# lachlants/denet

Hardware: AMD Instinct MI355X
Metric: images/sec train step, DeNet-34 skip 512x512 (higher is better)
Workload: dtype f32

## Files before the change

denet_amd/build.py:

```python
import hashlib
import os
import subprocess
import sys

HERE = os.path.dirname(os.path.abspath(__file__))
CSRC = os.path.join(HERE, "csrc")
LIB = os.path.join(CSRC, "libdenet_hip.so")

SOURCES = ["runtime.hip", "igemm.hip", "bn.hip", "pool.hip", "elementwise.hip", "dss.hip", "samples.hip", "detect.hip", "winograd.hip", "wino2f.hip", "wino4f.hip", "wino4t.hip", "dgrad_s2.hip", "wino4g.hip", "stem.hip", "gemm3b.hip", "bn_moments.hip",
           "regression.hip", "augment.hip", "image.hip", "activation.hip", "conv_rect.hip", "pool_border.hip"]
NO_CONTRACT = {"dss.hip", "samples.hip", "detect.hip", "augment.hip", "image.hip"}
COMMON = ["--offload-arch=gfx950", "-O3", "-std=c++17", "-fPIC", "-Wall", "-Wno-unused-function"]


def _hipcc_version(hipcc):
    try:
        return subprocess.run([hipcc, "--version"], check=True, capture_output=True, text=True).stdout
    except (OSError, subprocess.CalledProcessError):
        return "unknown"


def _digest(parts, files):
    h = hashlib.sha256()
    for p in parts:
        h.update(p.encode())
        h.update(b"\0")
    for f in files:
        with open(f, "rb") as fh:
            h.update(hashlib.sha256(fh.read()).digest())
    return h.hexdigest()


def _stale(target, digest):
    stamp = target + ".sha256"
    if not (os.path.exists(target) and os.path.exists(stamp)):
        return True
    with open(stamp) as f:
        return f.read().strip() != digest


def _stamp(target, digest):
    with open(target + ".sha256", "w") as f:
        f.write(digest + "\n")


def build(force=False, verbose=False):
    hipcc = os.environ.get("HIPCC", "/opt/rocm/bin/hipcc")
    if not os.path.exists(hipcc):
        hipcc = "hipcc"
    version = _hipcc_version(hipcc)
    objs, todo = [], []
    headers = [os.path.join(CSRC, "common.h"), os.path.join(CSRC, "bn_final.h"), os.path.join(HERE, "..", "include", "denet_hip.h")]
    for src in SOURCES:
        s = os.path.join(CSRC, src)
        o = os.path.join(CSRC, src.replace(".hip", ".o"))
        objs.append(o)
        flags = COMMON + (["-ffp-contract=off"] if src in NO_CONTRACT else [])
        digest = _digest([version] + flags, [s] + headers)
        if force or _stale(o, digest):
            todo.append(([hipcc] + flags + ["-c", s, "-o", o], o, digest))
    todo.sort(key=lambda t: -os.path.getsize(t[0][-3]))
    running = []
    jobs = max(1, min(len(todo), int(os.environ.get("DENET_BUILD_JOBS", os.cpu_count() or 1))))

    def reap(block):
        for ent in list(running):
            proc, cmd, o, digest = ent
            rc = proc.wait() if block else proc.poll()
            if rc is None:
                continue
            running.remove(ent)
            if rc != 0:
                for other in running:
                    other[0].kill()
                raise subprocess.CalledProcessError(rc, cmd)
            _stamp(o, digest)
            if block:
                return

    for cmd, o, digest in todo:
        while len(running) >= jobs:
            reap(block=True)
        if verbose:
            print(" ".join(cmd), flush=True)
        running.append((subprocess.Popen(cmd), cmd, o, digest))
    while running:
        reap(block=True)
    link = ["--offload-arch=gfx950", "-shared", "-fPIC"]
    digest = _digest([version] + link, objs)
    if force or _stale(LIB, digest):
        cmd = [hipcc] + link + ["-o", LIB] + objs
        if verbose:
            print(" ".join(cmd), flush=True)
        subprocess.run(cmd, check=True)
        _stamp(LIB, digest)
    return LIB


if __name__ == "__main__":
    print(build(force="--force" in sys.argv, verbose=True))
```

denet_amd/csrc/dgrad_s2.hip:

```cpp
#include "common.h"
#include "../../include/denet_hip.h"
#include <stdlib.h>

namespace {

typedef __attribute__((address_space(3))) void* lds_ptr_t;
typedef int i32x4_t __attribute__((ext_vector_type(4)));

__device__ __forceinline__ void s2_store_b128(const f32x4& v, const i32x4_t& rsrc, int voff, int soff) {
    asm volatile("buffer_store_dwordx4 %0, %1, %2, %3 offen\n\ts_nop 1" ::"v"(v), "v"(voff), "s"(rsrc), "s"(soff) : "memory");
}

struct S2Params {
    const float* dy;
    const float* wp;
    const float* add;
    float* dx;
    double* stats;
    const float* bs_x;
    const float* bs_y;
    const float* bs_gamma;
    const float* bs_beta;
    const float* bs_mean;
    const float* bs_invstd;
    int bs_relu;
    int N, H, W, C, K, OH, OW;
    int bh, bw;
    int tiles_c;
    int chunks;
    unsigned dy_bytes, dx_bytes, w_bytes;
};

constexpr int S2_OOB = (int)0xF0000000u;
constexpr int S2_SLOTS = 81 * 16;
constexpr int S2_PIECES = 21;
constexpr int S2_BUF = S2_PIECES * 1024;
constexpr int S2_LDS = 2 * S2_BUF + 1024;
constexpr int S2_D = 9;
constexpr int S2_R = 18;

#define S2_WAIT_VM(vm) __builtin_amdgcn_s_waitcnt(((vm) & 15) | ((((vm) >> 4) & 3) << 14) | (7 << 4) | (15 << 8))
#define S2_BARRIER()                       \
    {                                      \
        asm volatile("" ::: "memory");     \
        __builtin_amdgcn_s_barrier();      \
        asm volatile("" ::: "memory");     \
    }

__device__ __forceinline__ int s2_key(int pi, int pj) { return ((pi & 1) << 3) | (pj & 7); }

template <int EP>
__global__ __launch_bounds__(256, 2) void dgrad_s2_kernel(const S2Params p) {
    extern __shared__ __attribute__((aligned(16))) char smem[];
    const int tid = threadIdx.x, lane = tid & 63;
    const int wave = __builtin_amdgcn_readfirstlane(tid >> 6);
    const uint32_t bid = xcd_remap(blockIdx.x, gridDim.x);
    const int cblk = (int)(bid % (uint32_t)p.tiles_c);
    const int brow = (int)(bid / (uint32_t)p.tiles_c);
    int blk = brow;
    const int bx = blk % p.bw;
    blk /= p.bw;
    const int by = blk % p.bh;
    const int n = blk / p.bh;
    const int c0 = cblk * 64;
    const int i0 = by * 8, j0 = bx * 8;
    const __amdgpu_buffer_rsrc_t rD = __builtin_amdgcn_make_buffer_rsrc((void*)p.dy, 0, p.dy_bytes, 0x00020000);
    const __amdgpu_buffer_rsrc_t rW = __builtin_amdgcn_make_buffer_rsrc((void*)p.wp, 0, p.w_bytes, 0x00020000);

    int pc_off[6];
#pragma unroll
    for (int j = 0; j < 6; ++j) {
        const int L = (wave + 4 * j) * 64 + lane;
        const int pos = L >> 4, sl = L & 15;
        const int pi = pos / 9, pj = pos - pi * 9;
        const int i = i0 + pi, jj = j0 + pj;
        const bool ok = L < S2_SLOTS && i < p.OH && jj < p.OW;
        pc_off[j] = ok ? (((n * p.OH + i) * p.OW + jj) * p.K + 4 * (sl ^ s2_key(pi, pj))) * 4 : S2_OOB;
    }
    int d_chunk = 0;
    auto issue = [&]() {
        const bool live = d_chunk < p.chunks;
        char* const dstb = smem + (d_chunk & 1) * S2_BUF;
#pragma unroll
        for (int j = 0; j < 6; ++j) {
            const int piece = wave + 4 * j;
            char* const dst = piece < S2_PIECES ? dstb + piece * 1024 : smem + 2 * S2_BUF;
            __builtin_amdgcn_raw_ptr_buffer_load_lds(rD, (lds_ptr_t)dst, 16, live ? pc_off[j] : S2_OOB, d_chunk * 256, 0, 0);
        }
        d_chunk += 1;
    };

    const int r15 = lane & 15, g = lane >> 4;
    const int w_voff = ((c0 + 16 * wave + r15) * 16 + 4 * g) * 4;
    const int w_tap = p.C * 64;
    const int w_step = 9 * w_tap;
    const int pr = r15 >> 3, pq = r15 & 7;
    int v_base[2][2];
    int v_key[2][2];
#pragma unroll
    for (int di = 0; di < 2; ++di)
#pragma unroll
        for (int dj = 0; dj < 2; ++dj) {
            v_base[di][dj] = ((pr + di) * 9 + pq + dj) * 256;
            v_key[di][dj] = s2_key(pr + di, pq + dj);
        }

    f32x4 acc[4][4];
#pragma unroll
    for (int a = 0; a < 4; ++a)
#pragma unroll
        for (int b = 0; b < 4; ++b) acc[a][b] = f32x4{0.f, 0.f, 0.f, 0.f};

    f32x4 fw[S2_R];
    const int steps_total = p.chunks * 4;
    auto load_w = [&](int s, int gt) {
        int st = 4 * s + gt / 9;
        st = st < steps_total ? st : steps_total - 1;
        fw[gt % S2_R] = __builtin_bit_cast(f32x4, __builtin_amdgcn_raw_buffer_load_b128(rW, w_voff, st * w_step + (gt % 9) * w_tap, 0));
    };

    issue();
    issue();
#pragma unroll
    for (int t = 0; t < S2_D; ++t) load_w(0, t);

    for (int s = 0; s < p.chunks; ++s) {
        S2_WAIT_VM(S2_D);
        S2_BARRIER();
        if (s >= 1) issue();
        const char* const buf = smem + (s & 1) * S2_BUF;
#pragma unroll
        for (int q = 0; q < 4; ++q) {
            f32x4 dv[2][2][4];
#pragma unroll
            for (int di = 0; di < 2; ++di)
#pragma unroll
                for (int dj = 0; dj < 2; ++dj)
#pragma unroll
                    for (int pb = 0; pb < 4; ++pb)
                        dv[di][dj][pb] = *(const f32x4*)(buf + v_base[di][dj] + pb * (2 * 9 * 256) + (((4 * q + g) ^ v_key[di][dj]) << 4));
            __builtin_amdgcn_sched_barrier(0);
#pragma unroll
            for (int tap = 0; tap < 9; ++tap) {
                const int gt = 9 * q + tap;
                load_w(s, gt + S2_D);
                const int r = tap / 3, sx = tap % 3;
                const int py = r == 1 ? 0 : 1, di = r == 0 ? 1 : 0;
                const int px = sx == 1 ? 0 : 1, dj = sx == 0 ? 1 : 0;
                const f32x4 wv = fw[gt % S2_R];
#pragma unroll
                for (int k = 0; k < 4; ++k)
#pragma unroll
                    for (int pb = 0; pb < 4; ++pb)
                        acc[2 * py + px][pb] = __builtin_amdgcn_mfma_f32_16x16x4f32(wv[k], dv[di][dj][pb][k], acc[2 * py + px][pb], 0, 0, 0);
                __builtin_amdgcn_sched_group_barrier(0x008, 1, 0);
                __builtin_amdgcn_sched_group_barrier(0x020, 1, 0);
                __builtin_amdgcn_sched_group_barrier(0x008, 15, 0);
                __builtin_amdgcn_sched_barrier(0);
            }
        }
    }
    __builtin_amdgcn_s_waitcnt(0);

    const f32x4 z = {0.f, 0.f, 0.f, 0.f};
    const i32x4_t rsX = {(int)(unsigned)(unsigned long long)p.dx, (int)(((unsigned long long)p.dx >> 32) & 0xffffu), (int)p.dx_bytes, 0x00020000};
    const __amdgpu_buffer_rsrc_t rA = __builtin_amdgcn_make_buffer_rsrc((void*)p.add, 0, p.add ? p.dx_bytes : 0u, 0x00020000);
    const __amdgpu_buffer_rsrc_t rBX = __builtin_amdgcn_make_buffer_rsrc((void*)p.bs_x, 0, p.bs_x ? p.dx_bytes : 0u, 0x00020000);
    const __amdgpu_buffer_rsrc_t rBY = __builtin_amdgcn_make_buffer_rsrc((void*)p.bs_y, 0, p.bs_y ? p.dx_bytes : 0u, 0x00020000);
    const bool has_add = p.add != nullptr;
    const bool mask_y = p.bs_relu && p.bs_y, mask_x = p.bs_relu && !p.bs_y;
    const int kc = c0 + 16 * wave + 4 * g;
    double ds[8];
#pragma unroll
    for (int c = 0; c < 8; ++c) ds[c] = 0.0;
    f32x4 bmu = z, bis = z, bsc = z, bsh = z;
    if (EP == 2) {
        bmu = *(const f32x4*)(p.bs_mean + kc);
        bis = *(const f32x4*)(p.bs_invstd + kc);
#pragma unroll
        for (int c = 0; c < 4; ++c) {
            bsc[c] = (p.bs_gamma ? p.bs_gamma[kc + c] : 1.f) * bis[c];
            bsh[c] = (p.bs_beta ? p.bs_beta[kc + c] : 0.f) - bmu[c] * bsc[c];
        }
    }
#pragma unroll
    for (int pb = 0; pb < 4; ++pb) {
        const int i = i0 + 2 * pb + pr, j = j0 + pq;
        const bool valid = i < p.OH && j < p.OW;
        const int voff = valid ? (((n * p.H + 2 * i) * p.W + 2 * j) * p.C + kc) * 4 : S2_OOB;
        f32x4 ssum = z, ssq = z;
        f32x4 av[4], xv[4], yv[4];
#pragma unroll
        for (int cl = 0; cl < 4; ++cl) {
            const int soff = ((cl >> 1) * p.W + (cl & 1)) * p.C * 4;
            av[cl] = z;
            if (has_add) av[cl] = __builtin_bit_cast(f32x4, __builtin_amdgcn_raw_buffer_load_b128(rA, voff, soff, 0));
            if (EP == 2) {
                xv[cl] = __builtin_bit_cast(f32x4, __builtin_amdgcn_raw_buffer_load_b128(rBX, voff, soff, 0));
                yv[cl] = __builtin_bit_cast(f32x4, __builtin_amdgcn_raw_buffer_load_b128(rBY, voff, soff, 0));
            }
        }
#pragma unroll
        for (int cl = 0; cl < 4; ++cl) {
            const int soff = ((cl >> 1) * p.W + (cl & 1)) * p.C * 4;
            const f32x4 o = acc[cl][pb] + av[cl];
            s2_store_b128(o, rsX, voff, soff);
            if (EP == 2) {
                f32x4 gq;
#pragma unroll
                for (int c = 0; c < 4; ++c) {
                    const float mk = mask_y ? yv[cl][c] : (mask_x ? fmaf(xv[cl][c], bsc[c], bsh[c]) : 1.f);
                    gq[c] = mk > 0.f ? o[c] : 0.f;
                    ssq[c] += gq[c] * ((xv[cl][c] - bmu[c]) * bis[c]);
                }
                ssum += gq;
            }
        }
        if (EP == 2 && valid) {
#pragma unroll
            for (int c = 0; c < 4; ++c) {
                ds[c] += (double)ssum[c];
                ds[4 + c] += (double)ssq[c];
            }
        }
    }
    if (EP != 2) return;
#pragma unroll
    for (int c = 0; c < 8; ++c) {
#pragma unroll
        for (int sh = 8; sh > 0; sh >>= 1) {
            const long long b = __double_as_longlong(ds[c]);
            int lo, hi;
            if (sh == 8) { lo = __builtin_amdgcn_update_dpp(0, (int)b, 0x128, 0xF, 0xF, false); hi = __builtin_amdgcn_update_dpp(0, (int)(b >> 32), 0x128, 0xF, 0xF, false); }
            else if (sh == 4) { lo = __builtin_amdgcn_update_dpp(0, (int)b, 0x124, 0xF, 0xF, false); hi = __builtin_amdgcn_update_dpp(0, (int)(b >> 32), 0x124, 0xF, 0xF, false); }
            else if (sh == 2) { lo = __builtin_amdgcn_update_dpp(0, (int)b, 0x122, 0xF, 0xF, false); hi = __builtin_amdgcn_update_dpp(0, (int)(b >> 32), 0x122, 0xF, 0xF, false); }
            else { lo = __builtin_amdgcn_update_dpp(0, (int)b, 0x121, 0xF, 0xF, false); hi = __builtin_amdgcn_update_dpp(0, (int)(b >> 32), 0x121, 0xF, 0xF, false); }
            ds[c] += __longlong_as_double(((long long)hi << 32) | (unsigned)lo);
        }
    }
    if (r15 == 0 && kc < p.C) {
        double* row = p.stats + (long)brow * 2 * p.C;
#pragma unroll
        for (int c = 0; c < 4; ++c) {
            row[kc + c] = ds[c];
            row[p.C + kc + c] = ds[4 + c];
        }
    }
}

__global__ __launch_bounds__(256) void dgrad_s2_pack_kernel(const float* __restrict__ w, float* __restrict__ P, int K, int C) {
    const long idx = (long)blockIdx.x * 256 + threadIdx.x;
    const long total = 9L * K * C;
    if (idx >= total) return;
    const int kk = (int)(idx & 15);
    long rest = idx >> 4;
    const int c = (int)(rest % C);
    rest /= C;
    const int tap = (int)(rest % 9);
    const int kc = (int)(rest / 9);
    P[idx] = w[((long)(kc * 16 + kk) * 9 + tap) * C + c];
}

}

extern "C" int denet_conv_dgrad_s2_ok(int N, int H, int W, int C, int K) {
    return (N > 0 && H > 0 && W > 0 && H % 2 == 0 && W % 2 == 0 && C > 0 && C % 64 == 0 && K > 0 && K % 64 == 0 &&
            (long)N * H * W * C * 4 < 0x7FFFFFFFL && (long)N * (H / 2) * (W / 2) * K * 4 < 0x7FFFFFFFL && 9L * K * C * 4 < 0x7FFFFFFFL) ? 1 : 0;
}

extern "C" int denet_conv_dgrad_s2_stats_rows(int N, int H, int W) {
    return N * ((H / 2 + 7) / 8) * ((W / 2 + 7) / 8);
}

extern "C" int denet_conv_dgrad_s2_pack(const float* w, float* packed, int C, int K, hipStream_t stream) {
    DENET_CHECK_ARG(w && packed && C > 0 && K > 0 && K % 16 == 0, "conv_dgrad_s2_pack: bad arguments");
    const long total = 9L * K * C;
    hipLaunchKernelGGL(dgrad_s2_pack_kernel, dim3((unsigned)((total + 255) / 256)), dim3(256), 0, stream, w, packed, K, C);
    DENET_CHECK_LAUNCH("conv_dgrad_s2_pack");
    return DENET_OK;
}

extern "C" int denet_conv_dgrad_s2(const float* dy, const float* w_packed, const float* add, float* dx, const denet_bn_link* sums_of,
                                   double* stats_partial, size_t stats_bytes, int* stats_rows, int N, int H, int W, int C, int K,
                                   hipStream_t stream) {
    DENET_CHECK_ARG(dy && w_packed && dx, "conv_dgrad_s2: null pointer");
    DENET_CHECK_ARG(denet_conv_dgrad_s2_ok(N, H, W, C, K), "conv_dgrad_s2: needs even H and W, C %% 64 = 0, K %% 64 = 0");
    S2Params p = {};
    p.dy = dy; p.wp = w_packed; p.add = add; p.dx = dx;
    p.N = N; p.H = H; p.W = W; p.C = C; p.K = K; p.OH = H / 2; p.OW = W / 2;
    p.bh = (p.OH + 7) / 8; p.bw = (p.OW + 7) / 8;
    p.tiles_c = C / 64; p.chunks = K / 64;
    p.dy_bytes = (unsigned)((size_t)N * p.OH * p.OW * K * 4);
    p.dx_bytes = (unsigned)((size_t)N * H * W * C * 4);
    p.w_bytes = (unsigned)((size_t)9 * K * C * 4);
    const long blocks = (long)N * p.bh * p.bw;
    int ep = 0;
    if (sums_of) {
        DENET_CHECK_ARG(stats_partial && stats_rows && stats_bytes >= (size_t)blocks * 2 * C * sizeof(double), "conv_dgrad_s2: statistics buffer too small");
        DENET_CHECK_ARG(sums_of->x && sums_of->mean && sums_of->invstd && (!sums_of->relu || sums_of->y || (sums_of->gamma && sums_of->beta)),
                        "conv_dgrad_s2: incomplete batch-norm description for the backward sums");
        *stats_rows = (int)blocks;
        p.stats = stats_partial;
        p.bs_x = sums_of->x; p.bs_y = sums_of->relu ? sums_of->y : nullptr; p.bs_gamma = sums_of->gamma; p.bs_beta = sums_of->beta;
        p.bs_mean = sums_of->mean; p.bs_invstd = sums_of->invstd; p.bs_relu = sums_of->relu;
        ep = 2;
    } else if (stats_rows) {
        *stats_rows = 0;
    }
    typedef void (*kern_t)(const S2Params);
    const kern_t fn = ep == 2 ? dgrad_s2_kernel<2> : dgrad_s2_kernel<0>;
    const int prof = denet_prof_begin(17, ep, 0, 0, stream);
    hipLaunchKernelGGL(fn, dim3((unsigned)(blocks * p.tiles_c)), dim3(256), S2_LDS, stream, p);
    denet_prof_end(prof, stream);
    DENET_CHECK_LAUNCH("conv_dgrad_s2");
    return DENET_OK;
}
```

denet_amd/csrc/gemm3b.hip:

```cpp
#include "common.h"

namespace {

typedef __bf16 bf16x8 __attribute__((ext_vector_type(8)));
typedef __bf16 bf16x2 __attribute__((ext_vector_type(2)));
typedef float f32x2 __attribute__((ext_vector_type(2)));
typedef unsigned u32x4 __attribute__((ext_vector_type(4)));

constexpr int BM = 128, BN = 128, BK = 32;
constexpr int ROWB = 80;
constexpr int IMG = BM * ROWB;
constexpr int OOBV = (int)0xF0000000u;

struct G3Params {
    const float* a;
    const float* b;
    const float* bias;
    float* c;
    int M, N, K;
    unsigned a_bytes, b_bytes;
};

__device__ __forceinline__ void split4(const f32x4 v, unsigned (&hi)[2], unsigned (&lo)[2]) {
#pragma unroll
    for (int p = 0; p < 2; ++p) {
        const f32x2 x = {v[2 * p], v[2 * p + 1]};
        const unsigned h = __builtin_bit_cast(unsigned, __builtin_convertvector(x, bf16x2));
        const f32x2 back = {__builtin_bit_cast(float, h << 16), __builtin_bit_cast(float, h & 0xFFFF0000u)};
        const f32x2 r = x - back;
        hi[p] = h;
        lo[p] = __builtin_bit_cast(unsigned, __builtin_convertvector(r, bf16x2));
    }
}

__global__ __launch_bounds__(256, 3) void gemm3b_nt_kernel(const G3Params p) {
    __shared__ __attribute__((aligned(16))) char smem[4 * IMG];
    char* Ah = smem;
    char* Al = smem + IMG;
    char* Bh = smem + 2 * IMG;
    char* Bl = smem + 3 * IMG;
    const int tid = threadIdx.x, lane = tid & 63, wave = tid >> 6;
    const int wm = wave & 1, wn = wave >> 1;
    const uint32_t tiles_n = p.N / BN;
    const uint32_t tile = xcd_remap(blockIdx.x, gridDim.x);
    const int m0 = (int)(tile / tiles_n) * BM, n0 = (int)(tile % tiles_n) * BN;
    const __amdgpu_buffer_rsrc_t ra = __builtin_amdgcn_make_buffer_rsrc((void*)p.a, 0, p.a_bytes, 0x00020000);
    const __amdgpu_buffer_rsrc_t rb = __builtin_amdgcn_make_buffer_rsrc((void*)p.b, 0, p.b_bytes, 0x00020000);
    const int lrow = tid >> 3, lk = (tid & 7) * 4;
    const int a_off = ((m0 + lrow) * p.K + lk) * 4, b_off = ((n0 + lrow) * p.K + lk) * 4;
    f32x4 ga[4], gb[4];
    auto gload = [&](int k0) {
#pragma unroll
        for (int i = 0; i < 4; ++i) {
            ga[i] = __builtin_bit_cast(f32x4, __builtin_amdgcn_raw_buffer_load_b128(
                ra, m0 + lrow + 32 * i < p.M ? a_off + (32 * i * p.K + k0) * 4 : OOBV, 0, 0));
            gb[i] = __builtin_bit_cast(f32x4, __builtin_amdgcn_raw_buffer_load_b128(rb, b_off + (32 * i * p.K + k0) * 4, 0, 0));
        }
    };
    typedef unsigned u32x2 __attribute__((ext_vector_type(2)));
    auto stage = [&]() {
#pragma unroll
        for (int i = 0; i < 4; ++i) {
            const int o = (lrow + 32 * i) * ROWB + lk * 2;
            unsigned h[2], l[2];
            split4(ga[i], h, l);
            *(u32x2*)(Ah + o) = u32x2{h[0], h[1]};
            *(u32x2*)(Al + o) = u32x2{l[0], l[1]};
            split4(gb[i], h, l);
            *(u32x2*)(Bh + o) = u32x2{h[0], h[1]};
            *(u32x2*)(Bl + o) = u32x2{l[0], l[1]};
        }
    };

    f32x16 acc[2][2];
#pragma unroll
    for (int i = 0; i < 2; ++i)
#pragma unroll
        for (int j = 0; j < 2; ++j)
#pragma unroll
            for (int e = 0; e < 16; ++e) acc[i][j][e] = 0.f;

    const int fa = (64 * wm + (lane & 31)) * ROWB + (lane >> 5) * 16;
    const int fb = (64 * wn + (lane & 31)) * ROWB + (lane >> 5) * 16;

    gload(0);
    stage();
    __syncthreads();
    const int nk = p.K / BK;
    for (int kb = 0; kb < nk; ++kb) {
        if (kb + 1 < nk) gload((kb + 1) * BK);
#pragma unroll
        for (int ks = 0; ks < 2; ++ks) {
            bf16x8 ah[2], al[2], bh[2], bl[2];
#pragma unroll
            for (int t = 0; t < 2; ++t) {
                ah[t] = *(const bf16x8*)(Ah + fa + t * 32 * ROWB + ks * 32);
                al[t] = *(const bf16x8*)(Al + fa + t * 32 * ROWB + ks * 32);
                bh[t] = *(const bf16x8*)(Bh + fb + t * 32 * ROWB + ks * 32);
                bl[t] = *(const bf16x8*)(Bl + fb + t * 32 * ROWB + ks * 32);
            }
#pragma unroll
            for (int i = 0; i < 2; ++i)
#pragma unroll
                for (int j = 0; j < 2; ++j) {
                    acc[i][j] = __builtin_amdgcn_mfma_f32_32x32x16_bf16(bh[j], al[i], acc[i][j], 0, 0, 0);
                    acc[i][j] = __builtin_amdgcn_mfma_f32_32x32x16_bf16(bl[j], ah[i], acc[i][j], 0, 0, 0);
                    acc[i][j] = __builtin_amdgcn_mfma_f32_32x32x16_bf16(bh[j], ah[i], acc[i][j], 0, 0, 0);
                }
        }
        __syncthreads();
        if (kb + 1 < nk) {
            stage();
            __syncthreads();
        }
    }
#pragma unroll
    for (int i = 0; i < 2; ++i) {
        const int m = m0 + 64 * wm + 32 * i + (lane & 31);
        if (m >= p.M) continue;
#pragma unroll
        for (int j = 0; j < 2; ++j)
#pragma unroll
            for (int q = 0; q < 4; ++q) {
                const int n = n0 + 64 * wn + 32 * j + 8 * q + 4 * (lane >> 5);
                f32x4 v = {acc[i][j][4 * q], acc[i][j][4 * q + 1], acc[i][j][4 * q + 2], acc[i][j][4 * q + 3]};
                if (p.bias) v += *(const f32x4*)(p.bias + n);
                *(f32x4*)(p.c + (long)m * p.N + n) = v;
            }
    }
}

__global__ __launch_bounds__(256) void transpose_f32_kernel(const float* __restrict__ src, float* __restrict__ dst, int R, int C) {
    __shared__ float tile[64][65];
    const int r0 = blockIdx.y * 64, c0 = blockIdx.x * 64;
    const int tx = threadIdx.x & 63, ty = threadIdx.x >> 6;
#pragma unroll
    for (int i = 0; i < 16; ++i) {
        const int r = r0 + ty + 4 * i, c = c0 + tx;
        tile[ty + 4 * i][tx] = (r < R && c < C) ? src[(long)r * C + c] : 0.f;
    }
    __syncthreads();
#pragma unroll
    for (int i = 0; i < 16; ++i) {
        const int c = c0 + ty + 4 * i, r = r0 + tx;
        if (r < R && c < C) dst[(long)c * R + r] = tile[tx][ty + 4 * i];
    }
}

}

extern "C" int denet_gemm_bf16x3_ok(int M, int N, int K) {
    return (M > 0 && N > 0 && K > 0 && N % 128 == 0 && K % 32 == 0 && (long)M * K * 4 < 0xF0000000L && (long)N * K * 4 < 0xF0000000L) ? 1 : 0;
}

extern "C" int denet_gemm_bf16x3_nt(const float* a, const float* b, const float* bias, float* c, int M, int N, int K,
                                    hipStream_t stream) {
    DENET_CHECK_ARG(a && b && c, "gemm_bf16x3_nt: null pointer");
    DENET_CHECK_ARG(denet_gemm_bf16x3_ok(M, N, K), "gemm_bf16x3_nt: needs N %% 128 = 0, K %% 32 = 0");
    G3Params p = {a, b, bias, c, M, N, K, (unsigned)((size_t)M * K * 4), (unsigned)((size_t)N * K * 4)};
    const unsigned tiles = (unsigned)(((M + BM - 1) / BM) * (N / BN));
    hipLaunchKernelGGL(gemm3b_nt_kernel, dim3(tiles), dim3(256), 0, stream, p);
    DENET_CHECK_LAUNCH("gemm_bf16x3_nt");
    return DENET_OK;
}

extern "C" int denet_transpose_f32(const float* src, float* dst, int R, int C, hipStream_t stream) {
    DENET_CHECK_ARG(src && dst && R > 0 && C > 0, "transpose_f32: bad arguments");
    hipLaunchKernelGGL(transpose_f32_kernel, dim3((C + 63) / 64, (R + 63) / 64), dim3(256), 0, stream, src, dst, R, C);
    DENET_CHECK_LAUNCH("transpose_f32");
    return DENET_OK;
}
```

denet_amd/csrc/wino4t.hip:

```cpp
#include "common.h"
#include "bn_final.h"
#include "../../include/denet_hip.h"
#include <stdlib.h>
#include <type_traits>

namespace {

typedef __attribute__((address_space(3))) void* lds_ptr_t;
typedef float f32x2 __attribute__((ext_vector_type(2)));
typedef int i32x4_t __attribute__((ext_vector_type(4)));

__device__ __forceinline__ void t_store_b128(const f32x4& v, const i32x4_t& rsrc, int voff, int soff) {
    asm volatile("buffer_store_dwordx4 %0, %1, %2, %3 offen\n\ts_nop 1" ::"v"(v), "v"(voff), "s"(rsrc), "s"(soff) : "memory");
}

struct W4TParams {
    const float* x;
    const float* U;
    const float* bias;
    const float* add;
    float* y;
    double* stats;
    const float* bs_x;
    const float* bs_y;
    const float* bs_gamma;
    const float* bs_beta;
    const float* bs_mean;
    const float* bs_invstd;
    int bs_relu;
    int N, H, W, C, K;
    int bh, bw;
    int tiles_k;
    int chunks;
    int relu;
    unsigned x_bytes, y_bytes, u_bytes;
    unsigned long long* dbg;
};

constexpr int T_OOB = (int)0xF0000000u;
constexpr int T_ROWS = 10;
constexpr int T_QS = 38;
constexpr int T_PLANE_SLOTS = T_ROWS * T_QS;
constexpr int T_PLANE_B = T_PLANE_SLOTS * 16;
constexpr int T_PATCH_SLOTS = 4 * T_PLANE_SLOTS;
constexpr int T_PATCH_B = 24 * 1024;
constexpr int T_V_B = 36 * 1024;
constexpr int T_LDS = T_PATCH_B + T_V_B;
#ifndef T_STAG
#define T_STAG 0
#endif
#ifndef T_STAG_N
#define T_STAG_N 1
#endif
#ifndef T_D_
#define T_D_ 3
#endif
#ifndef T_ISSUE_
#define T_ISSUE_ 9
#endif
constexpr int T_D = T_D_;
constexpr int T_R = 12;
constexpr int T_ISSUE = T_ISSUE_;
static_assert(36 % T_R == 0 && T_R >= 2 * T_D + 2, "the ring index must run on across chunks and cover the fragments in flight");

#define T_WAITCNT(vm) __builtin_amdgcn_s_waitcnt(((vm) & 15) | ((((vm) >> 4) & 3) << 14) | (7 << 4))
#define T_WAIT_VM(vm) __builtin_amdgcn_s_waitcnt(((vm) & 15) | ((((vm) >> 4) & 3) << 14) | (7 << 4) | (15 << 8))
#define T_BARRIER()                        \
    {                                      \
        asm volatile("" ::: "memory");     \
        __builtin_amdgcn_s_barrier();      \
        asm volatile("" ::: "memory");     \
    }

template <int LH>
__device__ __forceinline__ void t_bt3(const f32x2 (&d)[6], f32x2 (&o)[3]) {
    if (LH == 0) {
        o[0] = __builtin_elementwise_fma(f32x2{-5.f, -5.f}, d[2], __builtin_elementwise_fma(f32x2{4.f, 4.f}, d[0], d[4]));
        const f32x2 p = __builtin_elementwise_fma(f32x2{-4.f, -4.f}, d[2], d[4]);
        const f32x2 q = __builtin_elementwise_fma(f32x2{-4.f, -4.f}, d[1], d[3]);
        o[1] = p + q;
        o[2] = p - q;
    } else {
        const f32x2 p = d[4] - d[2];
        const f32x2 q = d[3] - d[1];
        o[0] = __builtin_elementwise_fma(f32x2{2.f, 2.f}, q, p);
        o[1] = __builtin_elementwise_fma(f32x2{-2.f, -2.f}, q, p);
        o[2] = __builtin_elementwise_fma(f32x2{-5.f, -5.f}, d[3], __builtin_elementwise_fma(f32x2{4.f, 4.f}, d[1], d[5]));
    }
}
__device__ __forceinline__ void t_bt6(const f32x2 (&t)[6], f32x2 (&o)[6]) {
    o[0] = __builtin_elementwise_fma(f32x2{-5.f, -5.f}, t[2], __builtin_elementwise_fma(f32x2{4.f, 4.f}, t[0], t[4]));
    const f32x2 p = __builtin_elementwise_fma(f32x2{-4.f, -4.f}, t[2], t[4]);
    const f32x2 q = __builtin_elementwise_fma(f32x2{-4.f, -4.f}, t[1], t[3]);
    o[1] = p + q;
    o[2] = p - q;
    const f32x2 p2 = t[4] - t[2];
    const f32x2 q2 = t[3] - t[1];
    o[3] = __builtin_elementwise_fma(f32x2{2.f, 2.f}, q2, p2);
    o[4] = __builtin_elementwise_fma(f32x2{-2.f, -2.f}, q2, p2);
    o[5] = __builtin_elementwise_fma(f32x2{-5.f, -5.f}, t[3], __builtin_elementwise_fma(f32x2{4.f, 4.f}, t[1], t[5]));
}

template <int LH>
__device__ __forceinline__ void t_transform(const char* prd, char* vwr) {
    f32x2 t[3][6];
#pragma unroll
    for (int b = 0; b < 6; ++b) {
        f32x2 d[6];
#pragma unroll
        for (int a = LH; a < LH + 5; ++a) d[a] = *(const f32x2*)(prd + (a * T_QS + (b & 3) * 9 + (b >> 2)) * 16);
        if (LH == 0) d[5] = f32x2{0.f, 0.f};
        else d[0] = f32x2{0.f, 0.f};
        f32x2 o[3];
        t_bt3<LH>(d, o);
        t[0][b] = o[0];
        t[1][b] = o[1];
        t[2][b] = o[2];
    }
#pragma unroll
    for (int i = 0; i < 3; ++i) {
        f32x2 o[6];
        t_bt6(t[i], o);
#pragma unroll
        for (int m = 0; m < 6; ++m) *(f32x2*)(vwr + (6 * (3 * LH + i) + m) * 1024) = o[m];
    }
}

template <int N>
__device__ __forceinline__ double t_row_ror(double v) {
    const long long b = __double_as_longlong(v);
    const int lo = __builtin_amdgcn_update_dpp(0, (int)b, 0x120 + N, 0xF, 0xF, false);
    const int hi = __builtin_amdgcn_update_dpp(0, (int)(b >> 32), 0x120 + N, 0xF, 0xF, false);
    return __longlong_as_double(((long long)hi << 32) | (unsigned)lo);
}

constexpr float T_AT[4][6] = {{1, 1, 1, 1, 1, 0}, {0, 1, -1, 2, -2, 0}, {0, 1, 1, 4, 4, 0}, {0, 1, -1, 8, -8, 1}};

#ifdef T_TRACE
#define T_STAMP() if (p.dbg && (blockIdx.x & 63) == 0 && tid == 0 && dbg_n < 32) p.dbg[(blockIdx.x >> 6) * 32 + dbg_n++] = __builtin_amdgcn_s_memtime()
#else
#define T_STAMP()
#endif
#ifndef T_EXP
#define T_EXP 0
#endif

template <int EP>
__global__ __launch_bounds__(256, 2) void wino4t_kernel(const W4TParams p) {
    extern __shared__ __attribute__((aligned(16))) char smem[];
    char* const vbuf = smem + T_PATCH_B;
    const int tid = threadIdx.x, lane = tid & 63;
    const int wave = __builtin_amdgcn_readfirstlane(tid >> 6);
    const uint32_t bid = xcd_remap(blockIdx.x, gridDim.x);
    const int kblk = (int)(bid % (uint32_t)p.tiles_k);
    const int brow = (int)(bid / (uint32_t)p.tiles_k);
    int blk = brow;
    const int bx = blk % p.bw;
    blk /= p.bw;
    const int by = blk % p.bh;
    const int n = blk / p.bh;
    const int k0 = kblk * 64;
    const int y0 = by * 8, x0 = bx * 32;
    const __amdgpu_buffer_rsrc_t rX = __builtin_amdgcn_make_buffer_rsrc((void*)p.x, 0, p.x_bytes, 0x00020000);

    int pc_off[6];
#pragma unroll
    for (int j = 0; j < 6; ++j) {
        const int L = (wave + 4 * j) * 64 + lane;
        const int pl = L / T_PLANE_SLOTS, rem = L - pl * T_PLANE_SLOTS;
        const int row = rem / T_QS, q = rem - row * T_QS;
        const int v = q / 9, u = q - v * 9;
        const int pcx = 4 * u + v;
        const int iy = y0 - 1 + row, ix = x0 - 1 + pcx;
        const bool ok = L < T_PATCH_SLOTS && q < 36 && pcx < 34 && (unsigned)iy < (unsigned)p.H && (unsigned)ix < (unsigned)p.W;
        pc_off[j] = ok ? (((n * p.H + iy) * p.W + ix) * p.C + pl * 4) * 4 : T_OOB;
    }
    int d_chunk = 0;
    auto issue = [&]() {
        if (T_EXP & 8) return;
        const bool live = d_chunk < p.chunks;
#pragma unroll
        for (int j = 0; j < 6; ++j)
            __builtin_amdgcn_raw_ptr_buffer_load_lds(rX, (lds_ptr_t)(smem + (wave + 4 * j) * 1024), 16, live ? pc_off[j] : T_OOB,
                                                     d_chunk * 64, 0, 0);
        d_chunk += 1;
    };

    const int t_half = lane & 1, t_tx = (lane >> 1) & 7, t_ty = (lane >> 4) & 1;
    const int t_cq = ((lane >> 5) & 1) | ((wave & 1) << 1), t_lh = wave >> 1;
    const int t_rd = t_cq * T_PLANE_B + (4 * t_ty * T_QS + t_tx) * 16 + t_half * 8;
    char* const t_wr = vbuf + t_cq * 256 + (t_ty * 8 + t_tx) * 16 + t_half * 8;

    const int r15 = lane & 15, g = lane >> 4;
    const int kw = wave;
    const char* const v_rd = vbuf + g * 256 + r15 * 16;
    const __amdgpu_buffer_rsrc_t rU = __builtin_amdgcn_make_buffer_rsrc((void*)p.U, 0, p.u_bytes, 0x00020000);
    const int u_voff = ((k0 + 16 * ((T_EXP & 256) ? (kw & 1) : kw) + r15) * 16 + 4 * g) * 4;
    const int u_xi = p.K * 64;
    const int u_chunk = 36 * u_xi;

    f32x4 acc[36];
#pragma unroll
    for (int i = 0; i < 36; ++i) acc[i] = f32x4{0.f, 0.f, 0.f, 0.f};

    f32x4 fu[T_R];
    if (T_EXP & 32) {
#pragma unroll
        for (int i = 0; i < T_R; ++i) asm volatile("" : "=v"(fu[i]));
    }
    auto load_u = [&](int chunk, int pair) {
        if (T_EXP & 32) return;
        if ((T_EXP & 128) && (pair & 1)) {
            fu[(2 * pair) % T_R] = fu[(2 * pair - 2) % T_R];
            fu[(2 * pair + 1) % T_R] = fu[(2 * pair - 1) % T_R];
            return;
        }
        const int so = chunk * u_chunk + (2 * pair) * u_xi;
        fu[(2 * pair) % T_R] = __builtin_bit_cast(f32x4, __builtin_amdgcn_raw_buffer_load_b128(rU, u_voff, so, 0));
        fu[(2 * pair + 1) % T_R] = __builtin_bit_cast(f32x4, __builtin_amdgcn_raw_buffer_load_b128(rU, u_voff, so + u_xi, 0));
    };
    f32x4 fv[2][2];
    if (T_EXP & 64) asm volatile("" : "=v"(fv[0][0]), "=v"(fv[0][1]), "=v"(fv[1][0]), "=v"(fv[1][1]));
    auto read_v = [&](int pair) {
        if (T_EXP & 64) return;
        fv[pair & 1][0] = *(const f32x4*)(v_rd + (2 * pair) * 1024);
        fv[pair & 1][1] = *(const f32x4*)(v_rd + (2 * pair + 1) * 1024);
    };

#if T_STAG
    {
        const bool late = T_STAG == 1 ? ((blockIdx.x >> 8) & 1) && blockIdx.x < 512 : (blockIdx.x & 1) && blockIdx.x < 512;
        if (late) {
#pragma unroll
            for (int i = 0; i < T_STAG_N; ++i) __builtin_amdgcn_s_sleep(115);
        }
    }
#endif
    int dbg_n = 0;
    (void)dbg_n;
    T_STAMP();
    issue();
    if (!(T_EXP & 2)) {
#pragma unroll
        for (int pr = 0; pr < T_D; ++pr) load_u(0, pr);
    }

    for (int s = 0; s < p.chunks; ++s) {
        T_WAIT_VM(2 * T_D);
        T_STAMP();
        T_BARRIER();
        T_STAMP();
        if (!(T_EXP & 1)) {
            const char* prd = smem + t_rd;
            if (t_lh == 0) t_transform<0>(prd, t_wr);
            else t_transform<1>(prd, t_wr);
        }
        T_WAITCNT(63);
        T_STAMP();
        T_BARRIER();
        T_STAMP();
        if (!(T_EXP & 2)) {
            const int sn = s + 1 < p.chunks ? s + 1 : s;
            read_v(0);
            __builtin_amdgcn_sched_barrier(0);
#pragma unroll
            for (int pr = 0; pr < 18; ++pr) {
                if (pr + T_D < 18) load_u(s, pr + T_D);
                else load_u(sn, pr + T_D - 18);
                if (pr + 1 < 18) read_v(pr + 1);
                const f32x4 ua = fu[(2 * pr) % T_R], ub = fu[(2 * pr + 1) % T_R];
                const f32x4 va = fv[pr & 1][0], vb = fv[pr & 1][1];
#pragma unroll
                for (int j = 0; j < 4; ++j) {
                    acc[2 * pr] = __builtin_amdgcn_mfma_f32_16x16x4f32(ua[j], va[j], acc[2 * pr], 0, 0, 0);
                    acc[2 * pr + 1] = __builtin_amdgcn_mfma_f32_16x16x4f32(ub[j], vb[j], acc[2 * pr + 1], 0, 0, 0);
                }
                __builtin_amdgcn_sched_group_barrier(0x008, 1, 0);
                __builtin_amdgcn_sched_group_barrier(0x020, 1, 0);
                __builtin_amdgcn_sched_group_barrier(0x008, 1, 0);
                __builtin_amdgcn_sched_group_barrier(0x020, 1, 0);
                if (pr + 1 < 18) {
                    __builtin_amdgcn_sched_group_barrier(0x008, 1, 0);
                    __builtin_amdgcn_sched_group_barrier(0x100, 1, 0);
                    __builtin_amdgcn_sched_group_barrier(0x008, 1, 0);
                    __builtin_amdgcn_sched_group_barrier(0x100, 1, 0);
                    __builtin_amdgcn_sched_group_barrier(0x008, 4, 0);
                } else {
                    __builtin_amdgcn_sched_group_barrier(0x008, 6, 0);
                }
                __builtin_amdgcn_sched_barrier(0);
                if (pr == T_ISSUE && s + 1 < p.chunks) {
                    issue();
                    __builtin_amdgcn_sched_barrier(0);
                }
            }
        } else if (s + 1 < p.chunks) {
            issue();
        }
    }
    T_STAMP();
    if (T_EXP & 4) {
#pragma unroll
        for (int i = 0; i < 36; ++i) asm volatile("" ::"v"(acc[i]));
        return;
    }

    f32x4 Y[16];
    {
        f32x4 Z[6][4];
#pragma unroll
        for (int l = 0; l < 6; ++l)
#pragma unroll
            for (int j = 0; j < 4; ++j) {
                f32x4 a = {0.f, 0.f, 0.f, 0.f};
                bool fst = true;
#pragma unroll
                for (int m = 0; m < 6; ++m) {
                    const float c = T_AT[j][m];
                    if (c == 0.f) continue;
                    if (fst) a = c == 1.f ? acc[6 * l + m] : acc[6 * l + m] * c;
                    else if (c == 1.f) a += acc[6 * l + m];
                    else if (c == -1.f) a -= acc[6 * l + m];
                    else a = __builtin_elementwise_fma(f32x4{c, c, c, c}, acc[6 * l + m], a);
                    fst = false;
                }
                Z[l][j] = a;
            }
#pragma unroll
        for (int i = 0; i < 4; ++i)
#pragma unroll
            for (int j = 0; j < 4; ++j) {
                f32x4 a = {0.f, 0.f, 0.f, 0.f};
                bool fst = true;
#pragma unroll
                for (int l = 0; l < 6; ++l) {
                    const float c = T_AT[i][l];
                    if (c == 0.f) continue;
                    if (fst) a = c == 1.f ? Z[l][j] : Z[l][j] * c;
                    else if (c == 1.f) a += Z[l][j];
                    else if (c == -1.f) a -= Z[l][j];
                    else a = __builtin_elementwise_fma(f32x4{c, c, c, c}, Z[l][j], a);
                    fst = false;
                }
                Y[4 * i + j] = a;
            }
    }

    T_STAMP();
    const int oy = y0 + 4 * (r15 >> 3), ox = x0 + 4 * (r15 & 7);
    const f32x4 z = {0.f, 0.f, 0.f, 0.f};
    const i32x4_t rsY = {(int)(unsigned)(unsigned long long)p.y, (int)(((unsigned long long)p.y >> 32) & 0xffffu), (int)p.y_bytes, 0x00020000};
    const __amdgpu_buffer_rsrc_t rA = __builtin_amdgcn_make_buffer_rsrc((void*)p.add, 0, p.add ? p.y_bytes : 0u, 0x00020000);
    const __amdgpu_buffer_rsrc_t rBX = __builtin_amdgcn_make_buffer_rsrc((void*)p.bs_x, 0, p.bs_x ? p.y_bytes : 0u, 0x00020000);
    const __amdgpu_buffer_rsrc_t rBY = __builtin_amdgcn_make_buffer_rsrc((void*)p.bs_y, 0, p.bs_y ? p.y_bytes : 0u, 0x00020000);
    const float floor_ = p.relu ? 0.f : -__builtin_inff();
    const bool has_add = p.add != nullptr;
    const bool mask_y = p.bs_relu && p.bs_y, mask_x = p.bs_relu && !p.bs_y;
    double ds[8];
    const int kc = k0 + 16 * kw + 4 * g;
    const bool valid = oy < p.H && ox < p.W && kc < p.K;
    {
#pragma unroll
        for (int c = 0; c < 8; ++c) ds[c] = 0.0;
        const int voff = valid ? (((n * p.H + oy) * p.W + ox) * p.K + kc) * 4 : T_OOB;
        const int voff_st = (T_EXP & 16) ? (valid ? (voff & 0xFFFFF) : T_OOB) : voff;
        const int kcs = valid ? kc : 0;
        f32x4 b = z;
        if (p.bias) b = *(const f32x4*)(p.bias + kcs);
        f32x4 bmu = z, bis = z, bsc = z, bsh = z;
        if (EP == 2) {
            bmu = *(const f32x4*)(p.bs_mean + kcs);
            bis = *(const f32x4*)(p.bs_invstd + kcs);
#pragma unroll
            for (int c = 0; c < 4; ++c) {
                bsc[c] = (p.bs_gamma ? p.bs_gamma[kcs + c] : 1.f) * bis[c];
                bsh[c] = (p.bs_beta ? p.bs_beta[kcs + c] : 0.f) - bmu[c] * bsc[c];
            }
        }
#pragma unroll
        for (int i = 0; i < 4; ++i) {
            f32x4 ssum = z, ssq = z;
            f32x4 av[4], xv[4], yv[4];
#pragma unroll
            for (int j = 0; j < 4; ++j) {
                const int soff = (i * p.W + j) * p.K * 4;
                av[j] = z;
                if (has_add) av[j] = __builtin_bit_cast(f32x4, __builtin_amdgcn_raw_buffer_load_b128(rA, voff, soff, 0));
                if (EP == 2) {
                    xv[j] = __builtin_bit_cast(f32x4, __builtin_amdgcn_raw_buffer_load_b128(rBX, voff, soff, 0));
                    yv[j] = __builtin_bit_cast(f32x4, __builtin_amdgcn_raw_buffer_load_b128(rBY, voff, soff, 0));
                }
            }
#pragma unroll
            for (int j = 0; j < 4; ++j) {
                const int soff = (i * p.W + j) * p.K * 4;
                f32x4 o = (Y[4 * i + j] + b) + av[j];
#pragma unroll
                for (int c = 0; c < 4; ++c) o[c] = fmaxf(o[c], floor_);
                t_store_b128(o, rsY, voff_st, soff);
                if (EP == 2) {
                    f32x4 gq;
#pragma unroll
                    for (int c = 0; c < 4; ++c) {
                        const float mk = mask_y ? yv[j][c] : (mask_x ? fmaf(xv[j][c], bsc[c], bsh[c]) : 1.f);
                        gq[c] = mk > 0.f ? o[c] : 0.f;
                        ssq[c] += gq[c] * ((xv[j][c] - bmu[c]) * bis[c]);
                    }
                    ssum += gq;
                } else if (EP == 1) {
                    ssum += o;
                    ssq += o * o;
                }
            }
            if (EP != 0 && valid) {
#pragma unroll
                for (int c = 0; c < 4; ++c) {
                    ds[c] += (double)ssum[c];
                    ds[4 + c] += (double)ssq[c];
                }
            }
        }
    }
    T_STAMP();
    if (EP == 0) return;
#pragma unroll
    for (int c = 0; c < 8; ++c) {
        ds[c] += t_row_ror<8>(ds[c]);
        ds[c] += t_row_ror<4>(ds[c]);
        ds[c] += t_row_ror<2>(ds[c]);
        ds[c] += t_row_ror<1>(ds[c]);
    }
    if (r15 == 0 && kc < p.K) {
        double* row = p.stats + (long)brow * 2 * p.K;
#pragma unroll
        for (int c = 0; c < 4; ++c) {
            row[kc + c] = ds[c];
            row[p.K + kc + c] = ds[4 + c];
        }
    }
    T_STAMP();
}

__global__ __launch_bounds__(256) void wino4t_pack_kernel(const float* __restrict__ U, float* __restrict__ P, int K, int C) {
    const long idx = (long)blockIdx.x * 256 + threadIdx.x;
    const long total = 36L * K * C / 4;
    if (idx >= total) return;
    const int q = (int)(idx & 3);
    long rest = idx >> 2;
    const int k = (int)(rest % K);
    rest /= K;
    const int xi = (int)(rest % 36);
    const int chunk = (int)(rest / 36);
    *(f32x4*)(P + idx * 4) = *(const f32x4*)(U + ((long)xi * K + k) * C + chunk * 16 + q * 4);
}

unsigned long long* g_w4t_dbg = nullptr;

}

#ifdef T_TRACE
extern "C" int denet_conv_wino4t_debug(unsigned long long* buf) { g_w4t_dbg = buf; return 0; }
#endif

extern "C" int denet_conv_wino4t_ok(int N, int H, int W, int C, int K) {
    return (N > 0 && H > 0 && W > 0 && H % 4 == 0 && W % 4 == 0 && C > 0 && C % 16 == 0 && K > 0 && K % 64 == 0 &&
            (long)N * H * W * C * 4 < 0x7FFFFFFFL && (long)N * H * W * K * 4 < 0x7FFFFFFFL && 36L * K * C * 4 < 0x7FFFFFFFL) ? 1 : 0;
}

extern "C" int denet_conv_wino4t_stats_rows(int N, int H, int W) {
    return N * ((H + 7) / 8) * ((W + 31) / 32);
}

extern "C" int denet_conv_wino4t_pack(const float* u, float* packed, int C, int K, hipStream_t stream) {
    DENET_CHECK_ARG(u && packed && C > 0 && C % 16 == 0 && K > 0, "conv_wino4t_pack: bad arguments");
    const long total = 36L * K * C / 4;
    hipLaunchKernelGGL(wino4t_pack_kernel, dim3((unsigned)((total + 255) / 256)), dim3(256), 0, stream, u, packed, K, C);
    DENET_CHECK_LAUNCH("conv_wino4t_pack");
    return DENET_OK;
}

extern "C" int denet_conv_wino4t_sums(const float* x, const float* u_packed, const float* bias, const float* add, float* y, int relu,
                                      double* stats_partial, size_t stats_bytes, int* stats_rows, const denet_bn_link* sums_of, int N,
                                      int H, int W, int C, int K, hipStream_t stream) {
    DENET_CHECK_ARG(x && u_packed && y, "conv_wino4t: null pointer");
    DENET_CHECK_ARG(denet_conv_wino4t_ok(N, H, W, C, K), "conv_wino4t: needs H, W %% 4 = 0, C %% 16 = 0, K %% 64 = 0");
    W4TParams p = {};
    p.x = x; p.U = u_packed; p.bias = bias; p.add = add; p.y = y;
    p.N = N; p.H = H; p.W = W; p.C = C; p.K = K;
    p.bh = (H + 7) / 8; p.bw = (W + 31) / 32;
    p.tiles_k = K / 64; p.chunks = C / 16; p.relu = relu;
    p.x_bytes = (unsigned)((size_t)N * H * W * C * 4);
    p.y_bytes = (unsigned)((size_t)N * H * W * K * 4);
    p.u_bytes = (unsigned)((size_t)36 * K * C * 4);
    p.dbg = g_w4t_dbg;
    const long blocks = (long)N * p.bh * p.bw;
    int ep = 0;
    if (stats_partial) {
        DENET_CHECK_ARG(stats_rows && stats_bytes >= (size_t)blocks * 2 * K * sizeof(double), "conv_wino4t: statistics buffer too small");
        *stats_rows = (int)blocks;
        p.stats = stats_partial;
        ep = 1;
        if (sums_of) {
            DENET_CHECK_ARG(sums_of->x && sums_of->mean && sums_of->invstd && (!sums_of->relu || sums_of->y || (sums_of->gamma && sums_of->beta)),
                            "conv_wino4t: incomplete batch-norm description for the backward sums");
            p.bs_x = sums_of->x; p.bs_y = sums_of->relu ? sums_of->y : nullptr; p.bs_gamma = sums_of->gamma; p.bs_beta = sums_of->beta;
            p.bs_mean = sums_of->mean; p.bs_invstd = sums_of->invstd; p.bs_relu = sums_of->relu;
            ep = 2;
        }
    }
    typedef void (*kern_t)(const W4TParams);
    static const kern_t kerns[3] = {wino4t_kernel<0>, wino4t_kernel<1>, wino4t_kernel<2>};
    static bool attr_done[3] = {};
    const kern_t fn = kerns[ep];
    if (!attr_done[ep]) {
        const hipError_t e = hipFuncSetAttribute((const void*)fn, hipFuncAttributeMaxDynamicSharedMemorySize, 163840);
        if (e != hipSuccess) {
            denet_set_error("conv_wino4t: hipFuncSetAttribute(%d B LDS): %s", T_LDS, hipGetErrorString(e));
            return -(int)e;
        }
        attr_done[ep] = true;
    }
    static const int lds_req = [] { const char* e = getenv("DENET_W4T_LDS"); const int v = e ? atoi(e) : 0; return v > T_LDS && v <= 163840 ? v : T_LDS; }();
    const int prof = denet_prof_begin(16, ep, 0, 0, stream);
    hipLaunchKernelGGL(fn, dim3((unsigned)(blocks * p.tiles_k)), dim3(256), lds_req, stream, p);
    denet_prof_end(prof, stream);
    DENET_CHECK_LAUNCH("conv_wino4t");
    return DENET_OK;
}
```

denet_amd/csrc/winograd.hip:

```cpp
#include "common.h"
#include <stdlib.h>
#include "../../include/denet_hip.h"

int denet_gemm_batched_nt(const float* a, const float* w, float* out, int batch, int M, int Nc, int Kc, long stride_a,
                          long stride_w, long stride_out, hipStream_t stream);
int denet_gemm_batched_tune(const float* a, const float* w, float* out, int batch, int M, int Nc, int Kc, long stride_a,
                            long stride_w, long stride_out, hipStream_t stream);

int denet_wgrad_batched(const float* x, const float* dy, float* dw, float* workspace, size_t workspace_bytes, int batch,
                        int T, int Cc, int Kr, hipStream_t stream);
int denet_wgrad_batched_tune(const float* x, const float* dy, float* dw, float* workspace, size_t workspace_bytes, int batch,
                             int T, int Cc, int Kr, hipStream_t stream);

int denet_wino4f_block(int tile, long T, int C, int K);
int denet_wino4f_stats_rows(int tb, long T);
int denet_wino4f_run(int tb, const float* V, const float* U, const float* bias, const float* add, float* y, double* stats,
                     const float* bs_x, const float* bs_y, const float* bs_gamma, const float* bs_beta, const float* bs_mean,
                     const float* bs_invstd, int bs_relu, int N, int H, int W, int C, int K, int relu, hipStream_t stream);

int denet_wino4g_splits(int tile, long T, int C, int K);
size_t denet_wino4g_workspace_bytes(int splits, int C, int K);
int denet_wino4g_run(int splits, const float* dM, const float* V, float* dU, float* part, size_t part_bytes, long T, int C, int K,
                     hipStream_t stream);

namespace {

__device__ __forceinline__ f32x4 ld4(const float* p) { return *(const f32x4*)p; }

template <int MO>
struct Wino;
template <>
struct Wino<2> {
    static constexpr int TS = 4;
    static constexpr float BT[4][4] = {{1, 0, -1, 0}, {0, 1, 1, 0}, {0, -1, 1, 0}, {0, 1, 0, -1}};
    static constexpr float G[4][3] = {{1, 0, 0}, {0.5f, 0.5f, 0.5f}, {0.5f, -0.5f, 0.5f}, {0, 0, 1}};
    static constexpr float AT[2][4] = {{1, 1, 1, 0}, {0, 1, -1, -1}};
};
template <>
struct Wino<4> {
    static constexpr int TS = 6;
    static constexpr float BT[6][6] = {{4, 0, -5, 0, 1, 0},  {0, -4, -4, 1, 1, 0}, {0, 4, -4, -1, 1, 0},
                                       {0, -2, -1, 2, 1, 0}, {0, 2, -1, -2, 1, 0}, {0, 4, 0, -5, 0, 1}};
    static constexpr float G[6][3] = {{0.25f, 0, 0},
                                      {-1.f / 6, -1.f / 6, -1.f / 6},
                                      {-1.f / 6, 1.f / 6, -1.f / 6},
                                      {1.f / 24, 1.f / 12, 1.f / 6},
                                      {1.f / 24, -1.f / 12, 1.f / 6},
                                      {0, 0, 1}};
    static constexpr float AT[4][6] = {{1, 1, 1, 1, 1, 0}, {0, 1, -1, 2, -2, 0}, {0, 1, 1, 4, 4, 0}, {0, 1, -1, 8, -8, 1}};
};

__device__ __forceinline__ float wino_fma(float c, float v, float acc) { return __builtin_fmaf(c, v, acc); }
__device__ __forceinline__ f32x4 wino_fma(float c, f32x4 v, f32x4 acc) {
    f32x4 r;
    r[0] = __builtin_fmaf(c, v[0], acc[0]);
    r[1] = __builtin_fmaf(c, v[1], acc[1]);
    r[2] = __builtin_fmaf(c, v[2], acc[2]);
    r[3] = __builtin_fmaf(c, v[3], acc[3]);
    return r;
}

#define WINO_DOT(acc, NL, COEF, VAL)                       \
    {                                                      \
        bool first_ = true;                                \
        _Pragma("unroll") for (int l_ = 0; l_ < (NL); ++l_) { \
            const float c_ = (COEF);                       \
            if (c_ != 0.f) {                               \
                if (first_) acc = c_ * (VAL);              \
                else acc = wino_fma(c_, (VAL), acc);       \
                first_ = false;                            \
            }                                              \
        }                                                  \
    }

template <int MO>
__global__ __launch_bounds__(256) void wino_input_kernel(const float* __restrict__ x, float* __restrict__ V, int N, int H,
                                                         int W, int C, int TH, int TW, long T, int up) {
    using WT = Wino<MO>;
    constexpr int TS = WT::TS;
    const int c4n = C / 4;
    const long idx = (long)blockIdx.x * 256 + threadIdx.x;
    if (idx >= T * c4n) return;
    const int c4 = (int)(idx % c4n);
    const long t = idx / c4n;
    const int tx = (int)(t % TW);
    const int ty = (int)((t / TW) % TH);
    const int n = (int)(t / ((long)TW * TH));
    const f32x4 z = {0.f, 0.f, 0.f, 0.f};
    f32x4 tt[TS][TS];
#pragma unroll
    for (int j = 0; j < TS; ++j) {
        const int ix = MO * tx - 1 + j;
        f32x4 d[TS];
#pragma unroll
        for (int i = 0; i < TS; ++i) {
            const int iy = MO * ty - 1 + i;
            const bool ok = ((unsigned)iy < (unsigned)H) && ((unsigned)ix < (unsigned)W);
            d[i] = ok ? ld4(x + (((long)n * (H >> up) + (iy >> up)) * (W >> up) + (ix >> up)) * C + c4 * 4) : z;
        }
#pragma unroll
        for (int i = 0; i < TS; ++i) {
            f32x4 acc = z;
            WINO_DOT(acc, TS, WT::BT[i][l_], d[l_]);
            tt[i][j] = acc;
        }
    }
#pragma unroll
    for (int i = 0; i < TS; ++i)
#pragma unroll
        for (int j = 0; j < TS; ++j) {
            f32x4 acc = z;
            WINO_DOT(acc, TS, WT::BT[j][l_], tt[i][l_]);
            *(f32x4*)(V + ((long)(TS * i + j) * T + t) * C + c4 * 4) = acc;
        }
}

struct BnFoldDev {
    const float* x;
    const float* aux;
    const float* y;
    const float* gamma;
    const float* beta;
    const float* mean;
    const float* invstd;
    const float* coef;
    float* out;
    int relu;
};

template <int MO, bool BWD>
__global__ __launch_bounds__(256) void wino_prep_kernel(BnFoldDev f, float* __restrict__ V, float* __restrict__ dM, int N, int H,
                                                        int W, int C, int TH, int TW, long T) {
    using WT = Wino<MO>;
    constexpr int TS = WT::TS;
    const int c4n = C / 4;
    const long idx = (long)blockIdx.x * 256 + threadIdx.x;
    if (idx >= T * c4n) return;
    const int c4 = (int)(idx % c4n);
    const long t = idx / c4n;
    const int tx = (int)(t % TW);
    const int ty = (int)((t / TW) % TH);
    const int n = (int)(t / ((long)TW * TH));
    const int c = c4 * 4;
    const f32x4 z = {0.f, 0.f, 0.f, 0.f};
    float mu[4], is[4], sc[4], sh[4], mg[4], mgx[4];
#pragma unroll
    for (int k = 0; k < 4; ++k) {
        mu[k] = f.mean[c + k];
        is[k] = f.invstd[c + k];
        sc[k] = f.gamma[c + k] * is[k];
        sh[k] = (f.beta ? f.beta[c + k] : 0.f) - mu[k] * sc[k];
        mg[k] = BWD ? f.coef[c + k] : 0.f;
        mgx[k] = BWD ? f.coef[C + c + k] : 0.f;
    }
    auto value = [&](int iy, int ix, bool inner) -> f32x4 {
        if (!(((unsigned)iy < (unsigned)H) && ((unsigned)ix < (unsigned)W))) return z;
        const long o = (((long)n * H + iy) * W + ix) * C + c;
        const f32x4 xv = ld4(f.x + o);
        f32x4 d;
        if (!BWD) {
#pragma unroll
            for (int k = 0; k < 4; ++k) d[k] = fmaf(xv[k], sc[k], sh[k]);
            if (f.aux) d += ld4(f.aux + o);
            if (f.relu) {
#pragma unroll
                for (int k = 0; k < 4; ++k) d[k] = fmaxf(d[k], 0.f);
            }
            if (inner) *(f32x4*)(f.out + o) = d;
        } else {
            f32x4 g = ld4(f.aux + o);
            if (f.relu) {
                if (f.y) {
                    const f32x4 yv = ld4(f.y + o);
#pragma unroll
                    for (int k = 0; k < 4; ++k) g[k] = yv[k] > 0.f ? g[k] : 0.f;
                } else {
#pragma unroll
                    for (int k = 0; k < 4; ++k) g[k] = fmaf(xv[k], sc[k], sh[k]) > 0.f ? g[k] : 0.f;
                }
            }
#pragma unroll
            for (int k = 0; k < 4; ++k) {
                const float xh = (xv[k] - mu[k]) * is[k];
                d[k] = sc[k] * (g[k] - mg[k] - xh * mgx[k]);
            }
            if (inner && f.out) *(f32x4*)(f.out + o) = g;
        }
        return d;
    };
    {
        f32x4 tt[TS][TS];
#pragma unroll
        for (int j = 0; j < TS; ++j) {
            const int ix = MO * tx - 1 + j;
            f32x4 d[TS];
#pragma unroll
            for (int i = 0; i < TS; ++i) d[i] = value(MO * ty - 1 + i, ix, i >= 1 && i <= MO && j >= 1 && j <= MO);
#pragma unroll
            for (int i = 0; i < TS; ++i) {
                f32x4 acc = z;
                WINO_DOT(acc, TS, WT::BT[i][l_], d[l_]);
                tt[i][j] = acc;
            }
        }
#pragma unroll
        for (int i = 0; i < TS; ++i)
#pragma unroll
            for (int j = 0; j < TS; ++j) {
                f32x4 acc = z;
                WINO_DOT(acc, TS, WT::BT[j][l_], tt[i][l_]);
                *(f32x4*)(V + ((long)(TS * i + j) * T + t) * C + c) = acc;
            }
    }
    if (BWD) {
        f32x4 a[TS][MO];
#pragma unroll
        for (int j = 0; j < MO; ++j) {
            f32x4 d[MO];
#pragma unroll
            for (int i = 0; i < MO; ++i) d[i] = value(MO * ty + i, MO * tx + j, false);
#pragma unroll
            for (int i = 0; i < TS; ++i) {
                f32x4 acc = z;
                WINO_DOT(acc, MO, WT::AT[l_][i], d[l_]);
                a[i][j] = acc;
            }
        }
#pragma unroll
        for (int i = 0; i < TS; ++i)
#pragma unroll
            for (int j = 0; j < TS; ++j) {
                f32x4 acc = z;
                WINO_DOT(acc, MO, WT::AT[l_][j], a[i][l_]);
                *(f32x4*)(dM + ((long)(TS * i + j) * T + t) * C + c) = acc;
            }
    }
}

template <int MO, bool BWD>
struct PrepLds {
    static constexpr int BT = 4;
    static constexpr int CQ = 8;
    static constexpr int PB = BT * MO;
    static constexpr int PP = PB + 2;
    static constexpr int NT = BT * BT * CQ;
    static constexpr int PS = CQ + 1;
    static constexpr size_t LDS = (size_t)PP * PP * PS * sizeof(f32x4);
};

template <int MO, bool BWD>
__global__ __launch_bounds__(128) void wino_prep_lds_kernel(BnFoldDev f, float* __restrict__ V, float* __restrict__ dM, int N,
                                                            int H, int W, int C, int TH, int TW, long T, int BH, int BW) {
    using WT = Wino<MO>;
    using PL = PrepLds<MO, BWD>;
    static_assert(PL::NT == 128, "launch bounds");
    constexpr int TS = WT::TS, BT = PL::BT, CQ = PL::CQ, PB = PL::PB, PP = PL::PP, NT = PL::NT, PS = PL::PS;
    extern __shared__ __attribute__((aligned(16))) unsigned char prep_smem[];
    f32x4* patch = (f32x4*)prep_smem;
    const int tid = threadIdx.x;
    const int cq = tid % CQ;
    const int cblk = blockIdx.y;
    const int c = (cblk * CQ + cq) * 4;
    int b = blockIdx.x;
    const int bx = b % BW; b /= BW;
    const int by = b % BH;
    const int n = b / BH;
    const f32x4 z = {0.f, 0.f, 0.f, 0.f};
    float mu[4], is[4], sc[4], sh[4], mg[4], mgx[4];
#pragma unroll
    for (int k = 0; k < 4; ++k) {
        mu[k] = f.mean[c + k];
        is[k] = f.invstd[c + k];
        sc[k] = f.gamma[c + k] * is[k];
        sh[k] = (f.beta ? f.beta[c + k] : 0.f) - mu[k] * sc[k];
        mg[k] = BWD ? f.coef[c + k] : 0.f;
        mgx[k] = BWD ? f.coef[C + c + k] : 0.f;
    }
    const int y0 = by * PB - 1, x0 = bx * PB - 1;
    constexpr int SLOTS = NT / CQ;
    constexpr int ROUNDS = (PP * PP + SLOTS - 1) / SLOTS;
    constexpr int UB = 7;
    for (int r0 = 0; r0 < ROUNDS; r0 += UB) {
        f32x4 xv[UB], av[UB], yv[UB];
        long off[UB];
        int pix[UB];
        bool ok[UB], inner[UB];
#pragma unroll
        for (int u = 0; u < UB; ++u) {
            const int p = (r0 + u) * SLOTS + tid / CQ;
            const int py = p / PP, px = p - py * PP;
            const int iy = y0 + py, ix = x0 + px;
            pix[u] = p;
            ok[u] = p < PP * PP && ((unsigned)iy < (unsigned)H) && ((unsigned)ix < (unsigned)W);
            inner[u] = py >= 1 && py <= PB && px >= 1 && px <= PB;
            off[u] = ok[u] ? (((long)n * H + iy) * W + ix) * C + c : (long)c;
            xv[u] = ld4(f.x + off[u]);
            if (BWD || f.aux) av[u] = ld4(f.aux + off[u]);
            if (BWD && f.relu && f.y) yv[u] = ld4(f.y + off[u]);
        }
#pragma unroll
        for (int u = 0; u < UB; ++u) {
            f32x4 d = z;
            if (!BWD) {
#pragma unroll
                for (int k = 0; k < 4; ++k) d[k] = fmaf(xv[u][k], sc[k], sh[k]);
                if (f.aux) d += av[u];
                if (f.relu) {
#pragma unroll
                    for (int k = 0; k < 4; ++k) d[k] = fmaxf(d[k], 0.f);
                }
                if (ok[u] && inner[u]) *(f32x4*)(f.out + off[u]) = d;
            } else {
                f32x4 g = av[u];
                if (f.relu) {
                    if (f.y) {
#pragma unroll
                        for (int k = 0; k < 4; ++k) g[k] = yv[u][k] > 0.f ? g[k] : 0.f;
                    } else {
#pragma unroll
                        for (int k = 0; k < 4; ++k) g[k] = fmaf(xv[u][k], sc[k], sh[k]) > 0.f ? g[k] : 0.f;
                    }
                }
#pragma unroll
                for (int k = 0; k < 4; ++k) {
                    const float xh = (xv[u][k] - mu[k]) * is[k];
                    d[k] = sc[k] * (g[k] - mg[k] - xh * mgx[k]);
                }
                if (ok[u] && inner[u] && f.out) *(f32x4*)(f.out + off[u]) = g;
            }
            if (pix[u] < PP * PP) patch[pix[u] * PS + cq] = ok[u] ? d : z;
        }
    }
    __syncthreads();
    const int tl = tid / CQ;
    const int tyl = tl / BT, txl = tl - tyl * BT;
    const int ty = by * BT + tyl, tx = bx * BT + txl;
    if (ty >= TH || tx >= TW) return;
    const long t = ((long)n * TH + ty) * TW + tx;
    {
        f32x4 tt[TS][TS];
#pragma unroll
        for (int j = 0; j < TS; ++j) {
            f32x4 d[TS];
#pragma unroll
            for (int i = 0; i < TS; ++i) d[i] = patch[((MO * tyl + i) * PP + MO * txl + j) * PS + cq];
#pragma unroll
            for (int i = 0; i < TS; ++i) {
                f32x4 acc = z;
                WINO_DOT(acc, TS, WT::BT[i][l_], d[l_]);
                tt[i][j] = acc;
            }
        }
#pragma unroll
        for (int i = 0; i < TS; ++i)
#pragma unroll
            for (int j = 0; j < TS; ++j) {
                f32x4 acc = z;
                WINO_DOT(acc, TS, WT::BT[j][l_], tt[i][l_]);
                *(f32x4*)(V + ((long)(TS * i + j) * T + t) * C + c) = acc;
            }
    }
    if (BWD) {
        f32x4 a[TS][MO];
#pragma unroll
        for (int j = 0; j < MO; ++j) {
            f32x4 d[MO];
#pragma unroll
            for (int i = 0; i < MO; ++i) d[i] = patch[((MO * tyl + 1 + i) * PP + MO * txl + 1 + j) * PS + cq];
#pragma unroll
            for (int i = 0; i < TS; ++i) {
                f32x4 acc = z;
                WINO_DOT(acc, MO, WT::AT[l_][i], d[l_]);
                a[i][j] = acc;
            }
        }
#pragma unroll
        for (int i = 0; i < TS; ++i)
#pragma unroll
            for (int j = 0; j < TS; ++j) {
                f32x4 acc = z;
                WINO_DOT(acc, MO, WT::AT[l_][j], a[i][l_]);
                *(f32x4*)(dM + ((long)(TS * i + j) * T + t) * C + c) = acc;
            }
    }
}

template <int MO, bool BWD>
int launch_prep_lds(const BnFoldDev& f, float* V, float* dM, int N, int H, int W, int C, int TH, int TW, long T, hipStream_t stream) {
    using PL = PrepLds<MO, BWD>;
    static bool attr_set = false;
    if (!attr_set) {
        const hipError_t e = hipFuncSetAttribute((const void*)wino_prep_lds_kernel<MO, BWD>, hipFuncAttributeMaxDynamicSharedMemorySize,
                                                 (int)PL::LDS);
        if (e != hipSuccess) {
            denet_set_error("conv_wino fold: hipFuncSetAttribute(%zu B LDS): %s", PL::LDS, hipGetErrorString(e));
            return -(int)e;
        }
        attr_set = true;
    }
    const int BH = (TH + PL::BT - 1) / PL::BT, BW = (TW + PL::BT - 1) / PL::BT;
    hipLaunchKernelGGL((wino_prep_lds_kernel<MO, BWD>), dim3((unsigned)(N * BH * BW), (unsigned)(C / (4 * PL::CQ))), dim3(PL::NT),
                       PL::LDS, stream, f, V, dM, N, H, W, C, TH, TW, T, BH, BW);
    return DENET_OK;
}

template <int MO, bool DGRAD>
__global__ __launch_bounds__(256) void wino_filter_kernel(const float* __restrict__ w, float* __restrict__ U, int K, int C) {
    using WT = Wino<MO>;
    constexpr int TS = WT::TS;
    const long idx = (long)blockIdx.x * 256 + threadIdx.x;
    if (idx >= (long)K * C) return;
    const int c = (int)(idx % C);
    const int k = (int)(idx / C);
    float g[3][3];
#pragma unroll
    for (int r = 0; r < 3; ++r)
#pragma unroll
        for (int s = 0; s < 3; ++s) g[r][s] = w[(((long)k * 3 + (DGRAD ? 2 - r : r)) * 3 + (DGRAD ? 2 - s : s)) * C + c];
    float a[TS][3];
#pragma unroll
    for (int i = 0; i < TS; ++i)
#pragma unroll
        for (int s = 0; s < 3; ++s) {
            float acc = 0.f;
            WINO_DOT(acc, 3, WT::G[i][l_], g[l_][s]);
            a[i][s] = acc;
        }
    const long KC = (long)K * C;
    const long o = DGRAD ? ((long)c * K + k) : ((long)k * C + c);
#pragma unroll
    for (int i = 0; i < TS; ++i)
#pragma unroll
        for (int j = 0; j < TS; ++j) {
            float acc = 0.f;
            WINO_DOT(acc, 3, WT::G[j][l_], a[i][l_]);
            U[(long)(TS * i + j) * KC + o] = acc;
        }
}

template <int MO>
__global__ __launch_bounds__(256) void wino_filter_dgrad_kernel(const float* __restrict__ w, float* __restrict__ U, int K,
                                                                int C) {
    using WT = Wino<MO>;
    constexpr int TS = WT::TS;
    __shared__ float tile[TS * TS][16][17];
    const int kl = threadIdx.x >> 4, cl = threadIdx.x & 15;
    const int k0 = blockIdx.y * 16, c0 = blockIdx.x * 16;
    {
        const int k = k0 + kl, c = c0 + cl;
        float g[3][3];
#pragma unroll
        for (int r = 0; r < 3; ++r)
#pragma unroll
            for (int q = 0; q < 3; ++q) g[r][q] = w[(((long)k * 3 + (2 - r)) * 3 + (2 - q)) * C + c];
        float a[TS][3];
#pragma unroll
        for (int i = 0; i < TS; ++i)
#pragma unroll
            for (int q = 0; q < 3; ++q) {
                float acc = 0.f;
                WINO_DOT(acc, 3, WT::G[i][l_], g[l_][q]);
                a[i][q] = acc;
            }
#pragma unroll
        for (int i = 0; i < TS; ++i)
#pragma unroll
            for (int j = 0; j < TS; ++j) {
                float acc = 0.f;
                WINO_DOT(acc, 3, WT::G[j][l_], a[i][l_]);
                tile[TS * i + j][cl][kl] = acc;
            }
    }
    __syncthreads();
    const long KC = (long)K * C;
    const int co = threadIdx.x >> 4, ko = threadIdx.x & 15;
#pragma unroll
    for (int xi = 0; xi < TS * TS; ++xi) U[(long)xi * KC + (long)(c0 + co) * K + k0 + ko] = tile[xi][co][ko];
}

template <int MO>
__global__ __launch_bounds__(256) void wino_output_kernel(const float* __restrict__ Mx, const float* __restrict__ bias,
                                                          const float* __restrict__ add, float* __restrict__ y, int N,
                                                          int H, int W, int K, int TH, int TW, long T, int relu,
                                                          double* __restrict__ stats, BnFoldDev bs) {
    using WT = Wino<MO>;
    constexpr int TS = WT::TS;
    __shared__ double red[2][256][4];
    const int k4n = K / 4;
    const long idx = (long)blockIdx.x * 256 + threadIdx.x;
    const bool valid = idx < T * k4n;
    const f32x4 z = {0.f, 0.f, 0.f, 0.f};
    double dsum[4] = {0.0, 0.0, 0.0, 0.0}, dsq[4] = {0.0, 0.0, 0.0, 0.0};
    if (valid) {
        const int k4 = (int)(idx % k4n);
        const long t = idx / k4n;
        const int tx = (int)(t % TW);
        const int ty = (int)((t / TW) % TH);
        const int n = (int)(t / ((long)TW * TH));
        f32x4 s[MO][TS];
#pragma unroll
        for (int j = 0; j < TS; ++j) {
            f32x4 m[TS];
#pragma unroll
            for (int i = 0; i < TS; ++i) m[i] = ld4(Mx + ((long)(TS * i + j) * T + t) * K + k4 * 4);
#pragma unroll
            for (int i = 0; i < MO; ++i) {
                f32x4 acc = z;
                WINO_DOT(acc, TS, WT::AT[i][l_], m[l_]);
                s[i][j] = acc;
            }
        }
        f32x4 b = z;
        if (bias) b = ld4(bias + k4 * 4);
        float bs_mu[4] = {0.f, 0.f, 0.f, 0.f}, bs_is[4] = {0.f, 0.f, 0.f, 0.f}, bs_sc[4] = {0.f, 0.f, 0.f, 0.f}, bs_sh[4] = {0.f, 0.f, 0.f, 0.f};
        if (bs.x) {
#pragma unroll
            for (int c = 0; c < 4; ++c) {
                bs_mu[c] = bs.mean[k4 * 4 + c];
                bs_is[c] = bs.invstd[k4 * 4 + c];
                bs_sc[c] = (bs.gamma ? bs.gamma[k4 * 4 + c] : 1.f) * bs_is[c];
                bs_sh[c] = (bs.beta ? bs.beta[k4 * 4 + c] : 0.f) - bs_mu[c] * bs_sc[c];
            }
        }
#pragma unroll
        for (int i = 0; i < MO; ++i) {
            f32x4 ssum = z, ssq = z;
#pragma unroll
            for (int j = 0; j < MO; ++j) {
                f32x4 acc = z;
                WINO_DOT(acc, TS, WT::AT[j][l_], s[i][l_]);
                if (MO * ty + i >= H || MO * tx + j >= W) continue;
                const long o = (((long)n * H + MO * ty + i) * W + MO * tx + j) * K + k4 * 4;
                acc += b;
                if (add) acc += ld4(add + o);
                if (relu) {
                    acc[0] = fmaxf(acc[0], 0.f);
                    acc[1] = fmaxf(acc[1], 0.f);
                    acc[2] = fmaxf(acc[2], 0.f);
                    acc[3] = fmaxf(acc[3], 0.f);
                }
                *(f32x4*)(y + o) = acc;
                if (bs.x) {
                    const f32x4 xv = ld4(bs.x + o);
                    f32x4 g = acc;
                    if (bs.relu) {
                        if (bs.y) {
                            const f32x4 yv = ld4(bs.y + o);
#pragma unroll
                            for (int c = 0; c < 4; ++c) g[c] = yv[c] > 0.f ? g[c] : 0.f;
                        } else {
#pragma unroll
                            for (int c = 0; c < 4; ++c) g[c] = fmaf(xv[c], bs_sc[c], bs_sh[c]) > 0.f ? g[c] : 0.f;
                        }
                    }
                    ssum += g;
#pragma unroll
                    for (int c = 0; c < 4; ++c) ssq[c] += g[c] * ((xv[c] - bs_mu[c]) * bs_is[c]);
                } else {
                    ssum += acc;
                    ssq += acc * acc;
                }
            }
            if (stats) {
#pragma unroll
                for (int c = 0; c < 4; ++c) {
                    dsum[c] += (double)ssum[c];
                    dsq[c] += (double)ssq[c];
                }
            }
        }
    }
    if (!stats) return;
#pragma unroll
    for (int c = 0; c < 4; ++c) {
        red[0][threadIdx.x][c] = dsum[c];
        red[1][threadIdx.x][c] = dsq[c];
    }
    __syncthreads();
    for (int st = 128; st >= k4n; st >>= 1) {
        if ((int)threadIdx.x < st) {
#pragma unroll
            for (int c = 0; c < 4; ++c) {
                red[0][threadIdx.x][c] += red[0][threadIdx.x + st][c];
                red[1][threadIdx.x][c] += red[1][threadIdx.x + st][c];
            }
        }
        __syncthreads();
    }
    if ((int)threadIdx.x < k4n) {
        double* ps = stats + (long)blockIdx.x * 2 * K + threadIdx.x * 4;
#pragma unroll
        for (int c = 0; c < 4; ++c) {
            ps[c] = red[0][threadIdx.x][c];
            ps[K + c] = red[1][threadIdx.x][c];
        }
    }
}

template <int MO>
__global__ __launch_bounds__(256) void wino_dout_kernel(const float* __restrict__ dy, float* __restrict__ dM, int N, int H,
                                                        int W, int K, int TH, int TW, long T) {
    using WT = Wino<MO>;
    constexpr int TS = WT::TS;
    const int k4n = K / 4;
    const long idx = (long)blockIdx.x * 256 + threadIdx.x;
    if (idx >= T * k4n) return;
    const int k4 = (int)(idx % k4n);
    const long t = idx / k4n;
    const int tx = (int)(t % TW);
    const int ty = (int)((t / TW) % TH);
    const int n = (int)(t / ((long)TW * TH));
    const f32x4 z = {0.f, 0.f, 0.f, 0.f};
    f32x4 a[TS][MO];
#pragma unroll
    for (int j = 0; j < MO; ++j) {
        f32x4 d[MO];
#pragma unroll
        for (int i = 0; i < MO; ++i) {
            const int oy = MO * ty + i, ox = MO * tx + j;
            const bool in = oy < H && ox < W;
            const f32x4 v = ld4(dy + (((long)n * H + (in ? oy : 0)) * W + (in ? ox : 0)) * K + k4 * 4);
            d[i] = in ? v : z;
        }
#pragma unroll
        for (int i = 0; i < TS; ++i) {
            f32x4 acc = z;
            WINO_DOT(acc, MO, WT::AT[l_][i], d[l_]);
            a[i][j] = acc;
        }
    }
#pragma unroll
    for (int i = 0; i < TS; ++i)
#pragma unroll
        for (int j = 0; j < TS; ++j) {
            f32x4 acc = z;
            WINO_DOT(acc, MO, WT::AT[l_][j], a[i][l_]);
            *(f32x4*)(dM + ((long)(TS * i + j) * T + t) * K + k4 * 4) = acc;
        }
}

template <int MO>
__global__ __launch_bounds__(256) void wino_dfilter_kernel(const float* __restrict__ dU, float* __restrict__ dw, int K, int C) {
    using WT = Wino<MO>;
    constexpr int TS = WT::TS;
    const long idx = (long)blockIdx.x * 256 + threadIdx.x;
    if (idx >= (long)K * C) return;
    const int c = (int)(idx % C);
    const int k = (int)(idx / C);
    const long KC = (long)K * C;
    float r[3][TS];
#pragma unroll
    for (int j = 0; j < TS; ++j) {
        float u[TS];
#pragma unroll
        for (int i = 0; i < TS; ++i) u[i] = dU[(long)(TS * i + j) * KC + (long)k * C + c];
#pragma unroll
        for (int i = 0; i < 3; ++i) {
            float acc = 0.f;
            WINO_DOT(acc, TS, WT::G[l_][i], u[l_]);
            r[i][j] = acc;
        }
    }
#pragma unroll
    for (int i = 0; i < 3; ++i)
#pragma unroll
        for (int j = 0; j < 3; ++j) {
            float acc = 0.f;
            WINO_DOT(acc, TS, WT::G[l_][j], r[i][l_]);
            dw[(((long)k * 3 + i) * 3 + j) * C + c] = acc;
        }
}

struct WinoDims {
    int TS, NX, TH, TW;
    long T;
    size_t nU, nV, nM;
};

int wino_dims(int mo, int N, int H, int W, int C, int K, WinoDims* d) {
    DENET_CHECK_ARG(mo == 2 || mo == 4, "conv_wino: output tile must be 2 or 4 (got %d)", mo);
    DENET_CHECK_ARG(H > 0 && W > 0 && C % 32 == 0 && K % 32 == 0, "conv_wino: the channel counts must be multiples of 32");
    d->TS = mo + 2;
    d->NX = d->TS * d->TS;
    d->TH = (H + mo - 1) / mo;
    d->TW = (W + mo - 1) / mo;
    d->T = (long)N * d->TH * d->TW;
    d->nU = (size_t)d->NX * C * K;
    d->nV = (size_t)d->NX * d->T * C;
    d->nM = (size_t)d->NX * d->T * K;
    DENET_CHECK_ARG(d->T < (1L << 31) / d->NX, "conv_wino: too many tiles");
    return DENET_OK;
}

#define WINO_LAUNCH(MO_, KERNEL, NTHREADS, ...)                                                                       \
    {                                                                                                               \
        const unsigned blocks_ = (unsigned)(((NTHREADS) + 255) / 256);                                              \
        if ((MO_) == 2) hipLaunchKernelGGL(KERNEL<2>, dim3(blocks_), dim3(256), 0, stream, __VA_ARGS__);             \
        else hipLaunchKernelGGL(KERNEL<4>, dim3(blocks_), dim3(256), 0, stream, __VA_ARGS__);                        \
    }

int wino_filter(int mo, bool dgrad, const float* w, float* U, int K, int C, hipStream_t stream) {
    const unsigned fb = (unsigned)(((long)K * C + 255) / 256);
    if (dgrad && K % 16 == 0 && C % 16 == 0) {
        if (mo == 2) hipLaunchKernelGGL(wino_filter_dgrad_kernel<2>, dim3(C / 16, K / 16), dim3(256), 0, stream, w, U, K, C);
        else hipLaunchKernelGGL(wino_filter_dgrad_kernel<4>, dim3(C / 16, K / 16), dim3(256), 0, stream, w, U, K, C);
    } else if (dgrad) {
        if (mo == 2) hipLaunchKernelGGL((wino_filter_kernel<2, true>), dim3(fb), dim3(256), 0, stream, w, U, K, C);
        else hipLaunchKernelGGL((wino_filter_kernel<4, true>), dim3(fb), dim3(256), 0, stream, w, U, K, C);
    } else {
        if (mo == 2) hipLaunchKernelGGL((wino_filter_kernel<2, false>), dim3(fb), dim3(256), 0, stream, w, U, K, C);
        else hipLaunchKernelGGL((wino_filter_kernel<4, false>), dim3(fb), dim3(256), 0, stream, w, U, K, C);
    }
    DENET_CHECK_LAUNCH("conv_wino filter transform");
    return DENET_OK;
}

int wino_run(int mo, bool dgrad, const float* in, const float* w, const float* u_cached, float* v_keep, const float* bias,
             const float* add, float* out, float* ws, size_t ws_bytes, int N, int H, int W, int Cin, int Cout,
             hipStream_t stream, int relu = 0, double* stats = nullptr, const BnFoldDev* fold = nullptr, float* dm_out = nullptr,
             hipEvent_t transform_done = nullptr, const BnFoldDev* out_sums = nullptr, int in_up = 0) {
    DENET_CHECK_ARG((in || fold) && w && out && ws, "conv_wino: null pointer");
    WinoDims d;
    int rc = wino_dims(mo, N, H, W, Cin, Cout, &d);
    if (rc) return rc;
    DENET_CHECK_ARG(ws_bytes >= (d.nU + d.nV + d.nM) * sizeof(float), "conv_wino: workspace too small (%zu < %zu)",
                    ws_bytes, (d.nU + d.nV + d.nM) * sizeof(float));
    float* Uw = ws;
    float* V = v_keep ? v_keep : Uw + d.nU;
    float* Mx = Uw + d.nU + d.nV;
    const long kc = (long)Cin * Cout;
    const float* U = u_cached;
    if (!U) {
        rc = dgrad ? wino_filter(mo, true, w, Uw, Cin, Cout, stream) : wino_filter(mo, false, w, Uw, Cout, Cin, stream);
        if (rc) return rc;
        U = Uw;
    }
    static const int prep_lds = [] { const char* e = getenv("DENET_PREP_LDS"); return e ? atoi(e) : 1; }();
    if (fold && prep_lds && Cin % 32 == 0 && (long)N * ((d.TH + 3) / 4) * ((d.TW + 3) / 4) < 0x7FFFFFFFL) {
        DENET_CHECK_ARG(!dgrad || dm_out, "conv_wino: the backward fold needs the dM buffer");
        if (dgrad) rc = mo == 2 ? launch_prep_lds<2, true>(*fold, V, dm_out, N, H, W, Cin, d.TH, d.TW, d.T, stream)
                                : launch_prep_lds<4, true>(*fold, V, dm_out, N, H, W, Cin, d.TH, d.TW, d.T, stream);
        else rc = mo == 2 ? launch_prep_lds<2, false>(*fold, V, nullptr, N, H, W, Cin, d.TH, d.TW, d.T, stream)
                          : launch_prep_lds<4, false>(*fold, V, nullptr, N, H, W, Cin, d.TH, d.TW, d.T, stream);
        if (rc) return rc;
    } else if (fold) {
        const unsigned blocks = (unsigned)((d.T * (Cin / 4) + 255) / 256);
        if (dgrad) {
            DENET_CHECK_ARG(dm_out, "conv_wino: the backward fold needs the dM buffer");
            if (mo == 2) hipLaunchKernelGGL((wino_prep_kernel<2, true>), dim3(blocks), dim3(256), 0, stream, *fold, V, dm_out, N, H, W, Cin, d.TH, d.TW, d.T);
            else hipLaunchKernelGGL((wino_prep_kernel<4, true>), dim3(blocks), dim3(256), 0, stream, *fold, V, dm_out, N, H, W, Cin, d.TH, d.TW, d.T);
        } else {
            if (mo == 2) hipLaunchKernelGGL((wino_prep_kernel<2, false>), dim3(blocks), dim3(256), 0, stream, *fold, V, (float*)nullptr, N, H, W, Cin, d.TH, d.TW, d.T);
            else hipLaunchKernelGGL((wino_prep_kernel<4, false>), dim3(blocks), dim3(256), 0, stream, *fold, V, (float*)nullptr, N, H, W, Cin, d.TH, d.TW, d.T);
        }
    } else {
        WINO_LAUNCH(mo, wino_input_kernel, d.T * (Cin / 4), in, V, N, H, W, Cin, d.TH, d.TW, d.T, in_up);
    }
    DENET_CHECK_LAUNCH("conv_wino transforms");
    if (transform_done) {
        const hipError_t e = hipEventRecord(transform_done, stream);
        if (e != hipSuccess) {
            denet_set_error("conv_wino: hipEventRecord: %s", hipGetErrorString(e));
            return -(int)e;
        }
    }
    BnFoldDev bs = {};
    if (out_sums && stats) bs = *out_sums;
    if (const int tb4 = (H % mo == 0 && W % mo == 0) ? denet_wino4f_block(mo, d.T, Cin, Cout) : 0)
        return denet_wino4f_run(tb4, V, U, bias, add, out, stats, bs.x, bs.y, bs.gamma, bs.beta, bs.mean, bs.invstd, bs.relu, N, H, W,
                                Cin, Cout, relu, stream);
    rc = denet_gemm_batched_nt(V, U, Mx, d.NX, (int)d.T, Cout, Cin, d.T * Cin, kc, d.T * Cout, stream);
    if (rc) return rc;
    WINO_LAUNCH(mo, wino_output_kernel, d.T * (Cout / 4), Mx, bias, add, out, N, H, W, Cout, d.TH, d.TW, d.T, relu, stats, bs);
    DENET_CHECK_LAUNCH("conv_wino output");
    return DENET_OK;
}

int wino_stats_rows(int tile, int N, int H, int W, int Cin, int Kout, size_t stats_bytes) {
    const long T = (long)N * ((H + tile - 1) / tile) * ((W + tile - 1) / tile);
    long rows;
    if (const int tb4 = (H % tile == 0 && W % tile == 0) ? denet_wino4f_block(tile, T, Cin, Kout) : 0) rows = denet_wino4f_stats_rows(tb4, T);
    else {
        const int k4n = Kout / 4;
        if (!(k4n > 0 && k4n <= 256 && 256 % k4n == 0)) return 0;
        rows = (T * k4n + 255) / 256;
    }
    return stats_bytes >= (size_t)rows * 2 * Kout * sizeof(double) ? (int)rows : 0;
}

}

static int wino_wgrad_run(const float* x, const float* dy, const float* dm_ready, const float* v_cached, float* dw,
                          float* workspace, size_t workspace_bytes, float* split_ws, size_t split_ws_bytes, int tile, int N,
                          int H, int W, int C, int K, hipStream_t stream) {
    DENET_CHECK_ARG((x || v_cached) && (dy || dm_ready) && dw && workspace, "conv_wino_wgrad: null pointer");
    WinoDims d;
    int rc = wino_dims(tile, N, H, W, C, K, &d);
    if (rc) return rc;
    DENET_CHECK_ARG(workspace_bytes >= (d.nU + d.nV + d.nM) * sizeof(float), "conv_wino_wgrad: workspace too small");
    float* dU = workspace;
    const float* V = v_cached;
    float* dM = dU + d.nU + d.nV;
    if (!V) {
        float* Vw = dU + d.nU;
        WINO_LAUNCH(tile, wino_input_kernel, d.T * (C / 4), x, Vw, N, H, W, C, d.TH, d.TW, d.T, 0);
        V = Vw;
    }
    const float* dMr = dm_ready;
    if (!dMr) {
        WINO_LAUNCH(tile, wino_dout_kernel, d.T * (K / 4), dy, dM, N, H, W, K, d.TH, d.TW, d.T);
        dMr = dM;
    }
    DENET_CHECK_LAUNCH("conv_wino_wgrad transforms");
    const int sp = denet_wino4g_splits(tile, d.T, C, K);
    if (sp && (sp == 1 || (split_ws && split_ws_bytes >= denet_wino4g_workspace_bytes(sp, C, K))))
        rc = denet_wino4g_run(sp, dMr, V, dU, split_ws, split_ws_bytes, d.T, C, K, stream);
    else
        rc = denet_wgrad_batched(V, dMr, dU, split_ws, split_ws_bytes, d.NX, (int)d.T, C, K, stream);
    if (rc) return rc;
    WINO_LAUNCH(tile, wino_dfilter_kernel, (long)K * C, dU, dw, K, C);
    DENET_CHECK_LAUNCH("conv_wino_wgrad filter");
    return DENET_OK;
}

extern "C" int denet_conv_wino_wgrad(const float* x, const float* dy, const float* v_cached, float* dw, float* workspace,
                                     size_t workspace_bytes, float* split_ws, size_t split_ws_bytes, int tile, int N, int H,
                                     int W, int C, int K, hipStream_t stream) {
    DENET_CHECK_ARG(x && dy, "conv_wino_wgrad: null pointer");
    return wino_wgrad_run(x, dy, nullptr, v_cached, dw, workspace, workspace_bytes, split_ws, split_ws_bytes, tile, N, H, W, C, K,
                          stream);
}

extern "C" int denet_conv_wino_wgrad_dm(const float* x, const float* dm, const float* v_cached, float* dw, float* workspace,
                                        size_t workspace_bytes, float* split_ws, size_t split_ws_bytes, int tile, int N, int H,
                                        int W, int C, int K, hipStream_t stream) {
    DENET_CHECK_ARG(dm, "conv_wino_wgrad_dm: null pointer");
    return wino_wgrad_run(x, nullptr, dm, v_cached, dw, workspace, workspace_bytes, split_ws, split_ws_bytes, tile, N, H, W, C, K,
                          stream);
}

static int fold_from(const denet_bn_link* bn, bool bwd, BnFoldDev* f) {
    DENET_CHECK_ARG(bn && bn->x && bn->gamma && bn->mean && bn->invstd, "conv_wino fold: null pointer");
    DENET_CHECK_ARG(bwd ? (bn->aux && bn->coef && (!bn->relu || bn->y || bn->beta)) : (bn->beta && bn->out),
                    "conv_wino fold: incomplete batch-norm description");
    f->x = bn->x; f->aux = bn->aux; f->y = bn->y; f->gamma = bn->gamma; f->beta = bn->beta; f->mean = bn->mean;
    f->invstd = bn->invstd; f->coef = bn->coef; f->out = bn->out; f->relu = bn->relu;
    return DENET_OK;
}

extern "C" int denet_conv_wino_fwd_fold(const denet_bn_link* bn, const float* w, const float* u_cached, float* v_keep,
                                        const float* bias, const float* add, float* y, int relu, double* stats_partial,
                                        size_t stats_bytes, int* stats_rows, float* workspace, size_t workspace_bytes, int tile,
                                        int N, int H, int W, int C, int K, hipStream_t stream) {
    BnFoldDev f;
    int rc = fold_from(bn, false, &f);
    if (rc) return rc;
    double* st = nullptr;
    if (stats_partial) {
        DENET_CHECK_ARG(stats_rows && !relu, "conv_wino_fwd_fold: bad statistics arguments");
        *stats_rows = wino_stats_rows(tile, N, H, W, C, K, stats_bytes);
        st = *stats_rows ? stats_partial : nullptr;
    }
    return wino_run(tile, false, nullptr, w, u_cached, v_keep, bias, add, y, workspace, workspace_bytes, N, H, W, C, K, stream,
                    relu ? 1 : 0, st, &f);
}

static int sums_request(const denet_bn_link* sums_of, double* stats_partial, size_t stats_bytes, int* stats_rows, int tile, int N,
                        int H, int W, int C, int K, BnFoldDev* bs, double** st) {
    *st = nullptr;
    if (!sums_of) return DENET_OK;
    DENET_CHECK_ARG(stats_partial && stats_rows, "conv_wino dgrad: the backward sums need a buffer");
    DENET_CHECK_ARG(sums_of->x && sums_of->mean && sums_of->invstd && (!sums_of->relu || sums_of->y || (sums_of->gamma && sums_of->beta)),
                    "conv_wino dgrad: incomplete batch-norm description for the backward sums");
    *stats_rows = wino_stats_rows(tile, N, H, W, K, C, stats_bytes);
    if (*stats_rows) {
        *bs = BnFoldDev{};
        bs->x = sums_of->x; bs->y = sums_of->relu ? sums_of->y : nullptr; bs->gamma = sums_of->gamma; bs->beta = sums_of->beta;
        bs->mean = sums_of->mean; bs->invstd = sums_of->invstd; bs->relu = sums_of->relu;
        *st = stats_partial;
    }
    return DENET_OK;
}

extern "C" int denet_conv_wino_dgrad_fold(const denet_bn_link* bn, float* dm_out, const float* w, const float* u_cached,
                                          const float* add, float* dx, const denet_bn_link* sums_of, double* stats_partial,
                                          size_t stats_bytes, int* stats_rows, float* workspace, size_t workspace_bytes, int tile,
                                          int N, int H, int W, int C, int K, void* transform_done_event, hipStream_t stream) {
    BnFoldDev f, bs;
    double* st;
    int rc = fold_from(bn, true, &f);
    if (rc) return rc;
    rc = sums_request(sums_of, stats_partial, stats_bytes, stats_rows, tile, N, H, W, C, K, &bs, &st);
    if (rc) return rc;
    return wino_run(tile, true, nullptr, w, u_cached, nullptr, nullptr, add, dx, workspace, workspace_bytes, N, H, W, K, C, stream,
                    0, st, &f, dm_out, (hipEvent_t)transform_done_event, st ? &bs : nullptr);
}

extern "C" int denet_conv_wino_dgrad_sums(const float* dy, const float* w, const float* u_cached, const float* add, float* dx,
                                          const denet_bn_link* sums_of, double* stats_partial, size_t stats_bytes, int* stats_rows,
                                          float* workspace, size_t workspace_bytes, int tile, int N, int H, int W, int C, int K,
                                          hipStream_t stream) {
    BnFoldDev bs;
    double* st;
    int rc = sums_request(sums_of, stats_partial, stats_bytes, stats_rows, tile, N, H, W, C, K, &bs, &st);
    if (rc) return rc;
    return wino_run(tile, true, dy, w, u_cached, nullptr, nullptr, add, dx, workspace, workspace_bytes, N, H, W, K, C, stream, 0, st,
                    nullptr, nullptr, nullptr, st ? &bs : nullptr);
}

extern "C" int denet_conv_wino_tune(float* workspace, size_t workspace_bytes, float* split_ws, size_t split_ws_bytes,
                                    int tile, int N, int H, int W, int C, int K, hipStream_t stream) {
    DENET_CHECK_ARG(workspace, "conv_wino_tune: null workspace");
    WinoDims d;
    int rc = wino_dims(tile, N, H, W, C, K, &d);
    if (rc) return rc;
    DENET_CHECK_ARG(workspace_bytes >= (d.nU + d.nV + d.nM) * sizeof(float), "conv_wino_tune: workspace too small");
    float* U = workspace;
    (void)hipMemsetAsync(U, 0, (d.nU + d.nV + d.nM) * sizeof(float), stream);
    const long T = d.T;
    rc = denet_gemm_batched_tune(U + d.nU, U, U + d.nU + d.nV, d.NX, (int)T, K, C, T * C, (long)C * K, T * K, stream);
    if (rc) return rc;
    rc = denet_gemm_batched_tune(U + d.nU + d.nV, U, U + d.nU, d.NX, (int)T, C, K, T * K, (long)C * K, T * C, stream);
    if (rc || !split_ws) return rc;
    return denet_wgrad_batched_tune(U + d.nU, U + d.nU + d.nV, U, split_ws, split_ws_bytes, d.NX, (int)T, C, K, stream);
}

extern "C" size_t denet_conv_wino_workspace_bytes(int tile, int N, int H, int W, int C, int K) {
    const size_t nx = (size_t)(tile + 2) * (tile + 2);
    const size_t T = (size_t)N * ((H + tile - 1) / tile) * ((W + tile - 1) / tile);
    return (nx * C * K + nx * T * C + nx * T * K) * sizeof(float);
}

extern "C" int denet_conv_wino_fwd(const float* x, const float* w, const float* u_cached, float* v_keep, const float* bias,
                                   const float* add, float* y, float* workspace, size_t workspace_bytes, int tile, int N,
                                   int H, int W, int C, int K, hipStream_t stream) {
    return wino_run(tile, false, x, w, u_cached, v_keep, bias, add, y, workspace, workspace_bytes, N, H, W, C, K, stream);
}

extern "C" int denet_conv_wino_fwd_act(const float* x, const float* w, const float* u_cached, float* v_keep,
                                       const float* bias, const float* add, float* y, int relu, float* workspace,
                                       size_t workspace_bytes, int tile, int N, int H, int W, int C, int K,
                                       hipStream_t stream) {
    return wino_run(tile, false, x, w, u_cached, v_keep, bias, add, y, workspace, workspace_bytes, N, H, W, C, K, stream,
                    relu ? 1 : 0);
}

extern "C" int denet_conv_wino_fwd_stats_up(const float* x_small, const float* w, const float* u_cached, float* v_keep,
                                            const float* bias, const float* add, float* y, double* stats_partial,
                                            size_t stats_bytes, int* stats_rows, float* workspace, size_t workspace_bytes,
                                            int tile, int N, int H, int W, int C, int K, hipStream_t stream) {
    DENET_CHECK_ARG((tile == 2 || tile == 4) && H % 2 == 0 && W % 2 == 0, "conv_wino_fwd_stats_up: bad arguments");
    double* st = nullptr;
    if (stats_partial) {
        DENET_CHECK_ARG(stats_rows, "conv_wino_fwd_stats_up: null pointer");
        *stats_rows = wino_stats_rows(tile, N, H, W, C, K, stats_bytes);
        st = *stats_rows ? stats_partial : nullptr;
    }
    return wino_run(tile, false, x_small, w, u_cached, v_keep, bias, add, y, workspace, workspace_bytes, N, H, W, C, K, stream, 0, st,
                    nullptr, nullptr, nullptr, nullptr, 1);
}

extern "C" int denet_conv_wino_fwd_stats(const float* x, const float* w, const float* u_cached, float* v_keep,
                                         const float* bias, const float* add, float* y, double* stats_partial,
                                         size_t stats_bytes, int* stats_rows, float* workspace, size_t workspace_bytes,
                                         int tile, int N, int H, int W, int C, int K, hipStream_t stream) {
    DENET_CHECK_ARG(stats_partial && stats_rows && (tile == 2 || tile == 4), "conv_wino_fwd_stats: bad arguments");
    *stats_rows = wino_stats_rows(tile, N, H, W, C, K, stats_bytes);
    return wino_run(tile, false, x, w, u_cached, v_keep, bias, add, y, workspace, workspace_bytes, N, H, W, C, K, stream, 0,
                    *stats_rows ? stats_partial : nullptr);
}

extern "C" int denet_conv_wino_filter(const float* w, float* u, int tile, int dgrad, int C, int K, hipStream_t stream) {
    DENET_CHECK_ARG(w && u && (tile == 2 || tile == 4) && C > 0 && K > 0, "conv_wino_filter: bad arguments");
    return wino_filter(tile, dgrad != 0, w, u, K, C, stream);
}

extern "C" int denet_conv_wino_dgrad(const float* dy, const float* w, const float* u_cached, const float* add, float* dx,
                                     float* workspace, size_t workspace_bytes, int tile, int N, int H, int W, int C, int K,
                                     hipStream_t stream) {
    return wino_run(tile, true, dy, w, u_cached, nullptr, nullptr, add, dx, workspace, workspace_bytes, N, H, W, K, C, stream);
}
```

denet_amd/lib.py:

```python
import ctypes
import os

_HERE = os.path.dirname(os.path.abspath(__file__))
LIB_PATH = os.path.join(_HERE, "csrc", "libdenet_hip.so")

P = ctypes.c_void_p
I = ctypes.c_int
L = ctypes.c_long
F = ctypes.c_float
Z = ctypes.c_size_t
U64 = ctypes.c_uint64
D = ctypes.c_double

SIGNATURES = {
    "denet_last_error": (ctypes.c_char_p, []),
    "denet_abi_version": (I, []),
    "denet_device_info": (I, [I, P, P, P, I]),
    "denet_host_py_random_sample": (I, [P, P, I, I, P, P]),
    "denet_host_edit_samples": (I, [P, P, P, P, I, I, I, P, P, I, P, P, P, P]),
    "denet_host_mt_prefetch": (I, [P, P, L, P, P, P, I, P]),
    "denet_host_edit_samples_stream": (I, [P, L, P, P, P, P, I, I, I, P, P, I, P, P, P, P]),
    "denet_host_handoff_stream": (I, [P, L, P, P, P, P, P, I, I, I, I, I, P, P, I, P, P, P, P, P]),
    "denet_host_handoff_boxes_stream": (I, [P, L, P, P, P, P, I, I, I, I, I, P, P, I, P, P]),
    "denet_host_handoff_boxes_stream_u": (I, [P, L, P, P, P, P, I, I, I, I, I, P, P, I, P, P, P]),
    "denet_host_mt_uniforms": (I, [P, L, P]),
    "denet_host_detect_targets": (I, [P, P, P, P, I, I, I, I, I, I, ctypes.c_double, ctypes.c_double, P, P, P, P]),
    "denet_conv_fwd": (I, [P, P, P, P, P] + [I] * 12 + [P]),
    "denet_conv_fwd_act": (I, [P, P, P, P, P] + [I] * 13 + [P]),
    "denet_spin": (I, [I, P]),
    "denet_tune_export": (I, [P, I]),
    "denet_tune_import": (I, [P, I]),
    "denet_tune_clear": (I, []),
    "denet_conv_fwd_stats": (I, [P, P, P, P, P, P, Z, P] + [I] * 12 + [P]),
    "denet_conv_dgrad": (I, [P, P, P, P] + [I] * 12 + [P]),
    "denet_conv_rect_fwd": (I, [P] * 5 + [I] * 15 + [P]),
    "denet_conv_rect_dgrad": (I, [P] * 4 + [I] * 14 + [P]),
    "denet_conv_rect_wgrad_workspace_bytes": (Z, [I] * 7),
    "denet_conv_rect_wgrad": (I, [P] * 4 + [Z] + [I] * 14 + [P]),
    "denet_conv_wgrad_workspace_bytes": (Z, [I] * 7),
    "denet_conv_wino_workspace_bytes": (Z, [I] * 6),
    "denet_conv_wino_tune": (I, [P, Z, P, Z] + [I] * 6 + [P]),
    "denet_conv_wino_wgrad": (I, [P, P, P, P, P, Z, P, Z] + [I] * 6 + [P]),
    "denet_conv_wino_filter": (I, [P, P, I, I, I, I, P]),
    "denet_conv_wino_fwd": (I, [P] * 8 + [Z] + [I] * 6 + [P]),
    "denet_conv_wino_fwd_act": (I, [P] * 7 + [I, P, Z] + [I] * 6 + [P]),
    "denet_conv_wino_fwd_stats": (I, [P] * 8 + [Z, P, P, Z] + [I] * 6 + [P]),
    "denet_conv_wino_fwd_stats_up": (I, [P] * 8 + [Z, P, P, Z] + [I] * 6 + [P]),
    "denet_conv_wino_dgrad": (I, [P] * 6 + [Z] + [I] * 6 + [P]),
    "denet_gemm_bf16x3_ok": (I, [I] * 3),
    "denet_gemm_bf16x3_nt": (I, [P] * 4 + [I] * 3 + [P]),
    "denet_transpose_f32": (I, [P, P, I, I, P]),
    "denet_conv_wino2f_ok": (I, [I] * 5),
    "denet_conv_wino2f": (I, [P] * 5 + [I, P, Z, P] + [I] * 5 + [P]),
    "denet_conv_wino2f_wgrad_ok": (I, [I] * 5),
    "denet_conv_wino2f_wgrad_workspace_bytes": (Z, [I] * 3),
    "denet_conv_wino2f_wgrad": (I, [P] * 4 + [Z] + [I] * 5 + [P]),
    "denet_conv_stem_ok": (I, [I] * 13),
    "denet_conv_stem_fwd": (I, [P] * 5 + [Z, P] + [I] * 3 + [P]),
    "denet_conv_stem_fwd_from": (I, [P, I] + [P] * 4 + [Z, P] + [I] * 3 + [P]),
    "denet_conv_stem_wgrad_from": (I, [P, I] + [P] * 3 + [Z] + [I] * 3 + [P]),
    "denet_conv_stem_fwd_act": (I, [P, I] + [P] * 3 + [I, P, Z, P] + [I] * 3 + [P]),
    "denet_conv_stem_wgrad_workspace_bytes": (Z, []),
    "denet_conv_stem_wgrad": (I, [P] * 4 + [Z] + [I] * 3 + [P]),
    "denet_conv_tune": (I, [I, P, P, P, P, P, P, Z] + [I] * 12 + [P]),
    "denet_conv_tuned": (I, [I] * 11 + [P, P, P]),
    "denet_conv_last_config": (I, [P] * 5),
    "denet_conv_wino4f_mode": (I, [I]),
    "denet_conv_wino4g_mode": (I, [I]),
    "denet_conv_profile": (I, [I]),
    "denet_conv_profile_count": (I, []),
    "denet_conv_profile_read": (I, [I] + [P] * 5),
    "denet_conv_wgrad": (I, [P, P, P, P, Z] + [I] * 12 + [P]),
    "denet_bn_final_arm_stats": (I, [L, I, F, F, P, P, P, P, P, I]),
    "denet_bn_final_arm_sums": (I, [L, I, P, P, P, P, I]),
    "denet_bn_final_disarm": (I, []),
    "denet_bn_final_mode": (I, [I]),
    "denet_bn_workspace_bytes": (Z, [L, I]),
    "denet_bn_fwd_train": (I, [P] * 10 + [L, I, F, F, I, P]),
    "denet_bn_fwd_train_pre": (I, [P] * 10 + [I, L, I, F, F, I, P]),
    "denet_bn_relu_pool_fwd_train": (I, [P] * 10 + [I, P] + [I] * 9 + [F, F, P]),
    "denet_bn_relu_pool_bwd": (I, [P] * 11 + [I] * 9 + [P]),
    "denet_bn_relu_pool_fwd_train_xhat": (I, [P] * 11 + [I, P] + [I] * 9 + [F, F, P]),
    "denet_bn_relu_pool_bwd_sums": (I, [P] * 9 + [I] * 6 + [P]),
    "denet_bn_relu_pool_bwd_apply": (I, [P] * 9 + [I] * 9 + [P]),
    "denet_bn_fold": (I, [P] * 6 + [F, P, P, I, L, P]),
    "denet_bn_stats_final": (I, [P, I, L, I, F, F, P, P, P, P, P]),
    "denet_bn_apply": (I, [P] * 7 + [L, I, I, P]),
    "denet_bn_bwd_sums": (I, [P] * 11 + [L, I, I, P]),
    "denet_bn_bwd_apply": (I, [P] * 10 + [L, I, I, P]),
    "denet_conv_wino_fwd_fold": (I, [P] * 7 + [I, P, Z, P, P, Z] + [I] * 6 + [P]),
    "denet_conv_wino_dgrad_fold": (I, [P] * 8 + [Z, P, P, Z] + [I] * 6 + [P, P]),
    "denet_conv_wino_dgrad_sums": (I, [P] * 7 + [Z, P, P, Z] + [I] * 6 + [P]),
    "denet_conv_dgrad_sums": (I, [P] * 6 + [Z, P] + [I] * 12 + [P]),
    "denet_conv_dgrad_1x1t": (I, [P] * 6 + [Z, P] + [I] * 5 + [P]),
    "denet_conv_dgrad_t": (I, [P] * 6 + [Z, P] + [I] * 12 + [P]),
    "denet_conv_wino2f_sums": (I, [P] * 5 + [I, P, Z, P, P] + [I] * 5 + [P]),
    "denet_conv_dgrad_s2_ok": (I, [I] * 5),
    "denet_conv_dgrad_s2_stats_rows": (I, [I] * 3),
    "denet_conv_dgrad_s2_pack": (I, [P, P, I, I, P]),
    "denet_conv_dgrad_s2": (I, [P] * 6 + [Z, P] + [I] * 5 + [P]),
    "denet_conv_wino4t_ok": (I, [I] * 5),
    "denet_conv_wino4t_stats_rows": (I, [I] * 3),
    "denet_conv_wino4t_pack": (I, [P, P, I, I, P]),
    "denet_conv_wino4t_sums": (I, [P] * 5 + [I, P, Z, P, P] + [I] * 5 + [P]),
    "denet_bn_bwd_final": (I, [P, I, L, I, P, P, P, P]),
    "denet_conv_wino_wgrad_dm": (I, [P, P, P, P, P, Z, P, Z] + [I] * 6 + [P]),
    "denet_bn_fwd_test": (I, [P] * 8 + [I, L, I, F, I, P]),
    "denet_bn_moments_workspace_bytes": (Z, [L, I]),
    "denet_bn_moments_accumulate": (I, [P, P, P, Z, L, I, P]),
    "denet_bn_moments_finish": (I, [P, L, F, P, P, I, P]),
    "denet_regression_workspace_bytes": (Z, [I, I]),
    "denet_regression_loss": (I, [P] * 6 + [Z] + [I] * 5 + [P]),
    "denet_regression_probs": (I, [P] * 3 + [I] * 5 + [P]),
    "denet_bn_bwd": (I, [P] * 12 + [L, I, I, P]),
    "denet_maxpool_fwd": (I, [P, P, P] + [I] * 9 + [P]),
    "denet_maxpool_bwd": (I, [P, P, P] + [I] * 9 + [P]),
    "denet_avgpool_fwd": (I, [P, P] + [I] * 9 + [P]),
    "denet_avgpool_bwd": (I, [P, P] + [I] * 9 + [P]),
    "denet_pool_inv_fwd": (I, [P, P] + [I] * 6 + [P]),
    "denet_pool_inv_bwd": (I, [P, P] + [I] * 6 + [P]),
    "denet_maxpool_border_fwd": (I, [P, P] + [I] * 10 + [P]),
    "denet_maxpool_border_bwd": (I, [P, P, P, P] + [I] * 10 + [P]),
    "denet_avgpool_border_fwd": (I, [P, P] + [I] * 10 + [P]),
    "denet_avgpool_border_bwd": (I, [P, P] + [I] * 10 + [P]),
    "denet_host_resample_coeffs": (I, [I, D, D, I, I, P, P, L]),
    "denet_image_crop": (I, [P, P] + [I] * 9 + [P]),
    "denet_image_reduce": (I, [P, P, I, I, I, I, P]),
    "denet_image_resample_pass": (I, [P, P, I, I, I, I, P, P, I, P]),
    "denet_image_render_batch": (I, [I] + [P] * 13 + [I, I, P, P, Z, P, P, P, Z, P, P]),
    "denet_image_finish": (I, [P, P, I, I, I, I, P, P, P, P, I, P, P]),
    "denet_border_fwd": (I, [P, P] + [I] * 8 + [P]),
    "denet_border_bwd": (I, [P, P] + [I] * 8 + [P]),
    "denet_crop_mirror_fwd": (I, [P, P] + [I] * 6 + [F, F, I, U64, P]),
    "denet_crop_mirror_bwd": (I, [P, P] + [I] * 6 + [F, F, I, U64, P]),
    "denet_dropout": (I, [P, P, I, I, I, I, F, U64, P]),
    "denet_concat_fwd": (I, [P, P, P, L] + [I] * 5 + [P]),
    "denet_concat_bwd": (I, [P, P, P, L] + [I] * 5 + [P]),
    "denet_add_bias": (I, [P, P, P, L, I, P]),
    "denet_nchw_to_nhwc": (I, [P, P] + [I] * 5 + [P]),
    "denet_nhwc_to_nchw": (I, [P, P] + [I] * 5 + [P]),
    "denet_add": (I, [P, P, P, L, I, P]),
    "denet_relu_fwd": (I, [P, P, L, P]),
    "denet_relu_bwd": (I, [P, P, P, L, P]),
    "denet_act_fwd": (I, [P, P, L, I, I, I, P]),
    "denet_act_bwd": (I, [P, P, P, L, I, I, I, P]),
    "denet_add_act_fwd": (I, [P, P, P, L, I, I, I, P]),
    "denet_colsum_workspace_bytes": (Z, [L, I]),
    "denet_colsum": (I, [P, P, P, L, I, P]),
    "denet_solver_step": (I, [P, P, P, L, L, F, F, I, F, F, I, P]),
    "denet_solver_adam": (I, [P, P, P, P, L, L, F, F, F, I, F, F, P]),
    "denet_scale": (I, [P, L, F, P]),
    "denet_corner_fwd": (I, [P, P] + [I] * 5 + [P]),
    "denet_loss_workspace_bytes": (Z, []),
    "denet_corner_loss": (I, [P] * 5 + [I] * 5 + [F, P]),
    "denet_sparse_fwd": (I, [P, P, P, P] + [I] * 10 + [P]),
    "denet_sparse_sort_workspace_bytes": (Z, [I] * 5),
    "denet_sparse_sort_is_single": (I, [I] * 5),
    "denet_sparse_sort": (I, [P, P, Z] + [I] * 5 + [P]),
    "denet_sparse_bwd": (I, [P, P, P, Z, P] + [I] * 10 + [P]),
    "denet_detect_loss": (I, [P] * 9 + [I] * 6 + [F, F, F, I, P]),
    "denet_detect_decode": (I, [P] * 5 + [I] * 6 + [F, P]),
    "denet_detect_nms": (I, [P] * 5 + [I, I, I, F, F, P]),
    "denet_soft_nms_batch_host": (L, [P, P, P, P, I, I, I, F, F, P, P, P, P, L]),
    "denet_soft_nms_host": (I, [P, P, I, F, P, P, P]),
    "denet_soft_nms_workspace_bytes": (Z, [I, I, I]),
    "denet_soft_nms_batch": (I, [P, P, P, P, I, I, I, F, F, P, P, P, P, P, P, Z, P]),
    "denet_build_samples_workspace_bytes": (Z, [I] * 6),
    "denet_build_samples": (I, [P, P, P, P, P, Z] + [I] * 4 + [F, I, I, I, P]),
    "denet_build_samples_stats": (I, [P, Z] + [I] * 6 + [P, P, P]),
    "denet_edit_samples_device": (I, [P, P, I, I, P, L, L, P, P] + [I] * 4 + [P, P, P]),
    "denet_host_cluster_samples": (I, [P, I, F, I, P, P]),
    "denet_samples_finish_host": (I, [P, P, P, I, I, I, I, P]),
}


class DenetHipError(RuntimeError):
    pass


_lib = None


def load():
    global _lib
    if _lib is not None:
        return _lib
    if not os.path.exists(LIB_PATH):
        raise DenetHipError(
            "libdenet_hip.so is missing (%s): run `python -m denet_amd.build` / __graft_entry__.build() first. "
            "The DeNet hot path has no CPU fallback." % LIB_PATH)
    import torch
    lib = ctypes.CDLL(LIB_PATH)
    for name, (res, args) in SIGNATURES.items():
        fn = getattr(lib, name)
        fn.restype = res
        fn.argtypes = args
    _lib = lib
    return lib


def check(rc, what=""):
    if rc != 0:
        msg = load().denet_last_error().decode("utf-8", "replace")
        raise DenetHipError("%s failed (rc=%d): %s" % (what or "denet call", rc, msg))


def ptr(t):
    return None if t is None else t.data_ptr()


def stream_ptr():
    import torch
    return torch.cuda.current_stream().cuda_stream
```

denet_amd/ops.py:

```python
import contextlib
import os

import torch

from . import lib as _lib
from .lib import check, ptr, stream_ptr


def _L():
    return _lib.load()


def empty(*shape, dtype=torch.float32):
    return torch.empty(*shape, dtype=dtype, device="cuda")


class Workspace:

    def __init__(self):
        self.bufs = {}

    def get(self, name, nbytes):
        nbytes = int(nbytes)
        buf = self.bufs.get(name)
# ... 400 lines not shown
    T = N * -(-H // tile) * -(-W // tile)
    dm = torch.empty((tile + 2) * (tile + 2) * T * K, dtype=torch.float32, device="cuda")
    dx = empty(N, H, W, C)
    u = _cached_u(cache, 1, tile) if cache is not None else None
    ws = _wino_ws(tile, N, H, W, C, K)
    ev = cache.get("prep_event") if cache is not None else None
    if ev is None:
        ev = torch.cuda.Event()
        ev.record()
        if cache is not None:
            cache["prep_event"] = ev
    bn = link.c_struct(link.out)
    rows = ctypes.c_int(0)
    sb = sums.buffer(cache, (T * (C // 4) + 255) // 256, C) if sums is not None else None
    so = sums.c_struct() if sums is not None else None
    with _armed(sums.final if sums is not None else None) as fin:
        check(_L().denet_conv_wino_dgrad_fold(ctypes.byref(bn), ptr(dm), ptr(w), ptr(u), ptr(add), ptr(dx),
                                              ctypes.byref(so) if so is not None else None, ptr(sb), sb.numel() * 8 if sb is not None else 0,
                                              ctypes.byref(rows), ptr(ws), ws.numel(), tile, N, H, W, C, K, ev.cuda_event, stream_ptr()),
              "conv_wino_dgrad_fold")
    if sums is not None:
        sums.done(sb, rows.value, fin)
    v = None
    if cache is not None and cache.get("V_tile") == tile:
        v = cache.get("V")
        cache["V_tile"] = None
    global _ON_WGRAD_STREAM
    if WGRAD_STREAM and _WGRAD_STREAM is None:
        init_streams()
    side = _WGRAD_STREAM if (WGRAD_STREAM and (PROFILE is None or not PROFILE.alone)) else None
    if side is not None:
        side.wait_event(ev)
        dm.record_stream(side)
        with torch.cuda.stream(side):
            _ON_WGRAD_STREAM = True
            try:
                _wgrad_dm(x, dm, v, dw_out, tile, N, H, W, C, K)
            finally:
                _ON_WGRAD_STREAM = False
    else:
        _wgrad_dm(x, dm, v, dw_out, tile, N, H, W, C, K)
    LINK_COUNT[1] += 1
    return dx


def _wgrad_dm(x, dm, v, dw, tile, N, H, W, C, K):
    ws = _wino_ws(tile, N, H, W, C, K)
    sws = WS.get("wgrad", WGRAD_WS_BYTES)
    check(_L().denet_conv_wino_wgrad_dm(ptr(x), ptr(dm), ptr(v), ptr(dw), ptr(ws), ws.numel(), ptr(sws), sws.numel(), tile, N, H, W,
                                        C, K, stream_ptr()), "conv_wino_wgrad_dm")


def _bf16x3_geom(g):
    N, H, W, C, K, R, S, s_real, stride, pad, OH, OW = g
    return HEAD_BF16X3 and R == 1 and S == 1 and stride == 1 and pad == 0 and C >= 512 and C % 128 == 0 and K % 128 == 0 \
        and (N * H * W) % 32 == 0 and _full(g)


def _gemm_bf16x3(a, b, bias, out, M, N, K):
    check(_L().denet_gemm_bf16x3_nt(ptr(a), ptr(b), ptr(bias), ptr(out), M, N, K, stream_ptr()), "gemm_bf16x3_nt")
    return out


def _transpose(src, R, C, out=None):
    dst = out if out is not None else empty(C, R)
    check(_L().denet_transpose_f32(ptr(src), ptr(dst), R, C, stream_ptr()), "transpose_f32")
    return dst


def conv_fwd(x, w, bias=None, add=None, stride=1, pad=0, s_real=None, out=None, logical=None, cache=None, relu=False,
             bn_stats=False, link=None, up=None, ohw=None):
    if link is not None:
        g = conv_geom(link.x.shape, w.shape, stride, pad, s_real, ohw)
        tile = _decided(0, g)
        if not (tile in (2, 4) and cache is not None and cache.get("train") and not relu and not _bf16x3_geom(g)):
            x = link.materialise()
            link = None
    if link is not None:
        if PROFILE is not None:
            PROFILE.add(_conv_flops(g, logical) / _WINO_GAIN[tile])
        return _conv_wino_fwd_linked(link, g, tile, w, bias, add, out, cache, bn_stats)
    if up is not None:
        gu = conv_geom(up.shape, w.shape, stride, pad, s_real, ohw)
        if not (_decided(0, gu) in (2, 4) and ((0, gu) in _TUNED or not AUTOTUNE or not MEASURE or POLICY is not None) and cache is not None and cache.get("train") and bn_stats
                and not relu and not _bf16x3_geom(gu)):
            x = up.materialise()
            up = None
    g = conv_geom(up.shape if up is not None else x.shape, w.shape, stride, pad, s_real, ohw)
    N, H, W, C, K, R, S, s_real, stride, pad, OH, OW = g
    y = out if out is not None else empty(N, OH, OW, K)
    if add is None and not relu and _bf16x3_geom(g):
        if cache is not None:
            _note_fwd_tile(cache, 0)
            cache["bn_stats"] = None
        return _gemm_bf16x3(x, w, bias, y, N * H * W, K, C)
    _tune_first(0, g, x, w, bias, add, y, None)
    st = None
    if bn_stats and cache is not None and not relu:
        rows = max((N * OH * OW + 127) // 128, (N * (OH // 2 + 1) * (OW // 2 + 1) * (K // 4) + 255) // 256,
                   N * ((OH + 15) // 16) * ((OW + 15) // 16), N * ((OH + 7) // 8) * ((OW + 31) // 32))
        st = cache.get("bn_stats_buf")
        if st is None or st.numel() < rows * 2 * K:
            st = cache["bn_stats_buf"] = torch.empty(rows * 2 * K, dtype=torch.float64, device="cuda")
        cache["bn_stats"] = None

    def direct(final=False):
        if final and st is not None:
            import ctypes
            rows = ctypes.c_int(0)
            with _armed(cache.get("bn_final")) as fin:
                check(_L().denet_conv_fwd_stats(ptr(x), ptr(w), ptr(bias), ptr(add), ptr(y), ptr(st), st.numel() * 8,
                                                ctypes.byref(rows), *g, stream_ptr()), "conv_fwd_stats")
            cache["bn_stats"] = _stats_result(st, rows.value, fin)
            return
        check(_L().denet_conv_fwd_act(ptr(x), ptr(w), ptr(bias), ptr(add), ptr(y), int(relu), *g, stream_ptr()), "conv_fwd")

    tile = _wino_tile(0, g, direct, lambda t: conv_wino_fwd(x, w, bias, add, out=y, tile=t, relu=relu))
    if cache is not None and not cache.get("train") and (3, g) in _WINO and _tile_allowed(3, _WINO[(3, g)]):
        t3 = _WINO[(3, g)]
        if (t3 == FUSED4 and conv_wino4t_ok(0, g)) or (t3 in (2, 4) and conv_wino_ok(g, t3)) or t3 == 0:
            tile = t3
    if tile:
        if PROFILE is not None:
            PROFILE.add(_conv_flops(g, logical) / _WINO_GAIN[tile])
        u = v_keep = None
        if cache is not None:
            _note_fwd_tile(cache, tile)
            u = _cached_u(cache, 0, tile) if cache.get("train") else None
            if u is None and not cache.get("train"):
                ent = cache.get("u_test")
                if ent is None or ent[0] != tile or ent[2] != WEIGHTS_VERSION or ent[3] != w.data_ptr():
                    uf = conv_wino4t_filter(w, dgrad=False) if tile == FUSED4 else conv_wino_filter(w, _filter_tile(tile), dgrad=False)
                    ent = cache["u_test"] = (tile, uf, WEIGHTS_VERSION, w.data_ptr())
                u = ent[1]
            if cache.get("train") and _decided(2, g) == tile:
                v_keep = cache.get("V")
                nv = (tile + 2) * (tile + 2) * (N * -(-H // tile) * -(-W // tile)) * C
                if v_keep is None or v_keep.numel() != nv:
                    v_keep = cache["V"] = torch.empty(nv, dtype=torch.float32, device="cuda")
                cache["V_tile"] = tile
        if up is not None and st is None:
            x, up = up.materialise(), None
        return conv_wino_fwd(x, w, bias, add, out=y, tile=tile, u=u, v_keep=v_keep, relu=relu, stats=(st, cache) if st is not None else None,
                             up=up)
    assert up is None
    if cache is not None:
        _note_fwd_tile(cache, 0)
    if PROFILE is not None:
        PROFILE.add(_conv_flops(g, logical))
    direct(final=True)
    return y


WINOGRAD = int(os.environ.get("DENET_WINOGRAD", "4"))
WINO_RAGGED = os.environ.get("DENET_WINO_RAGGED", "1") != "0"
_WINO = {}
FUSED2 = 22
WINO2F = int(os.environ.get("DENET_WINO2F", "7"))
FUSED4 = 44
WINO4T = int(os.environ.get("DENET_WINO4T", "3"))
_WINO_GAIN = {2: 2.25, 4: 4.0, FUSED2: 2.25, FUSED4: 4.0}


POLICY = None


def static_policy(mode, g):
    if _tile_allowed(mode, FUSED2) and conv_wino2f_ok(mode, g):
        return FUSED2
    for t in (4, 2):
        if t <= WINOGRAD and conv_wino_ok(g, t):
            return t
    return 0


def _decided(mode, g):
    _load_tuned_once()
    use = _WINO.get((mode, g))
    if use is None:
        policy = POLICY if POLICY is not None else (static_policy if AUTOTUNE and not MEASURE else None)
        if policy is not None:
            use = _WINO[(mode, g)] = int(policy(mode, g))
    return use


def _tile_allowed(mode, tile):
    if tile == FUSED2:
        return WINOGRAD >= 2 and mode in (0, 1, 2) and bool((WINO2F >> mode) & 1)
    if tile == FUSED4:
        return WINOGRAD >= 4 and mode in (0, 1, 3) and bool((WINO4T >> (1 if mode == 1 else 0)) & 1)
    return tile <= WINOGRAD


def _filter_tile(tile):
    return 2 if tile == FUSED2 else (4 if tile == FUSED4 else tile)


def conv_wino4t_ok(mode, g):
    N, H, W, C, K, R, S, s_real, stride, pad, OH, OW = g
    if not (mode in (0, 1) and R == 3 and S == 3 and s_real == 3 and stride == 1 and pad == 1 and _full(g)):
        return False
    red, out = (C, K) if mode == 0 else (K, C)
    return bool(_L().denet_conv_wino4t_ok(N, H, W, red, out))


def conv_wino2f_ok(mode, g):
    N, H, W, C, K, R, S, s_real, stride, pad, OH, OW = g
    if not (R == 3 and S == 3 and s_real == 3 and stride == 1 and pad == 1 and _full(g)):
        return False
    if mode == 2:
        return bool(_L().denet_conv_wino2f_wgrad_ok(N, H, W, C, K))
    ci, co = (C, K) if mode == 0 else (K, C)
    return bool(_L().denet_conv_wino2f_ok(N, H, W, ci, co))


def _time_ms(fn, reps=3):
    fn()
    best = 1e30
    for _ in range(reps):
        s, e = torch.cuda.Event(enable_timing=True), torch.cuda.Event(enable_timing=True)
        s.record()
        fn()
        e.record()
        e.synchronize()
        best = min(best, s.elapsed_time(e))
    return best


def conv_wino_ok(g, tile=2):
    N, H, W, C, K, R, S, s_real, stride, pad, OH, OW = g
    return R == 3 and S == 3 and s_real == 3 and stride == 1 and pad == 1 and (WINO_RAGGED or (H % tile == 0 and W % tile == 0)) \
        and H >= tile and W >= tile and C % 32 == 0 and K % 32 == 0 and _full(g)


def _wino_tile(mode, g, direct, wino):
    key = (mode, g)
    use = _decided(mode, g)
    if use is None:
        tiles = [t for t in (2, 4) if t <= WINOGRAD and conv_wino_ok(g, t)] if AUTOTUNE else []
        if AUTOTUNE and _tile_allowed(mode, FUSED2) and conv_wino2f_ok(mode, g):
            tiles.append(FUSED2)
        if AUTOTUNE and _tile_allowed(mode, FUSED4) and conv_wino4t_ok(mode, g) and (g[3] if mode == 0 else g[4]) == 64:
            tiles.append(FUSED4)
        if not tiles:
            use = 0
        elif PROFILE is not None:
            return 0
        else:
            N, H, W, C, K = g[0], g[1], g[2], g[3], g[4]
            sws = WS.get("wgrad", WGRAD_WS_BYTES)
            best, use = 0.97 * _time_ms(direct), 0
            for t in tiles:
                if t not in (FUSED2, FUSED4):
                    ws = WS.get("wino", _L().denet_conv_wino_workspace_bytes(t, N, H, W, C, K))
                    check(_L().denet_conv_wino_tune(ptr(ws), ws.numel(), ptr(sws), sws.numel(), t, N, H, W, C, K, stream_ptr()),
                          "conv_wino_tune")
                ms = _time_ms(lambda: wino(t))
                if ms < best:
                    best, use = ms, t
        _WINO[key] = use
    return use


def _note_fwd_tile(cache, tile):
    cache["fwd_tile"] = tile
    if cache.get("train"):
        cache["fwd_tile_train"] = tile


def _cached_u(cache, dgrad, tile):
    ent = cache.get(("u", dgrad))
    if ent is None or ent[0] != tile or not ent[2] or ent[3] != WEIGHTS_VERSION:
        return None
    wait_upload(cache.get(("u_event", dgrad)))
    ent[2] = False
    return ent[1]


def _cached_ws2(cache):
    ent = cache.get("ws2") if cache is not None else None
    if ent is None or not ent[1]:
        return None
    wait_upload(cache.get("ws2_event"))
    ent[1] = False
    return ent[0]


def conv_dgrad_s2_pack(w, out=None):
    K, _, _, C = w.shape
    pk = out if out is not None else empty(9 * K * C)
    check(_L().denet_conv_dgrad_s2_pack(ptr(w), ptr(pk), C, K, stream_ptr()), "conv_dgrad_s2_pack")
    return pk


def _cached_wt(cache):
    ent = cache.get("wt") if cache is not None else None
    if ent is None or not ent[1]:
        return None
    wait_upload(cache.get("wt_event"))
    ent[1] = False
    return ent[0]


def wino_prefetch_filters(caches_and_weights, after=None):
    global _SIDE_FILTER
    todo = [(c, w) for c, w in caches_and_weights if c.get("fwd_tile_train") or c.get("dgrad_tile")]
    tr = [(c, w) for c, w in caches_and_weights if c.get("dgrad_1x1t") or c.get("dgrad_t")]
    s2 = [(c, w) for c, w in caches_and_weights if c.get("dgrad_s2")]
    if not todo and not tr and not s2:
        return
    if _SIDE_FILTER is None:
        init_streams()
    if after is not None:
        _SIDE_FILTER.wait_event(after)
    else:
        _SIDE_FILTER.wait_stream(torch.cuda.current_stream())
    with torch.cuda.stream(_SIDE_FILTER):
        def run(items, dgrad, key):
            for c, w in items:
                tile = c.get(key)
                if not tile:
                    continue
                ent = c.get(("u", dgrad))
                ft = _filter_tile(tile)
                if ent is None or ent[0] != tile:
                    K, _, _, C = w.shape
                    ent = c[("u", dgrad)] = [tile, torch.empty((ft + 2) * (ft + 2) * K * C, dtype=torch.float32, device="cuda"), False,
                                             None]
                if tile == FUSED4:
                    conv_wino4t_filter(w, dgrad, out=ent[1])
                else:
                    conv_wino_filter(w, ft, dgrad, out=ent[1])
                ent[2] = True
                ent[3] = WEIGHTS_VERSION
            ev = torch.cuda.Event()
            ev.record(_SIDE_FILTER)
            for c, _ in items:
                c[("u_event", dgrad)] = ev
        for i in range(0, len(todo), 8):
            run(todo[i:i + 8], 0, "fwd_tile_train")
        run(todo, 1, "dgrad_tile")
        if tr:
            for c, w in tr:
                K = w.shape[0]
                C = w.numel() // K
                ent = c.get("wt")
                if ent is None or ent[0].numel() != K * C:
                    ent = c["wt"] = [torch.empty(C, K, dtype=torch.float32, device="cuda"), False]
                _transpose(w, K, C, out=ent[0])
                ent[1] = True
            ev = torch.cuda.Event()
            ev.record(_SIDE_FILTER)
            for c, _ in tr:
                c["wt_event"] = ev
        if s2:
            for c, w in s2:
                ent = c.get("ws2")
                if ent is None or ent[0].numel() != w.numel():
                    ent = c["ws2"] = [torch.empty(w.numel(), dtype=torch.float32, device="cuda"), False]
                conv_dgrad_s2_pack(w, out=ent[0])
                ent[1] = True
            ev = torch.cuda.Event()
            ev.record(_SIDE_FILTER)
            for c, _ in s2:
                c["ws2_event"] = ev


_SIDE_FILTER = None


_WGRAD_STREAM = None
_ON_WGRAD_STREAM = False
WGRAD_STREAM = os.environ.get("DENET_WGRAD_STREAM", "1") != "0"
DGRAD_FIRST_GFLOP = float(os.environ.get("DENET_DGRAD_FIRST_GFLOP", "100"))
DGRAD_1X1T_GFLOP = float(os.environ.get("DENET_DGRAD_1X1T_GFLOP", "100"))
DGRAD_T = os.environ.get("DENET_DGRAD_T", "0") != "0"
DGRAD_S2 = os.environ.get("DENET_DGRAD_S2", "1") != "0"


class wgrad_stream:

    def __enter__(self):
        global _WGRAD_STREAM, _ON_WGRAD_STREAM
        self.active = WGRAD_STREAM and (PROFILE is None or not PROFILE.alone)
        if not self.active:
            return self
        if _WGRAD_STREAM is None:
            init_streams()
        _WGRAD_STREAM.wait_stream(torch.cuda.current_stream())
        self.ctx = torch.cuda.stream(_WGRAD_STREAM)
        self.ctx.__enter__()
        _ON_WGRAD_STREAM = True
        return self

    def __exit__(self, *a):
        global _ON_WGRAD_STREAM
        if self.active:
            _ON_WGRAD_STREAM = False
            self.ctx.__exit__(*a)
        return False


def join_wgrad_stream():
    if _WGRAD_STREAM is not None:
        torch.cuda.current_stream().wait_stream(_WGRAD_STREAM)


def _wino_ws(tile, N, H, W, C, K):
    return WS.get("wino_side" if _ON_WGRAD_STREAM else "wino", _L().denet_conv_wino_workspace_bytes(tile, N, H, W, C, K))


def conv_wino_fwd(x, w, bias=None, add=None, out=None, tile=2, u=None, v_keep=None, relu=False, stats=None, up=None):
    N, H, W, C = up.shape if up is not None else x.shape
    K = w.shape[0]
    y = out if out is not None else empty(N, H, W, K)
    if tile == FUSED2:
        import ctypes
        if u is None:
            u = conv_wino_filter(w, 2, dgrad=False)
        st, cache = stats if stats is not None and not relu else (None, None)
        rows = ctypes.c_int(0)
        with _armed(cache.get("bn_final") if st is not None else None) as fin:
            check(_L().denet_conv_wino2f(ptr(x), ptr(u), ptr(bias), ptr(add), ptr(y), int(relu), ptr(st), st.numel() * 8 if st is not None
                                         else 0, ctypes.byref(rows), N, H, W, C, K, stream_ptr()), "conv_wino2f")
        if st is not None:
            cache["bn_stats"] = _stats_result(st, rows.value, fin)
        return y
    if tile == FUSED4:
        import ctypes
        if u is None:
            u = conv_wino4t_filter(w, dgrad=False)
        st, cache = stats if stats is not None and not relu else (None, None)
        rows = ctypes.c_int(0)
        check(_L().denet_conv_wino4t_sums(ptr(x), ptr(u), ptr(bias), ptr(add), ptr(y), int(relu), ptr(st), st.numel() * 8 if st is not None
                                          else 0, ctypes.byref(rows), None, N, H, W, C, K, stream_ptr()), "conv_wino4t")
        if st is not None:
            cache["bn_stats"] = _stats_result(st, rows.value, None)
        return y
    ws = _wino_ws(tile, N, H, W, C, K)
    if stats is not None and not relu:
        import ctypes
        st, cache = stats
        rows = ctypes.c_int(0)
        fn = _L().denet_conv_wino_fwd_stats_up if up is not None else _L().denet_conv_wino_fwd_stats
        with _armed(cache.get("bn_final")) as fin:
            check(fn(ptr(up.src if up is not None else x), ptr(w), ptr(u), ptr(v_keep), ptr(bias), ptr(add), ptr(y), ptr(st),
                     st.numel() * 8, ctypes.byref(rows), ptr(ws), ws.numel(), tile, N, H, W, C, K, stream_ptr()), "conv_wino_fwd_stats")
        cache["bn_stats"] = _stats_result(st, rows.value, fin)
        return y
    assert up is None, "an up-sampled input is only read by the statistics form"
    check(_L().denet_conv_wino_fwd_act(ptr(x), ptr(w), ptr(u), ptr(v_keep), ptr(bias), ptr(add), ptr(y), int(relu), ptr(ws),
                                       ws.numel(), tile, N, H, W, C, K, stream_ptr()), "conv_wino_fwd")
    return y


def conv_wino_dgrad(dy, w, add=None, out=None, tile=2, u=None, sums=None, cache=None):
    import ctypes
    N, H, W, K = dy.shape
    C = w.shape[3]
    dx = out if out is not None else empty(N, H, W, C)
    rows = ctypes.c_int(0)
    so = sums.c_struct() if sums is not None else None
    if tile == FUSED2:
        if u is None:
            u = conv_wino_filter(w, 2, dgrad=True)
        sb = sums.buffer(cache, N * ((H + 15) // 16) * ((W + 15) // 16), C) if sums is not None else None
        with _armed(sums.final if sums is not None else None) as fin:
            check(_L().denet_conv_wino2f_sums(ptr(dy), ptr(u), None, ptr(add), ptr(dx), 0, ptr(sb), sb.numel() * 8 if sb is not None else 0,
                                              ctypes.byref(rows), ctypes.byref(so) if so is not None else None, N, H, W, K, C,
                                              stream_ptr()), "conv_wino2f")
        if sums is not None:
            sums.done(sb, rows.value, fin)
        return dx
    if tile == FUSED4:
        if u is None:
            u = conv_wino4t_filter(w, dgrad=True)
        sb = sums.buffer(cache, _L().denet_conv_wino4t_stats_rows(N, H, W), C) if sums is not None else None
        check(_L().denet_conv_wino4t_sums(ptr(dy), ptr(u), None, ptr(add), ptr(dx), 0, ptr(sb), sb.numel() * 8 if sb is not None else 0,
                                          ctypes.byref(rows), ctypes.byref(so) if so is not None else None, N, H, W, K, C,
                                          stream_ptr()), "conv_wino4t")
        if sums is not None:
            sums.done(sb, rows.value, None)
        return dx
    ws = _wino_ws(tile, N, H, W, C, K)
    if sums is not None:
        T = N * -(-H // tile) * -(-W // tile)
        sb = sums.buffer(cache, (T * (C // 4) + 255) // 256, C)
        with _armed(sums.final) as fin:
            check(_L().denet_conv_wino_dgrad_sums(ptr(dy), ptr(w), ptr(u), ptr(add), ptr(dx), ctypes.byref(so), ptr(sb), sb.numel() * 8,
                                                  ctypes.byref(rows), ptr(ws), ws.numel(), tile, N, H, W, C, K, stream_ptr()),
                  "conv_wino_dgrad_sums")
        sums.done(sb, rows.value, fin)
        return dx
    check(_L().denet_conv_wino_dgrad(ptr(dy), ptr(w), ptr(u), ptr(add), ptr(dx), ptr(ws), ws.numel(), tile, N, H, W, C, K,
                                     stream_ptr()), "conv_wino_dgrad")
    return dx


def conv_wino_wgrad(x, dy, out=None, tile=2, v=None):
    N, H, W, C = x.shape
    K = dy.shape[3]
    dw = out if out is not None else empty(K, 3, 3, C)
    if tile == FUSED2:
        ws = WS.get("wino2f_side" if _ON_WGRAD_STREAM else "wino2f", _L().denet_conv_wino2f_wgrad_workspace_bytes(N, H, W))
        check(_L().denet_conv_wino2f_wgrad(ptr(x), ptr(dy), ptr(dw), ptr(ws), ws.numel(), N, H, W, C, K, stream_ptr()),
              "conv_wino2f_wgrad")
        return dw
    ws = _wino_ws(tile, N, H, W, C, K)
    sws = WS.get("wgrad", WGRAD_WS_BYTES)
    check(_L().denet_conv_wino_wgrad(ptr(x), ptr(dy), ptr(v), ptr(dw), ptr(ws), ws.numel(), ptr(sws), sws.numel(), tile, N, H,
                                     W, C, K, stream_ptr()), "conv_wino_wgrad")
    return dw


def conv_wino_filter(w, tile, dgrad, out=None):
    K, _, _, C = w.shape
    nx = (tile + 2) * (tile + 2)
    u = out if out is not None else empty(nx, K, C)
    check(_L().denet_conv_wino_filter(ptr(w), ptr(u), tile, int(dgrad), C, K, stream_ptr()), "conv_wino_filter")
    return u


def conv_wino4t_filter(w, dgrad, out=None):
    K, _, _, C = w.shape
    u = WS.get("w4t_filter_%x" % torch.cuda.current_stream().cuda_stream, 36 * K * C * 4)[:36 * K * C * 4].view(torch.float32)
    conv_wino_filter(w, 4, dgrad, out=u)
    pk = out if out is not None else empty(36 * K * C)
    red, outc = (K, C) if dgrad else (C, K)
    check(_L().denet_conv_wino4t_pack(ptr(u), ptr(pk), red, outc, stream_ptr()), "conv_wino4t_pack")
    return pk


def conv_dgrad(dy, w, x_shape, add=None, stride=1, pad=0, s_real=None, out=None, logical=None, cache=None, sums=None, ohw=None):
    g = conv_geom(x_shape, w.shape, stride, pad, s_real, ohw)
    assert tuple(dy.shape) == (g[0], g[10], g[11], g[4]), (dy.shape, g)
    dx = out if out is not None else empty(*x_shape)
    if add is None and _bf16x3_geom(g):
        N, H, W, C, K = g[0], g[1], g[2], g[3], g[4]
        if cache is not None:
            cache["dgrad_tile"] = 0
        return _gemm_bf16x3(dy, _transpose(w, K, C), None, dx, N * H * W, C, K)
    if DGRAD_1X1T_GFLOP > 0 and g[5] == 1 and g[6] == 1 and g[8] == 1 and g[9] == 0 and g[3] % 32 == 0 and g[4] % 32 == 0 \
            and 2e-9 * dy.numel() * g[3] >= DGRAD_1X1T_GFLOP and _full(g):
        import ctypes
        N, H, W, C, K = g[0], g[1], g[2], g[3], g[4]
        wt = _cached_wt(cache)
        if wt is None:
            wt = _transpose(w, K, C)
        if cache is not None:
            cache["dgrad_tile"] = 0
            cache["dgrad_1x1t"] = True
        gt = conv_geom((N, H, W, K), (C, 1, 1, K), 1, 0, None)
        if not _tune_first(0, gt, dy, wt, None, add, dx, None) and PROFILE is not None:
            PROFILE.add(_conv_flops(g, logical))
        rows = ctypes.c_int(0)
        sb = so = None
        if sums is not None and (int(BWD_SUMS) & 2):
            sb = sums.buffer(cache, (N * H * W + 127) // 128, C)
            so = sums.c_struct()
        with _armed(sums.final if sb is not None else None) as fin:
            check(_L().denet_conv_dgrad_1x1t(ptr(dy), ptr(wt), ptr(add), ptr(dx), ctypes.byref(so) if so is not None else None, ptr(sb),
                                             sb.numel() * 8 if sb is not None else 0, ctypes.byref(rows), N, H, W, C, K, stream_ptr()),
                  "conv_dgrad_1x1t")
        if sb is not None:
            sums.done(sb, rows.value, fin)
        return dx
    if DGRAD_S2 and g[5] == 3 and g[6] == 3 and g[7] == 3 and g[8] == 2 and g[9] == 1 and _full(g) and \
            _L().denet_conv_dgrad_s2_ok(g[0], g[1], g[2], g[3], g[4]):
        import ctypes
        N, H, W, C, K = g[0], g[1], g[2], g[3], g[4]
        wp = _cached_ws2(cache)
        if wp is None:
            wp = conv_dgrad_s2_pack(w)
        if cache is not None:
            cache["dgrad_tile"] = 0
            cache["dgrad_s2"] = True
        if PROFILE is not None:
            PROFILE.add(_conv_flops(g, logical))
        rows = ctypes.c_int(0)
        sb = so = None
        if sums is not None and (int(BWD_SUMS) & 2):
            sb = sums.buffer(cache, _L().denet_conv_dgrad_s2_stats_rows(N, H, W), C)
            so = sums.c_struct()
        check(_L().denet_conv_dgrad_s2(ptr(dy), ptr(wp), ptr(add), ptr(dx), ctypes.byref(so) if so is not None else None, ptr(sb),
                                       sb.numel() * 8 if sb is not None else 0, ctypes.byref(rows), N, H, W, C, K, stream_ptr()),
              "conv_dgrad_s2")
        if sb is not None:
            sums.done(sb, rows.value, None)
        return dx
    _tune_first(1, g, dy, w, None, add, dx, None)

    def direct():
        check(_L().denet_conv_dgrad(ptr(dy), ptr(w), ptr(add), ptr(dx), *g, stream_ptr()), "conv_dgrad")

    tile = _wino_tile(1, g, direct, lambda t: conv_wino_dgrad(dy, w, add, out=dx, tile=t))
    if tile:
        if PROFILE is not None:
            PROFILE.add(_conv_flops(g, logical) / _WINO_GAIN[tile])
        u = None
        if cache is not None:
            cache["dgrad_tile"] = tile
            u = _cached_u(cache, 1, tile)
        return conv_wino_dgrad(dy, w, add, out=dx, tile=tile, u=u, sums=sums if (int(BWD_SUMS) & 1) else None, cache=cache)
    if cache is not None:
        cache["dgrad_tile"] = 0
    if PROFILE is not None:
        PROFILE.add(_conv_flops(g, logical))
    if DGRAD_T and g[3] % 32 == 0 and g[4] % 32 == 0:
        import ctypes
        N, H, W, C, K = g[0], g[1], g[2], g[3], g[4]
        wt = _cached_wt(cache)
        if wt is None:
            wt = _transpose(w, K, w.numel() // K)
        if cache is not None:
            cache["dgrad_t"] = True
        rows = ctypes.c_int(0)
        sb = so = None
        if sums is not None and (int(BWD_SUMS) & 2) and g[1] % g[8] == 0 and g[2] % g[8] == 0:
            sb = sums.buffer(cache, (N * H * W + 127) // 128 + g[8] * g[8], C)
            so = sums.c_struct()
        with _armed(sums.final if sb is not None else None) as fin:
            check(_L().denet_conv_dgrad_t(ptr(dy), ptr(wt), ptr(add), ptr(dx), ctypes.byref(so) if so is not None else None, ptr(sb),
                                          sb.numel() * 8 if sb is not None else 0, ctypes.byref(rows), *g, stream_ptr()), "conv_dgrad_t")
        if sb is not None:
            sums.done(sb, rows.value, fin)
        return dx
    if sums is not None and (int(BWD_SUMS) & 2) and g[1] % g[8] == 0 and g[2] % g[8] == 0:
        import ctypes
        N, H, W, C = g[0], g[1], g[2], g[3]
        rows = ctypes.c_int(0)
        sb = sums.buffer(cache, (N * H * W + 127) // 128 + g[8] * g[8], C)
        so = sums.c_struct()
        with _armed(sums.final) as fin:
            check(_L().denet_conv_dgrad_sums(ptr(dy), ptr(w), ptr(add), ptr(dx), ctypes.byref(so), ptr(sb), sb.numel() * 8,
                                             ctypes.byref(rows), *g, stream_ptr()), "conv_dgrad_sums")
        sums.done(sb, rows.value, fin)
        return dx
    direct()
    return dx


def conv_wgrad(x, dy, w_shape, stride=1, pad=0, s_real=None, out=None, logical=None, cache=None, ohw=None):
    g = conv_geom(x.shape, w_shape, stride, pad, s_real, ohw)
    assert tuple(dy.shape) == (g[0], g[10], g[11], g[4]), (dy.shape, g)
    dw = out if out is not None else empty(*w_shape)
    if _bf16x3_geom(g):
        N, H, W, C, K = g[0], g[1], g[2], g[3], g[4]
        M = N * H * W
        return _gemm_bf16x3(_transpose(dy, M, K), _transpose(x, M, C), None, dw, K, C, M)
    ws = WS.get("wgrad", WGRAD_WS_BYTES)
    _tune_first(2, g, x, dy, None, None, dw, ws)

    def direct():
        check(_L().denet_conv_wgrad(ptr(x), ptr(dy), ptr(dw), ptr(ws), ws.numel(), *g, stream_ptr()), "conv_wgrad")

    tile = _wino_tile(2, g, direct, lambda t: conv_wino_wgrad(x, dy, out=dw, tile=t))
    if tile:
        if PROFILE is not None:
            PROFILE.add(_conv_flops(g, logical) / _WINO_GAIN[tile])
        v = None
        if cache is not None and cache.get("V_tile") == tile:
            v = cache.get("V")
            cache["V_tile"] = None
        return conv_wino_wgrad(x, dy, out=dw, tile=tile, v=v)
    if PROFILE is not None:
        PROFILE.add(_conv_flops(g, logical))
    direct()
    return dw
# ... 842 lines not shown
```

denet_amd/switches.py:

```python

SWITCHES = {
    "DENET_AUTOTUNE": ("1", "kernels", "use the committed decisions and the Winograd / fused algorithms (0: launch heuristics, direct kernels only)"),
    "DENET_TUNE": ("0", "kernels", "1: MEASURE the launch configuration / algorithm of geometries the tuned file does not cover on their first call (what tools/tune.py does); 0, the product default: such a geometry runs ops.static_policy, nothing is ever timed, every process runs the same kernels"),
    "DENET_TUNE_CACHE": ("denet_amd/tuned/gfx950.json", "kernels", "the committed measured decisions (0: ignore the file)"),
    "DENET_WINOGRAD": ("4", "kernels", "largest Winograd tile allowed for the 3x3 stride-1 layers (0: direct only, 2: F(2x2) only)"),
    "DENET_WINO_RAGGED": ("1", "kernels", "Winograd on maps that are no multiple of the tile (ceil tiles; 0: multiples only)"),
    "DENET_WINO2F": ("7", "kernels", "fused F(2x2) kernels of the 64-channel layers: bit 0 forward, 1 data gradient, 2 filter gradient"),
    "DENET_DGRAD_S2": ("1", "kernels", "3x3 stride-2 data gradients: the four parity classes in one workgroup (csrc/dgrad_s2.hip; 0: implicit GEMM per class)"),
    "DENET_WINO4T": ("3", "kernels", "tile-parallel fully fused F(4x4) kernel (csrc/wino4t.hip) where the tuned file names it: bit 0 forward (training and the inference entries, mode 3), 1 data gradient"),
    "DENET_W4T_LDS": ("0", "kernels", "experiment: LDS bytes a wino4t workgroup requests (100000: one workgroup per CU)"),
    "DENET_WINO4F": ("1", "kernels", "fused F(4x4) product + output-transform kernel (0: un-fused component GEMMs + transform)"),
    "DENET_WINO4F_TB": ("0", "kernels", "force a shape of the fused F(4x4) kernel (32 / 33 / 34 / 64; 0: the occupancy policy)"),
    "DENET_WINO4G": ("1", "kernels", "dedicated F(4x4) filter-gradient kernel (0: the generic batched split-K products)"),
    "DENET_STEM": ("3", "kernels", "the first layer's own kernels: bit 0 forward, bit 1 filter gradient (0: generic implicit GEMM)"),
    "DENET_HEAD_BF16X3": ("0", "kernels", "OPT-IN, never the headline: head GEMMs as 3-term bf16 splits on the bf16 matrix cores"),
    "DENET_DGRAD_FIRST_GFLOP": ("100", "kernels", "a layer whose data-gradient GEMM is at least this large runs it before its filter gradient is queued"),
    "DENET_DGRAD_1X1T_GFLOP": ("100", "kernels", "1x1 stride-1 data gradients at least this large run as forward products over the transposed filter (0: never)"),
    "DENET_DGRAD_T": ("0", "kernels", "OPT-IN (no faster): the other implicit-GEMM data gradients over the transposed filter (igemm mode 3)"),
    "DENET_DGRAD_T_NBUF": ("0", "kernels", "experiment: loop structure of igemm mode 3"),
    "DENET_DGRAD_T_TILE": ("0", "kernels", "experiment: tile of igemm mode 3"),
    "DENET_IGEMM_NBUF": ("0", "kernels", "experiment: force the LDS buffering of the implicit-GEMM kernels"),
    "DENET_IGEMM_TILE": ("0", "kernels", "experiment: force the implicit-GEMM tile"),
    "DENET_WGRAD_BLOCKS": ("0", "kernels", "experiment: force the split-K workgroup count of the filter gradient"),
    "DENET_WGRAD_SPLIT_SLOW": ("1", "kernels", "filter gradient: the split slice is the slow (XCD-local) workgroup index"),
    "DENET_BN_LINK": ("1", "kernels", "batch-norm pointwise passes evaluated inside the Winograd transforms next to them"),
    "DENET_BN_BWD_SUMS": ("3", "kernels", "backward reductions written by the data-gradient pass: bit 0 Winograd passes, bit 1 direct passes"),
    "DENET_BN_FINAL_FOLD": ("0", "kernels", "OPT-IN (slower): the reductions' second stage inside the producing launch: bit 0 forward, bit 1 backward"),
    "DENET_BN_POOL_FUSE": ("1", "kernels", "the stem's BN + ReLU + max pool as one pass each way"),
    "DENET_BN_ACT_FUSE": ("1", "kernels", "`BN A` layer pairs run as the fused BN + ReLU"),
    "DENET_POOL_QUAD": ("1", "kernels", "the stem's backward pointwise pass on 2x2 pixel quads"),
    "DENET_PREP_LDS": ("1", "kernels", "the linked transforms stage their block through LDS (0: one thread per tile)"),
    "DENET_SKIP_FUSE": ("1", "kernels", "SKIP additions in the epilogue of the convolution in front"),
    "DENET_UP_LINK": ("1", "kernels", "the pool-inverse layer read inside the next convolution's input transform"),
    "DENET_INFER_FOLD": ("1", "kernels", "inference: batch norm folded into the convolution in front of it"),
    "DENET_WGRAD_STREAM": ("1", "kernels", "the filter-gradient chain of the backward sweep on a second stream"),
    "DENET_SHORT_HANDOFF": ("1", "host", "the short forms of the RoI hand-off (device-side editing / one native call)"),
    "DENET_HANDOFF_WARM_MS": ("0.25", "host", "milliseconds between dry runs of the hand-off's native call while the host waits for the proposal (0: none)"),
    "DENET_SIDE_SORT": ("1", "kernels", "the gather gradient's tap sort queued right behind the forward gather"),
    "DENET_SORT_ONE_KERNEL": ("1", "kernels", "the tap sort as one 1024-thread workgroup per image"),
    "DENET_SOFT_NMS_HOST": ("unset", "host", "inference: force the host (1) / device (0) form of Gaussian soft-NMS"),
    "DENET_FORCE_DP": ("unset", "driver", "run the data-parallel collectives at world size 1 (single-GPU exercise of the RCCL path)"),
    "DENET_BENCH_SHARE_GPU": ("unset", "driver", "bench.py --share-gpu: all ranks on cuda:0 over gloo (launch-path debug mode)"),
    "DENET_BUILD_JOBS": ("cpu count", "build", "parallel hipcc processes of denet_amd/build.py"),
    "DENET_TORCH_THREADS": ("unset", "driver", "torch CPU thread count set when the package is imported"),
    "DENET_TEST_PRESSURE": ("unset", "tests", "every GPU test starts beside a saturated memory system (tests/conftest.py)"),
}


def active():
    import os
    return {k: v for k, v in sorted(os.environ.items()) if k.startswith("DENET_")}


def changes_kernels(env=None):
    env = active() if env is None else env
    return [k for k in env if SWITCHES.get(k, (None, "kernels"))[1] in ("kernels", "host")]
```

include/denet_hip.h:

```cpp
#ifndef DENET_HIP_H
#define DENET_HIP_H

#include <stddef.h>
#include <stdint.h>

#ifdef __cplusplus
extern "C" {
#endif

typedef struct ihipStream_t* hipStream_t;

#define DENET_ERR_ARG (-1000)
#define DENET_TAP_THEANO 0
#define DENET_TAP_CUDA 1
#define DENET_ACT_SIGMOID 1
#define DENET_ACT_TANH 2
#define DENET_ACT_ELU 3
#define DENET_ACT_SOFTPLUS 4
#define DENET_SOLVER_SGD 0
#define DENET_SOLVER_NESTEROV 1

const char* denet_last_error(void);
int denet_abi_version(void);
int denet_device_info(int device, int* cu_count, int* clock_khz, char* arch, int arch_len);

int denet_host_py_random_sample(unsigned* mt_host, int* pos_host, int n, int k, int* pool_ws_host, int* out_host);
int denet_host_edit_samples(unsigned* mt_host, int* pos_host, const float* det_host, const int* count_host, int B, int S,
                            int n_keep, const double* gt_host, const int* gt_off_host, int sample_gt, int* ws_host,
                            double* out_pr_host, double* out_box_host, float* out_box_f32_host);
int denet_host_mt_prefetch(unsigned* mt_host, int* pos_host, long n, unsigned* out_host, unsigned* snaps_host,
                           long* snap_first_host, int max_snaps, int* n_snaps_host);
int denet_host_edit_samples_stream(const unsigned* stream_host, long n_stream, long* cursor_host, int* exhausted_host,
                                   const float* det_host, const int* count_host, int B, int S, int n_keep, const double* gt_host,
                                   const int* gt_off_host, int sample_gt, int* ws_host, double* out_pr_host, double* out_box_host,
                                   float* out_box_f32_host);
int denet_host_handoff_stream(const unsigned* stream_host, long n_stream, long* cursor_host, int* exhausted_host,
                              const int* box_host, const float* absd_host, const int* count_host, int H, int W, int B, int S,
                              int n_keep, const double* gt_host, const int* gt_off_host, int sample_gt, int* ws_host,
                              float* det_out_host, double* out_pr_host, double* out_box_host, float* out_box_f32_host);
int denet_host_handoff_boxes_stream(const unsigned* stream_host, long n_stream, long* cursor_host, int* exhausted_host,
                                    const int* box_host, const int* count_host, int H, int W, int B, int S, int n_keep,
                                    const double* gt_host, const int* gt_off_host, int sample_gt, int* ws_host, float* out_box_f32_host);
int denet_host_handoff_boxes_stream_u(const unsigned* stream_host, long n_stream, long* cursor_host, int* exhausted_host,
                                      const int* box_host, const int* count_host, int H, int W, int B, int S, int n_keep,
                                      const double* gt_host, const int* gt_off_host, int sample_gt, int* ws_host, float* out_box_f32_host,
                                      const double* uniforms_host);
int denet_host_mt_uniforms(const unsigned* stream_host, long n, double* uniforms_host);
int denet_host_detect_targets(const double* gt_host, const int* gt_off_host, const int* gt_class_host,
                              const double* roi_host, int B, int S, int s0, int null_class, int fitness_num,
                              int jointfit, double t0, double t1, float* det_host, float* valid_host, float* reg_host,
                              float* indfit_host );

int denet_conv_fwd(const float* x, const float* w, const float* bias, const float* add, float* y, int N, int H, int W,
                   int C, int K, int R, int S, int S_real, int stride, int pad, int OH, int OW, hipStream_t stream);
int denet_conv_fwd_act(const float* x, const float* w, const float* bias, const float* add, float* y, int relu, int N, int H,
                       int W, int C, int K, int R, int S, int S_real, int stride, int pad, int OH, int OW,
                       hipStream_t stream);
int denet_conv_fwd_stats(const float* x, const float* w, const float* bias, const float* add, float* y,
                         double* stats_partial, size_t stats_bytes, int* stats_rows, int N, int H, int W, int C, int K,
                         int R, int S, int S_real, int stride, int pad, int OH, int OW, hipStream_t stream);
int denet_conv_dgrad(const float* dy, const float* w, const float* add, float* dx, int N, int H, int W, int C, int K,
                     int R, int S, int S_real, int stride, int pad, int OH, int OW, hipStream_t stream);
size_t denet_conv_wgrad_workspace_bytes(int N, int C, int K, int R, int S, int OH, int OW);
size_t denet_conv_wino_workspace_bytes(int tile, int N, int H, int W, int C, int K);
int denet_conv_wino_tune(float* workspace, size_t workspace_bytes, float* split_ws, size_t split_ws_bytes, int tile, int N,
                         int H, int W, int C, int K, hipStream_t stream);
int denet_conv_wino_filter(const float* w, float* u, int tile, int dgrad, int C, int K, hipStream_t stream);
int denet_conv_wino_fwd(const float* x, const float* w, const float* u_cached, float* v_keep, const float* bias,
                        const float* add, float* y, float* workspace, size_t workspace_bytes, int tile, int N, int H, int W,
                        int C, int K, hipStream_t stream);
int denet_conv_wino_fwd_act(const float* x, const float* w, const float* u_cached, float* v_keep, const float* bias,
                            const float* add, float* y, int relu, float* workspace, size_t workspace_bytes, int tile, int N,
                            int H, int W, int C, int K, hipStream_t stream);
int denet_conv_wino_fwd_stats(const float* x, const float* w, const float* u_cached, float* v_keep, const float* bias,
                              const float* add, float* y, double* stats_partial, size_t stats_bytes, int* stats_rows,
                              float* workspace, size_t workspace_bytes, int tile, int N, int H, int W, int C, int K,
                              hipStream_t stream);
int denet_conv_wino_fwd_stats_up(const float* x_small, const float* w, const float* u_cached, float* v_keep, const float* bias,
                              const float* add, float* y, double* stats_partial, size_t stats_bytes, int* stats_rows,
                              float* workspace, size_t workspace_bytes, int tile, int N, int H, int W, int C, int K,
                              hipStream_t stream);
int denet_gemm_bf16x3_ok(int M, int N, int K);
int denet_gemm_bf16x3_nt(const float* a, const float* b, const float* bias, float* c, int M, int N, int K, hipStream_t stream);
int denet_transpose_f32(const float* src, float* dst, int R, int C, hipStream_t stream);
int denet_conv_wino2f_ok(int N, int H, int W, int Ci, int Co);
int denet_conv_wino2f(const float* x, const float* u, const float* bias, const float* add, float* y, int relu,
                      double* stats_partial, size_t stats_bytes, int* stats_rows, int N, int H, int W, int Ci, int Co,
                      hipStream_t stream);
int denet_conv_wino2f_wgrad_ok(int N, int H, int W, int C, int K);
size_t denet_conv_wino2f_wgrad_workspace_bytes(int N, int H, int W);
int denet_conv_wino2f_wgrad(const float* x, const float* dy, float* dw, void* workspace, size_t workspace_bytes, int N, int H,
                            int W, int C, int K, hipStream_t stream);
int denet_conv_stem_ok(int pass, int N, int H, int W, int C, int K, int R, int S, int S_real, int stride, int pad, int OH, int OW);
int denet_conv_stem_fwd(const float* x, const float* w, const float* bias, float* y, double* stats_partial, size_t stats_bytes,
                        int* stats_rows, int N, int H, int W, hipStream_t stream);
int denet_conv_stem_fwd_from(const float* x, int x_nchw, const float* w, const float* bias, float* y, double* stats_partial,
                             size_t stats_bytes, int* stats_rows, int N, int H, int W, hipStream_t stream);
int denet_conv_stem_fwd_act(const float* x, int x_nchw, const float* w, const float* bias, float* y, int relu, double* stats_partial,
                            size_t stats_bytes, int* stats_rows, int N, int H, int W, hipStream_t stream);
int denet_conv_stem_wgrad_from(const float* x, int x_nchw, const float* dy, float* dw, float* workspace, size_t workspace_bytes,
                               int N, int H, int W, hipStream_t stream);
size_t denet_conv_stem_wgrad_workspace_bytes(void);
int denet_conv_stem_wgrad(const float* x, const float* dy, float* dw, float* workspace, size_t workspace_bytes, int N, int H, int W,
                          hipStream_t stream);
int denet_conv_rect_fwd(const float* x, const float* w, const float* bias, const float* add, float* y, int relu, int N, int H,
                        int W, int C, int K, int R, int S, int S_real, int sh, int sw, int ph, int pw, int OH, int OW,
                        hipStream_t stream);
int denet_conv_rect_dgrad(const float* dy, const float* w, const float* add, float* dx, int N, int H, int W, int C, int K, int R,
                          int S, int S_real, int sh, int sw, int ph, int pw, int OH, int OW, hipStream_t stream);
size_t denet_conv_rect_wgrad_workspace_bytes(int N, int C, int K, int R, int S, int OH, int OW);
int denet_conv_rect_wgrad(const float* x, const float* dy, float* dw, float* workspace, size_t workspace_bytes, int N, int H,
                          int W, int C, int K, int R, int S, int S_real, int sh, int sw, int ph, int pw, int OH, int OW,
                          hipStream_t stream);
typedef struct denet_bn_link {
    const float* x;
    const float* aux;
    const float* y;
    const float* gamma;
    const float* beta;
    const float* mean;
    const float* invstd;
    const float* coef;
    float* out;
    int relu;
} denet_bn_link;
int denet_conv_wino_fwd_fold(const denet_bn_link* bn, const float* w, const float* u_cached, float* v_keep, const float* bias,
                             const float* add, float* y, int relu, double* stats_partial, size_t stats_bytes, int* stats_rows,
                             float* workspace, size_t workspace_bytes, int tile, int N, int H, int W, int C, int K,
                             hipStream_t stream);
int denet_conv_wino_dgrad_fold(const denet_bn_link* bn, float* dm_out, const float* w, const float* u_cached, const float* add,
                               float* dx, const denet_bn_link* sums_of, double* stats_partial, size_t stats_bytes, int* stats_rows,
                               float* workspace, size_t workspace_bytes, int tile, int N, int H, int W, int C, int K,
                               void* transform_done_event, hipStream_t stream);
int denet_conv_wino_dgrad_sums(const float* dy, const float* w, const float* u_cached, const float* add, float* dx,
                               const denet_bn_link* sums_of, double* stats_partial, size_t stats_bytes, int* stats_rows,
                               float* workspace, size_t workspace_bytes, int tile, int N, int H, int W, int C, int K,
                               hipStream_t stream);
int denet_conv_dgrad_sums(const float* dy, const float* w, const float* add, float* dx, const denet_bn_link* sums_of,
                          double* stats_partial, size_t stats_bytes, int* stats_rows, int N, int H, int W, int C, int K, int R,
                          int S, int S_real, int stride, int pad, int OH, int OW, hipStream_t stream);
int denet_conv_dgrad_t(const float* dy, const float* wt, const float* add, float* dx, const denet_bn_link* sums_of,
                       double* stats_partial, size_t stats_bytes, int* stats_rows, int N, int H, int W, int C, int K, int R, int S,
                       int S_real, int stride, int pad, int OH, int OW, hipStream_t stream);
int denet_conv_dgrad_s2_ok(int N, int H, int W, int C, int K);
int denet_conv_dgrad_s2_stats_rows(int N, int H, int W);
int denet_conv_dgrad_s2_pack(const float* w, float* packed, int C, int K, hipStream_t stream);
int denet_conv_dgrad_s2(const float* dy, const float* w_packed, const float* add, float* dx, const denet_bn_link* sums_of,
                        double* stats_partial, size_t stats_bytes, int* stats_rows, int N, int H, int W, int C, int K,
                        hipStream_t stream);
int denet_conv_dgrad_1x1t(const float* dy, const float* wt, const float* add, float* dx, const denet_bn_link* sums_of,
                          double* stats_partial, size_t stats_bytes, int* stats_rows, int N, int H, int W, int C, int K,
                          hipStream_t stream);
int denet_conv_wino2f_sums(const float* x, const float* u, const float* bias, const float* add, float* y, int relu,
                           double* stats_partial, size_t stats_bytes, int* stats_rows, const denet_bn_link* sums_of, int N, int H,
                           int W, int Ci, int Co, hipStream_t stream);
int denet_conv_wino4t_ok(int N, int H, int W, int C, int K);
int denet_conv_wino4t_stats_rows(int N, int H, int W);
int denet_conv_wino4t_pack(const float* u, float* packed, int C, int K, hipStream_t stream);
int denet_conv_wino4t_sums(const float* x, const float* u_packed, const float* bias, const float* add, float* y, int relu,
                           double* stats_partial, size_t stats_bytes, int* stats_rows, const denet_bn_link* sums_of, int N, int H,
                           int W, int C, int K, hipStream_t stream);
int denet_conv_wino_wgrad_dm(const float* x, const float* dm, const float* v_cached, float* dw, float* workspace,
                             size_t workspace_bytes, float* split_ws, size_t split_ws_bytes, int tile, int N, int H, int W, int C,
                             int K, hipStream_t stream);
int denet_conv_wino_dgrad(const float* dy, const float* w, const float* u_cached, const float* add, float* dx,
                          float* workspace, size_t workspace_bytes, int tile, int N, int H, int W, int C, int K,
                          hipStream_t stream);
int denet_conv_wino_wgrad(const float* x, const float* dy, const float* v_cached, float* dw, float* workspace,
                          size_t workspace_bytes, float* split_ws, size_t split_ws_bytes, int tile, int N, int H, int W, int C,
                          int K, hipStream_t stream);
int denet_conv_tune(int mode, const float* a, const float* b, const float* bias, const float* add, float* out,
                    float* workspace, size_t workspace_bytes, int N, int H, int W, int C, int K, int R, int S, int S_real,
                    int stride, int pad, int OH, int OW, hipStream_t stream);
int denet_conv_tuned(int mode, int N, int H, int W, int C, int K, int R, int S, int S_real, int stride, int pad,
                     int* tile, int* nbuf, int* rounds);
int denet_spin(int microseconds, hipStream_t stream);
int denet_tune_export(int* records, int capacity);
int denet_tune_import(const int* records, int count);
int denet_tune_clear(void);
int denet_conv_last_config(int* mode, int* bm, int* bn, int* nbuf, int* grid_y);
int denet_conv_wino4f_mode(int mode);
int denet_conv_wino4g_mode(int mode);
int denet_conv_profile(int enable);
int denet_conv_profile_count(void);
int denet_conv_profile_read(int i, float* ms, int* mode, int* bm, int* bn, int* nbuf);
int denet_conv_wgrad(const float* x, const float* dy, float* dw, float* workspace, size_t workspace_bytes, int N,
                     int H, int W, int C, int K, int R, int S, int S_real, int stride, int pad, int OH, int OW,
                     hipStream_t stream);

int denet_bn_final_arm_stats(long M, int C, float momentum, float eps, float* run_mean, float* run_stdinv, float* save_mean,
                             float* save_invstd, unsigned* counters, int ncounters);
int denet_bn_final_arm_sums(long M, int C, float* dgamma, float* dbeta, float* coef, unsigned* counters, int ncounters);
int denet_bn_final_disarm(void);
int denet_bn_final_mode(int bits);
size_t denet_bn_workspace_bytes(long M, int C);
int denet_bn_fwd_train(const float* x, const float* res, float* y, const float* gamma, const float* beta,
                       float* run_mean, float* run_stdinv, float* save_mean, float* save_invstd, void* workspace,
                       long M, int C, float momentum, float eps, int relu, hipStream_t stream);
int denet_bn_fwd_train_pre(const float* x, const float* res, float* y, const float* gamma, const float* beta,
                           float* run_mean, float* run_stdinv, float* save_mean, float* save_invstd, const double* partial,
                           int rows, long M, int C, float momentum, float eps, int relu, hipStream_t stream);
int denet_bn_stats_final(const double* partial, int rows, long M, int C, float momentum, float eps, float* run_mean,
                         float* run_stdinv, float* save_mean, float* save_invstd, hipStream_t stream);
int denet_bn_apply(const float* x, const float* res, float* y, const float* gamma, const float* beta, const float* save_mean,
                   const float* save_invstd, long M, int C, int relu, hipStream_t stream);
int denet_bn_bwd_sums(const float* x, const float* y, const float* dy, const float* gamma, const float* beta,
                      const float* save_mean, const float* save_invstd, float* dgamma, float* dbeta, float* coef,
                      void* workspace, long M, int C, int relu, hipStream_t stream);
int denet_bn_bwd_final(const double* partial, int rows, long M, int C, float* dgamma, float* dbeta, float* coef,
                       hipStream_t stream);
int denet_bn_bwd_apply(const float* x, const float* y, const float* dy, const float* gamma, const float* beta,
                       const float* save_mean, const float* save_invstd, const float* coef, float* dx, float* dres, long M,
                       int C, int relu, hipStream_t stream);
int denet_bn_fwd_test(const float* x, const float* res, float* y, const float* gamma, const float* beta,
                      const float* run_mean, const float* run_stdinv, float* coef, int coef_ready, long M, int C, float eps,
                      int relu, hipStream_t stream);
size_t denet_bn_moments_workspace_bytes(long M, int C);
int denet_bn_moments_accumulate(const float* x, double* acc, void* workspace, size_t workspace_bytes, long M, int C,
                                hipStream_t stream);
int denet_bn_moments_finish(const double* acc, long n, float eps, float* run_mean, float* run_stdinv, int C, hipStream_t stream);
size_t denet_regression_workspace_bytes(int B, int V);
int denet_regression_loss(const float* logits, const int* offsets, const int* cls, float* dlogits, float* costs, void* workspace,
                          size_t workspace_bytes, int B, int HW, int CP, int C, int V, hipStream_t stream);
int denet_regression_probs(const float* logits, const int* offsets, float* pr, int B, int HW, int CP, int C, int V,
                           hipStream_t stream);
int denet_bn_fold(const float* w, const float* conv_bias, const float* gamma, const float* beta, const float* run_mean,
                  const float* run_stdinv, float eps, float* w_out, float* b_out, int K, long per_k, hipStream_t stream);
int denet_bn_bwd(const float* x, const float* y, const float* dy, const float* gamma, const float* beta,
                 const float* save_mean, const float* save_invstd, float* dx, float* dres, float* dgamma, float* dbeta,
                 void* workspace, long M, int C, int relu, hipStream_t stream);
int denet_bn_relu_pool_fwd_train(const float* x, float* y_pool, unsigned char* argmax, const float* gamma, const float* beta,
                                 float* run_mean, float* run_stdinv, float* save_mean, float* save_invstd, const double* partial,
                                 int rows, void* workspace, int N, int H, int W, int C, int OH, int OW, int k, int stride, int pad,
                                 float momentum, float eps, hipStream_t stream);
int denet_bn_relu_pool_bwd(const float* x, const float* dy_pool, const unsigned char* argmax, const float* gamma,
                           const float* beta, const float* save_mean, const float* save_invstd, float* dx, float* dgamma,
                           float* dbeta, void* workspace, int N, int H, int W, int C, int OH, int OW, int k, int stride, int pad,
                           hipStream_t stream);
int denet_bn_relu_pool_fwd_train_xhat(const float* x, float* y_pool, unsigned char* argmax, float* xhat_pool, const float* gamma,
                                      const float* beta, float* run_mean, float* run_stdinv, float* save_mean, float* save_invstd,
                                      const double* partial, int rows, void* workspace, int N, int H, int W, int C, int OH, int OW,
                                      int k, int stride, int pad, float momentum, float eps, hipStream_t stream);
int denet_bn_relu_pool_bwd_sums(const float* xhat_pool, const float* y_pool, const float* dy_pool, const float* zeros,
                                const float* ones, float* dgamma, float* dbeta, float* coef, void* workspace, int N, int H, int W,
                                int C, int OH, int OW, hipStream_t stream);
int denet_bn_relu_pool_bwd_apply(const float* x, const float* dy_pool, const unsigned char* argmax, const float* gamma,
                                 const float* beta, const float* save_mean, const float* save_invstd, const float* coef, float* dx,
                                 int N, int H, int W, int C, int OH, int OW, int k, int stride, int pad, hipStream_t stream);

int denet_maxpool_fwd(const float* x, float* y, unsigned char* argmax, int N, int H, int W, int C, int OH, int OW,
                      int k, int stride, int pad, hipStream_t stream);
int denet_maxpool_bwd(const float* dy, const unsigned char* argmax, float* dx, int N, int H, int W, int C, int OH,
                      int OW, int k, int stride, int pad, hipStream_t stream);
int denet_avgpool_fwd(const float* x, float* y, int N, int H, int W, int C, int OH, int OW, int k, int stride, int pad,
                      hipStream_t stream);
int denet_avgpool_bwd(const float* dy, float* dx, int N, int H, int W, int C, int OH, int OW, int k, int stride,
                      int pad, hipStream_t stream);
int denet_pool_inv_fwd(const float* x, float* y, int N, int H, int W, int C, int fy, int fx, hipStream_t stream);
int denet_pool_inv_bwd(const float* dy, float* dx, int N, int H, int W, int C, int fy, int fx, hipStream_t stream);
int denet_maxpool_border_fwd(const float* x, float* y, int N, int H, int W, int C, int OH, int OW, int kh, int kw, int sh, int sw,
                             hipStream_t stream);
int denet_maxpool_border_bwd(const float* x, const float* y, const float* dy, float* dx, int N, int H, int W, int C, int OH,
                             int OW, int kh, int kw, int sh, int sw, hipStream_t stream);
int denet_avgpool_border_fwd(const float* x, float* y, int N, int H, int W, int C, int OH, int OW, int kh, int kw, int sh, int sw,
                             hipStream_t stream);
int denet_avgpool_border_bwd(const float* dy, float* dx, int N, int H, int W, int C, int OH, int OW, int kh, int kw, int sh,
                             int sw, hipStream_t stream);

int denet_host_resample_coeffs(int in_size, double in0, double in1, int out_size, int filter, int* bounds_host,
                               int* kk_host, long kk_capacity);
int denet_image_crop(const unsigned char* src, unsigned char* dst_rgbx, int sw, int sh, int src_bpp, int px, int py, int x0,
                     int y0, int w, int h, hipStream_t stream);
int denet_image_reduce(const unsigned char* in_rgbx, unsigned char* out_rgbx, int in_w, int in_h, int fx, int fy,
                       hipStream_t stream);
int denet_image_resample_pass(const unsigned char* in_rgbx, unsigned char* out_rgbx, int in_w, int in_h, int out_n,
                              int horizontal, const int* bounds_dev, const int* kk_dev, int ksize, hipStream_t stream);
int denet_image_render_batch(int B, const unsigned char* const* src_host, const int* src_wh, const int* op_off, const int* ops,
                             const int* ops_wh, const double* ops_in1, const int* photo_n, const int* photo_ops,
                             const double* photo_alpha, const double* noise, const unsigned char* has_noise,
                             const float* mean_std, const unsigned char* mirror, int crop, int cp, float* out_dev,
                             unsigned char* pinned_host, size_t pinned_bytes, unsigned char* staging_dev,
                             unsigned char* scratch0, unsigned char* scratch1, size_t scratch_bytes,
                             unsigned long long* sums_dev, hipStream_t stream);
int denet_image_finish(const unsigned char* img_rgbx, float* out_nhwc, int w, int h, int cp, int n_ops,
                       const int* ops_host, const double* alphas_host, const double* noise_host,
                       const float* mean_std_host, int mirror, unsigned long long* sums_ws, hipStream_t stream);

int denet_border_fwd(const float* x, float* y, int N, int H, int W, int C, int left, int right, int top, int bottom,
                     hipStream_t stream);
int denet_border_bwd(const float* dy, float* dx, int N, int H, int W, int C, int left, int right, int top, int bottom,
                     hipStream_t stream);
int denet_crop_mirror_fwd(const float* x, float* y, int N, int H, int W, int C, int crop_h, int crop_w, float mirror_pr,
                          float flip_pr, int train, uint64_t seed, hipStream_t stream);
int denet_crop_mirror_bwd(const float* dy, float* dx, int N, int H, int W, int C, int crop_h, int crop_w,
                          float mirror_pr, float flip_pr, int train, uint64_t seed, hipStream_t stream);
int denet_dropout(const float* x, float* y, int N, int HW, int C, int C_logical, float rate, uint64_t seed,
                  hipStream_t stream);
int denet_concat_fwd(const float* a, const float* b, float* y, long rows, int CA, int CAP, int CB, int CBP, int CYP,
                     hipStream_t stream);
int denet_concat_bwd(const float* dy, float* da, float* db, long rows, int CA, int CAP, int CB, int CBP, int CYP,
                     hipStream_t stream);
int denet_add_bias(const float* x, const float* bias, float* y, long rows, int C, hipStream_t stream);

int denet_nchw_to_nhwc(const float* x, float* y, int N, int C, int H, int W, int CP, hipStream_t stream);
int denet_nhwc_to_nchw(const float* x, float* y, int N, int C, int H, int W, int CP, hipStream_t stream);
int denet_add(const float* a, const float* b, float* y, long n, int relu, hipStream_t stream);
int denet_relu_fwd(const float* x, float* y, long n, hipStream_t stream);
int denet_relu_bwd(const float* y, const float* dy, float* dx, long n, hipStream_t stream);
int denet_act_fwd(const float* x, float* y, long M, int C, int CP, int kind, hipStream_t stream);
int denet_act_bwd(const float* y, const float* dy, float* dx, long M, int C, int CP, int kind, hipStream_t stream);
int denet_add_act_fwd(const float* a, const float* b, float* y, long M, int C, int CP, int kind, hipStream_t stream);
size_t denet_colsum_workspace_bytes(long M, int C);
int denet_colsum(const float* x, float* out, void* workspace, long M, int C, hipStream_t stream);
int denet_solver_step(float* params, float* moments, const float* grads, long n, long n_decay, float lr,
                      float momentum, int iteration, float decay, float grad_scale, int mode, hipStream_t stream);
int denet_solver_adam(float* params, float* m, float* v, const float* grads, long n, long n_decay, float lr,
                      float beta1, float beta2, int iteration, float decay, float grad_scale, hipStream_t stream);
int denet_scale(float* x, long n, float s, hipStream_t stream);

int denet_corner_fwd(const float* conv, float* corner_pr, int B, int H, int W, int CP, int Cn, hipStream_t stream);
size_t denet_loss_workspace_bytes(void);
int denet_corner_loss(const float* corner_pr, const float* target, float* dconv, float* cost, void* workspace, int B,
                      int H, int W, int CP, int Cn, float cost_factor, hipStream_t stream);

int denet_sparse_fwd(const float* fmap, const float* bbox, float* out, int* taps, int B, int H, int W, int CP,
                     int coff, int F, int rois_per_image, int gs, int KP, int tap_rule, hipStream_t stream);
size_t denet_sparse_sort_workspace_bytes(int B, int H, int W, int rois_per_image, int gs);
int denet_sparse_sort_is_single(int B, int H, int W, int rois_per_image, int gs);
int denet_sparse_sort(const int* taps, void* sort_ws, size_t sort_ws_bytes, int B, int H, int W, int rois_per_image,
                      int gs, hipStream_t stream);
int denet_sparse_bwd(const float* dy, const int* taps, void* sort_ws, size_t sort_ws_bytes, float* dfmap, int B, int H,
                     int W, int CP, int coff, int F, int rois_per_image, int gs, int KP, int zero_from,
                     hipStream_t stream);

int denet_detect_loss(const float* logits, const float* det_target, const float* bbox_valid, const float* bbox_target,
                      const float* roi_bbox, const float* fit_target, float* dlogits, float* costs, void* workspace, int M,
                      int batch, int CP, int ncls, int nreg, int nfit, float cost_factor, float bbox_factor,
                      float fit_factor, int bounded_iou, hipStream_t stream);

int denet_detect_decode(const float* logits, const float* roi_bbox, float* det_pr, float* fitness, float* bbox, int M,
                        int CP, int class_num, int jointfit, int nreg, int nfit ,
                        float overlap_threshold, hipStream_t stream);
int denet_detect_nms(const float* det_pr, const float* fitness, const float* bbox, const int* count,
                     unsigned char* keep, int B, int S, int class_num, float pr_threshold, float nms_threshold,
                     hipStream_t stream);
int denet_soft_nms_host(const float* score_host, const float* box_host, int n, float nms_threshold,
                        int* out_order_host, float* out_score_host, int* out_n_host);
long denet_soft_nms_batch_host(const float* det_pr, const float* fitness, const float* bbox, const int* counts, int B, int S,
                               int class_num, float pr_threshold, float nms_threshold, float* out_score, int* out_cls,
                               int* out_row, int* out_count, long capacity);
size_t denet_soft_nms_workspace_bytes(int B, int S, int class_num);
int denet_soft_nms_batch(const float* det_pr, const float* fitness, const float* bbox, const int* count, int B, int S,
                         int class_num, float pr_threshold, float nms_threshold, float* out_score, int* out_cls, int* out_row,
                         int* out_count, int* out_total, void* workspace, size_t workspace_bytes, hipStream_t stream);

size_t denet_build_samples_workspace_bytes(int B, int Cn, int H, int W, int max_corners, int sample_count);
int denet_build_samples(const float* corner_pr, int* out_box, float* out_absd, int* out_count, void* workspace,
                        size_t workspace_bytes, int B, int Cn, int H, int W, float corner_threshold, int sample_count,
                        int max_corners, int local_max, hipStream_t stream);
int denet_edit_samples_device(const int* box, const int* count, int H, int W, const uint32_t* mt_out, long n_out, long cursor0,
                              const double* gt, const int* gt_off, int sample_gt, int B, int S, int n_keep, float* out_bbox,
                              int* status, hipStream_t stream);
int denet_build_samples_stats(const void* workspace, size_t workspace_bytes, int B, int Cn, int H, int W, int max_corners,
                              int sample_count, int* ncorner_out, unsigned* candidates_out, hipStream_t stream);
int denet_host_cluster_samples(const float* samples_host, int n, float threshold, int output_num, float* out_host,
                               int* out_count);
int denet_samples_finish_host(const int* box_host, const float* absd_host, const int* count_host, int B,
                              int sample_count, int H, int W, float* samples_host);

#ifdef __cplusplus
}
#endif
#endif
```

Before: 1086.

## Batch per-layer filter preparation into one launch per kind via descriptor table

```diff
diff --git a/denet_amd/build.py b/denet_amd/build.py
--- a/denet_amd/build.py
+++ b/denet_amd/build.py
@@ -8,7 +8,7 @@
 LIB = os.path.join(CSRC, "libdenet_hip.so")
 
 SOURCES = ["runtime.hip", "igemm.hip", "bn.hip", "pool.hip", "elementwise.hip", "dss.hip", "samples.hip", "detect.hip", "winograd.hip", "wino2f.hip", "wino4f.hip", "wino4t.hip", "dgrad_s2.hip", "wino4g.hip", "stem.hip", "gemm3b.hip", "bn_moments.hip",
-           "regression.hip", "augment.hip", "image.hip", "activation.hip", "conv_rect.hip", "pool_border.hip"]
+           "regression.hip", "augment.hip", "image.hip", "activation.hip", "conv_rect.hip", "pool_border.hip", "filter_batch.hip"]
 NO_CONTRACT = {"dss.hip", "samples.hip", "detect.hip", "augment.hip", "image.hip"}
 COMMON = ["--offload-arch=gfx950", "-O3", "-std=c++17", "-fPIC", "-Wall", "-Wno-unused-function"]
 
@@ -50,7 +50,7 @@
         hipcc = "hipcc"
     version = _hipcc_version(hipcc)
     objs, todo = [], []
-    headers = [os.path.join(CSRC, "common.h"), os.path.join(CSRC, "bn_final.h"), os.path.join(HERE, "..", "include", "denet_hip.h")]
+    headers = [os.path.join(CSRC, "common.h"), os.path.join(CSRC, "bn_final.h"), os.path.join(CSRC, "filter_batch.h"), os.path.join(HERE, "..", "include", "denet_hip.h")]
     for src in SOURCES:
         s = os.path.join(CSRC, src)
         o = os.path.join(CSRC, src.replace(".hip", ".o"))
diff --git a/denet_amd/csrc/dgrad_s2.hip b/denet_amd/csrc/dgrad_s2.hip
--- a/denet_amd/csrc/dgrad_s2.hip
+++ b/denet_amd/csrc/dgrad_s2.hip
@@ -1,5 +1,6 @@
 #include "common.h"
 #include "../../include/denet_hip.h"
+#include "filter_batch.h"
 #include <stdlib.h>
 
 namespace {
@@ -248,8 +249,8 @@
     }
 }
 
-__global__ __launch_bounds__(256) void dgrad_s2_pack_kernel(const float* __restrict__ w, float* __restrict__ P, int K, int C) {
-    const long idx = (long)blockIdx.x * 256 + threadIdx.x;
+__device__ __forceinline__ void dgrad_s2_pack_body(const float* __restrict__ w, float* __restrict__ P, int K, int C, unsigned block) {
+    const long idx = (long)block * 256 + threadIdx.x;
     const long total = 9L * K * C;
     if (idx >= total) return;
     const int kk = (int)(idx & 15);
@@ -261,6 +262,16 @@
     P[idx] = w[((long)(kc * 16 + kk) * 9 + tap) * C + c];
 }
 
+__global__ __launch_bounds__(256) void dgrad_s2_pack_kernel(const float* __restrict__ w, float* __restrict__ P, int K, int C) {
+    dgrad_s2_pack_body(w, P, K, C, blockIdx.x);
+}
+
+__global__ __launch_bounds__(256) void prep_dgrad_s2_pack_kernel(const float* __restrict__ params, const denet_prep_desc* __restrict__ t,
+                                                                 int n) {
+    const denet_prep_desc& d = prep_find(t, n, blockIdx.x);
+    dgrad_s2_pack_body(params + d.src_off, d.dst, d.K, d.C, blockIdx.x - (unsigned)d.first_wg);
+}
+
 }
 
 extern "C" int denet_conv_dgrad_s2_ok(int N, int H, int W, int C, int K) {
@@ -277,6 +288,12 @@
     const long total = 9L * K * C;
     hipLaunchKernelGGL(dgrad_s2_pack_kernel, dim3((unsigned)((total + 255) / 256)), dim3(256), 0, stream, w, packed, K, C);
     DENET_CHECK_LAUNCH("conv_dgrad_s2_pack");
+    return DENET_OK;
+}
+
+int denet_prep_launch_s2_pack(const float* params, const denet_prep_desc* t, int n, int wgs, hipStream_t stream) {
+    hipLaunchKernelGGL(prep_dgrad_s2_pack_kernel, dim3((unsigned)wgs), dim3(256), 0, stream, params, t, n);
+    DENET_CHECK_LAUNCH("wino_prepare_filters: dgrad_s2 pack");
     return DENET_OK;
 }
 
diff --git a/denet_amd/csrc/filter_batch.h b/denet_amd/csrc/filter_batch.h
--- /dev/null
+++ b/denet_amd/csrc/filter_batch.h
@@ -0,0 +1,20 @@
+#pragma once
+#include "common.h"
+#include "../../include/denet_hip.h"
+
+__device__ __forceinline__ const denet_prep_desc& prep_find(const denet_prep_desc* __restrict__ t, int n, unsigned wg) {
+    int lo = 0, hi = n - 1;
+    while (lo < hi) {
+        const int mid = (lo + hi + 1) >> 1;
+        if ((unsigned)t[mid].first_wg <= wg) lo = mid;
+        else hi = mid - 1;
+    }
+    return t[lo];
+}
+
+__host__ __device__ inline bool prep_dgrad_blocked(int K, int C) { return K % 16 == 0 && C % 16 == 0; }
+
+int denet_prep_launch_transform(int dgrad, const float* params, const denet_prep_desc* t, int n, int wgs, hipStream_t stream);
+int denet_prep_launch_wino4t_pack(const denet_prep_desc* t, int n, int wgs, hipStream_t stream);
+int denet_prep_launch_s2_pack(const float* params, const denet_prep_desc* t, int n, int wgs, hipStream_t stream);
+int denet_prep_launch_transpose(const float* params, const denet_prep_desc* t, int n, int wgs, hipStream_t stream);
diff --git a/denet_amd/csrc/filter_batch.hip b/denet_amd/csrc/filter_batch.hip
--- /dev/null
+++ b/denet_amd/csrc/filter_batch.hip
@@ -0,0 +1,78 @@
+#include "filter_batch.h"
+
+namespace {
+
+int prep_grid(denet_prep_desc* d) {
+    const long KC = (long)d->K * d->C;
+    long gx = 0, gy = 1;
+    switch (d->kind) {
+    case 0: gx = (KC + 255) / 256; break;
+    case 2:
+        if (prep_dgrad_blocked(d->K, d->C)) { gx = d->C / 16; gy = d->K / 16; }
+        else gx = (KC + 255) / 256;
+        break;
+    case 1:
+    case 3: gx = (36L * KC / 4 + 255) / 256; break;
+    case 4: gx = (9L * KC + 255) / 256; break;
+    case 5: gx = (d->C + 63) / 64; gy = (d->K + 63) / 64; break;
+    }
+    DENET_CHECK_ARG(gx > 0 && gx * gy < (1L << 31), "filter_batch_plan: a layer of %ld x %ld workgroups", gx, gy);
+    d->grid_x = (int32_t)gx;
+    d->grid_y = (int32_t)gy;
+    return DENET_OK;
+}
+
+}
+
+extern "C" int denet_filter_batch_plan(denet_prep_desc* descs, int n, int* plan) {
+    DENET_CHECK_ARG(descs && plan && n > 0, "filter_batch_plan: bad arguments");
+    for (int k = 0; k < 3 * DENET_PREP_KINDS; ++k) plan[k] = 0;
+    long wgs = 0;
+    for (int i = 0; i < n; ++i) {
+        denet_prep_desc* d = descs + i;
+        DENET_CHECK_ARG(d->kind >= 0 && d->kind < DENET_PREP_KINDS && (i == 0 || d->kind >= d[-1].kind),
+                        "filter_batch_plan: descriptor %d: kind %d (the table is sorted by kind, 0 .. %d)", i, d->kind, DENET_PREP_KINDS - 1);
+        DENET_CHECK_ARG(d->dst && d->K > 0 && d->C > 0, "filter_batch_plan: descriptor %d: null destination or empty shape", i);
+        if (d->kind == 1 || d->kind == 3) DENET_CHECK_ARG(d->src && d->C % 16 == 0, "filter_batch_plan: descriptor %d: wino4t pack needs a source and C %% 16 = 0", i);
+        else DENET_CHECK_ARG(d->src_off >= 0, "filter_batch_plan: descriptor %d: source in front of the parameter buffer", i);
+        if (d->kind == 0 || d->kind == 2) DENET_CHECK_ARG(d->tile == 2 || d->tile == 4, "filter_batch_plan: descriptor %d: tile %d", i, d->tile);
+        if (d->kind == 4) DENET_CHECK_ARG(d->K % 16 == 0, "filter_batch_plan: descriptor %d: dgrad_s2 pack needs K %% 16 = 0", i);
+        const int rc = prep_grid(d);
+        if (rc != DENET_OK) return rc;
+        int* p = plan + 3 * d->kind;
+        if (p[1] == 0) {
+            p[0] = i;
+            wgs = 0;
+        }
+        d->first_wg = (int32_t)wgs;
+        d->reserved = 0;
+        wgs += (long)d->grid_x * d->grid_y;
+        DENET_CHECK_ARG(wgs < (1L << 31), "filter_batch_plan: kind %d has too many workgroups", d->kind);
+        p[1] += 1;
+        p[2] = (int)wgs;
+    }
+    return DENET_OK;
+}
+
+extern "C" int denet_wino_prepare_filters(const float* params, const denet_prep_desc* table, const int* plan, int first_kind,
+                                          int last_kind, hipStream_t stream) {
+    DENET_CHECK_ARG(table && plan, "wino_prepare_filters: null table / plan");
+    DENET_CHECK_ARG(0 <= first_kind && first_kind <= last_kind && last_kind < DENET_PREP_KINDS, "wino_prepare_filters: kinds %d .. %d",
+                    first_kind, last_kind);
+    for (int kind = first_kind; kind <= last_kind; ++kind) {
+        const int first = plan[3 * kind], n = plan[3 * kind + 1], wgs = plan[3 * kind + 2];
+        if (n == 0) continue;
+        DENET_CHECK_ARG(first >= 0 && n > 0 && wgs >= n && (params || kind == 1 || kind == 3), "wino_prepare_filters: bad plan for kind %d", kind);
+        int rc = DENET_OK;
+        switch (kind) {
+        case 0:
+        case 2: rc = denet_prep_launch_transform(kind == 2, params, table + first, n, wgs, stream); break;
+        case 1:
+        case 3: rc = denet_prep_launch_wino4t_pack(table + first, n, wgs, stream); break;
+        case 4: rc = denet_prep_launch_s2_pack(params, table + first, n, wgs, stream); break;
+        case 5: rc = denet_prep_launch_transpose(params, table + first, n, wgs, stream); break;
+        }
+        if (rc != DENET_OK) return rc;
+    }
+    return DENET_OK;
+}
diff --git a/denet_amd/csrc/gemm3b.hip b/denet_amd/csrc/gemm3b.hip
--- a/denet_amd/csrc/gemm3b.hip
+++ b/denet_amd/csrc/gemm3b.hip
@@ -1,4 +1,5 @@
 #include "common.h"
+#include "filter_batch.h"
 
 namespace {
 
@@ -130,9 +131,9 @@
     }
 }
 
-__global__ __launch_bounds__(256) void transpose_f32_kernel(const float* __restrict__ src, float* __restrict__ dst, int R, int C) {
-    __shared__ float tile[64][65];
-    const int r0 = blockIdx.y * 64, c0 = blockIdx.x * 64;
+__device__ __forceinline__ void transpose_f32_body(const float* __restrict__ src, float* __restrict__ dst, int R, int C, int bx, int by,
+                                                   float (*tile)[65]) {
+    const int r0 = by * 64, c0 = bx * 64;
     const int tx = threadIdx.x & 63, ty = threadIdx.x >> 6;
 #pragma unroll
     for (int i = 0; i < 16; ++i) {
@@ -145,6 +146,19 @@
         const int c = c0 + ty + 4 * i, r = r0 + tx;
         if (r < R && c < C) dst[(long)c * R + r] = tile[tx][ty + 4 * i];
     }
+}
+
+__global__ __launch_bounds__(256) void transpose_f32_kernel(const float* __restrict__ src, float* __restrict__ dst, int R, int C) {
+    __shared__ float tile[64][65];
+    transpose_f32_body(src, dst, R, C, blockIdx.x, blockIdx.y, tile);
+}
+
+__global__ __launch_bounds__(256) void prep_transpose_kernel(const float* __restrict__ params, const denet_prep_desc* __restrict__ t,
+                                                             int n) {
+    __shared__ float tile[64][65];
+    const denet_prep_desc& d = prep_find(t, n, blockIdx.x);
+    const unsigned b = blockIdx.x - (unsigned)d.first_wg;
+    transpose_f32_body(params + d.src_off, d.dst, d.K, d.C, (int)(b % (unsigned)d.grid_x), (int)(b / (unsigned)d.grid_x), tile);
 }
 
 }
@@ -170,3 +184,9 @@
     DENET_CHECK_LAUNCH("transpose_f32");
     return DENET_OK;
 }
+
+int denet_prep_launch_transpose(const float* params, const denet_prep_desc* t, int n, int wgs, hipStream_t stream) {
+    hipLaunchKernelGGL(prep_transpose_kernel, dim3((unsigned)wgs), dim3(256), 0, stream, params, t, n);
+    DENET_CHECK_LAUNCH("wino_prepare_filters: transpose");
+    return DENET_OK;
+}
diff --git a/denet_amd/csrc/wino4t.hip b/denet_amd/csrc/wino4t.hip
--- a/denet_amd/csrc/wino4t.hip
+++ b/denet_amd/csrc/wino4t.hip
@@ -1,6 +1,7 @@
 #include "common.h"
 #include "bn_final.h"
 #include "../../include/denet_hip.h"
+#include "filter_batch.h"
 #include <stdlib.h>
 #include <type_traits>
 
@@ -441,8 +442,8 @@
     T_STAMP();
 }
 
-__global__ __launch_bounds__(256) void wino4t_pack_kernel(const float* __restrict__ U, float* __restrict__ P, int K, int C) {
-    const long idx = (long)blockIdx.x * 256 + threadIdx.x;
+__device__ __forceinline__ void wino4t_pack_body(const float* __restrict__ U, float* __restrict__ P, int K, int C, unsigned block) {
+    const long idx = (long)block * 256 + threadIdx.x;
     const long total = 36L * K * C / 4;
     if (idx >= total) return;
     const int q = (int)(idx & 3);
@@ -454,6 +455,15 @@
     *(f32x4*)(P + idx * 4) = *(const f32x4*)(U + ((long)xi * K + k) * C + chunk * 16 + q * 4);
 }
 
+__global__ __launch_bounds__(256) void wino4t_pack_kernel(const float* __restrict__ U, float* __restrict__ P, int K, int C) {
+    wino4t_pack_body(U, P, K, C, blockIdx.x);
+}
+
+__global__ __launch_bounds__(256) void prep_wino4t_pack_kernel(const denet_prep_desc* __restrict__ t, int n) {
+    const denet_prep_desc& d = prep_find(t, n, blockIdx.x);
+    wino4t_pack_body(d.src, d.dst, d.K, d.C, blockIdx.x - (unsigned)d.first_wg);
+}
+
 unsigned long long* g_w4t_dbg = nullptr;
 
 }
@@ -476,6 +486,12 @@
     const long total = 36L * K * C / 4;
     hipLaunchKernelGGL(wino4t_pack_kernel, dim3((unsigned)((total + 255) / 256)), dim3(256), 0, stream, u, packed, K, C);
     DENET_CHECK_LAUNCH("conv_wino4t_pack");
+    return DENET_OK;
+}
+
+int denet_prep_launch_wino4t_pack(const denet_prep_desc* t, int n, int wgs, hipStream_t stream) {
+    hipLaunchKernelGGL(prep_wino4t_pack_kernel, dim3((unsigned)wgs), dim3(256), 0, stream, t, n);
+    DENET_CHECK_LAUNCH("wino_prepare_filters: wino4t pack");
     return DENET_OK;
 }
 
diff --git a/denet_amd/csrc/winograd.hip b/denet_amd/csrc/winograd.hip
--- a/denet_amd/csrc/winograd.hip
+++ b/denet_amd/csrc/winograd.hip
@@ -1,6 +1,7 @@
 #include "common.h"
 #include <stdlib.h>
 #include "../../include/denet_hip.h"
+#include "filter_batch.h"
 
 int denet_gemm_batched_nt(const float* a, const float* w, float* out, int batch, int M, int Nc, int Kc, long stride_a,
                           long stride_w, long stride_out, hipStream_t stream);
@@ -405,10 +406,10 @@
 }
 
 template <int MO, bool DGRAD>
-__global__ __launch_bounds__(256) void wino_filter_kernel(const float* __restrict__ w, float* __restrict__ U, int K, int C) {
+__device__ __forceinline__ void wino_filter_body(const float* __restrict__ w, float* __restrict__ U, int K, int C, unsigned block) {
     using WT = Wino<MO>;
     constexpr int TS = WT::TS;
-    const long idx = (long)blockIdx.x * 256 + threadIdx.x;
+    const long idx = (long)block * 256 + threadIdx.x;
     if (idx >= (long)K * C) return;
     const int c = (int)(idx % C);
     const int k = (int)(idx / C);
@@ -438,14 +439,18 @@
         }
 }
 
+template <int MO, bool DGRAD>
+__global__ __launch_bounds__(256) void wino_filter_kernel(const float* __restrict__ w, float* __restrict__ U, int K, int C) {
+    wino_filter_body<MO, DGRAD>(w, U, K, C, blockIdx.x);
+}
+
 template <int MO>
-__global__ __launch_bounds__(256) void wino_filter_dgrad_kernel(const float* __restrict__ w, float* __restrict__ U, int K,
-                                                                int C) {
+__device__ __forceinline__ void wino_filter_dgrad_body(const float* __restrict__ w, float* __restrict__ U, int K, int C, int bx,
+                                                       int by, float (*tile)[16][17]) {
     using WT = Wino<MO>;
     constexpr int TS = WT::TS;
-    __shared__ float tile[TS * TS][16][17];
     const int kl = threadIdx.x >> 4, cl = threadIdx.x & 15;
-    const int k0 = blockIdx.y * 16, c0 = blockIdx.x * 16;
+    const int k0 = by * 16, c0 = bx * 16;
     {
         const int k = k0 + kl, c = c0 + cl;
         float g[3][3];
@@ -476,6 +481,30 @@
     const int co = threadIdx.x >> 4, ko = threadIdx.x & 15;
 #pragma unroll
     for (int xi = 0; xi < TS * TS; ++xi) U[(long)xi * KC + (long)(c0 + co) * K + k0 + ko] = tile[xi][co][ko];
+}
+
+template <int MO>
+__global__ __launch_bounds__(256) void wino_filter_dgrad_kernel(const float* __restrict__ w, float* __restrict__ U, int K,
+                                                                int C) {
+    __shared__ float tile[Wino<MO>::TS * Wino<MO>::TS][16][17];
+    wino_filter_dgrad_body<MO>(w, U, K, C, blockIdx.x, blockIdx.y, tile);
+}
+
+template <bool DGRAD>
+__global__ __launch_bounds__(256) void prep_filter_kernel(const float* __restrict__ params, const denet_prep_desc* __restrict__ t,
+                                                          int n) {
+    __shared__ float tile[DGRAD ? 36 : 1][16][17];
+    const denet_prep_desc& d = prep_find(t, n, blockIdx.x);
+    const unsigned b = blockIdx.x - (unsigned)d.first_wg;
+    const float* w = params + d.src_off;
+    if (DGRAD && prep_dgrad_blocked(d.K, d.C)) {
+        const int bx = (int)(b % (unsigned)d.grid_x), by = (int)(b / (unsigned)d.grid_x);
+        if (d.tile == 2) wino_filter_dgrad_body<2>(w, d.dst, d.K, d.C, bx, by, tile);
+        else wino_filter_dgrad_body<4>(w, d.dst, d.K, d.C, bx, by, tile);
+    } else {
+        if (d.tile == 2) wino_filter_body<2, DGRAD>(w, d.dst, d.K, d.C, b);
+        else wino_filter_body<4, DGRAD>(w, d.dst, d.K, d.C, b);
+    }
 }
 
 template <int MO>
@@ -701,7 +730,7 @@
 
 int wino_filter(int mo, bool dgrad, const float* w, float* U, int K, int C, hipStream_t stream) {
     const unsigned fb = (unsigned)(((long)K * C + 255) / 256);
-    if (dgrad && K % 16 == 0 && C % 16 == 0) {
+    if (dgrad && prep_dgrad_blocked(K, C)) {
         if (mo == 2) hipLaunchKernelGGL(wino_filter_dgrad_kernel<2>, dim3(C / 16, K / 16), dim3(256), 0, stream, w, U, K, C);
         else hipLaunchKernelGGL(wino_filter_dgrad_kernel<4>, dim3(C / 16, K / 16), dim3(256), 0, stream, w, U, K, C);
     } else if (dgrad) {
@@ -975,6 +1004,13 @@
     return wino_filter(tile, dgrad != 0, w, u, K, C, stream);
 }
 
+int denet_prep_launch_transform(int dgrad, const float* params, const denet_prep_desc* t, int n, int wgs, hipStream_t stream) {
+    if (dgrad) hipLaunchKernelGGL(prep_filter_kernel<true>, dim3((unsigned)wgs), dim3(256), 0, stream, params, t, n);
+    else hipLaunchKernelGGL(prep_filter_kernel<false>, dim3((unsigned)wgs), dim3(256), 0, stream, params, t, n);
+    DENET_CHECK_LAUNCH("wino_prepare_filters: filter transforms");
+    return DENET_OK;
+}
+
 extern "C" int denet_conv_wino_dgrad(const float* dy, const float* w, const float* u_cached, const float* add, float* dx,
                                      float* workspace, size_t workspace_bytes, int tile, int N, int H, int W, int C, int K,
                                      hipStream_t stream) {
diff --git a/denet_amd/lib.py b/denet_amd/lib.py
--- a/denet_amd/lib.py
+++ b/denet_amd/lib.py
@@ -103,6 +103,8 @@
     "denet_conv_wino4t_stats_rows": (I, [I] * 3),
     "denet_conv_wino4t_pack": (I, [P, P, I, I, P]),
     "denet_conv_wino4t_sums": (I, [P] * 5 + [I, P, Z, P, P] + [I] * 5 + [P]),
+    "denet_filter_batch_plan": (I, [P, I, P]),
+    "denet_wino_prepare_filters": (I, [P, P, P, I, I, P]),
     "denet_bn_bwd_final": (I, [P, I, L, I, P, P, P, P]),
     "denet_conv_wino_wgrad_dm": (I, [P, P, P, P, P, Z, P, Z] + [I] * 6 + [P]),
     "denet_bn_fwd_test": (I, [P] * 8 + [I, L, I, F, I, P]),
diff --git a/denet_amd/ops.py b/denet_amd/ops.py
--- a/denet_amd/ops.py
+++ b/denet_amd/ops.py
@@ -726,6 +726,11 @@
     return ent[0]
 
 
+FILTER_BATCH = os.environ.get("DENET_FILTER_BATCH", "1") != "0"
+_PREP = None
+_PREP_BUILDS = 0
+
+
 def wino_prefetch_filters(caches_and_weights, after=None):
     global _SIDE_FILTER
     todo = [(c, w) for c, w in caches_and_weights if c.get("fwd_tile_train") or c.get("dgrad_tile")]
@@ -740,54 +745,166 @@
     else:
         _SIDE_FILTER.wait_stream(torch.cuda.current_stream())
     with torch.cuda.stream(_SIDE_FILTER):
-        def run(items, dgrad, key):
-            for c, w in items:
-                tile = c.get(key)
+        if FILTER_BATCH:
+            _prefetch_batched(todo, tr, s2)
+        else:
+            _prefetch_per_layer(todo, tr, s2)
+
+
+def _u_entry(c, w, dgrad, tile):
+    ent = c.get(("u", dgrad))
+    if ent is None or ent[0] != tile:
+        ft = _filter_tile(tile)
+        K, _, _, C = w.shape
+        ent = c[("u", dgrad)] = [tile, torch.empty((ft + 2) * (ft + 2) * K * C, dtype=torch.float32, device="cuda"), False, None]
+    return ent
+
+
+def _wt_entry(c, w):
+    K = w.shape[0]
+    C = w.numel() // K
+    ent = c.get("wt")
+    if ent is None or ent[0].numel() != K * C:
+        ent = c["wt"] = [torch.empty(C, K, dtype=torch.float32, device="cuda"), False]
+    return ent, K, C
+
+
+def _ws2_entry(c, w):
+    ent = c.get("ws2")
+    if ent is None or ent[0].numel() != w.numel():
+        ent = c["ws2"] = [torch.empty(w.numel(), dtype=torch.float32, device="cuda"), False]
+    return ent
+
+
+def _prefetch_per_layer(todo, tr, s2):
+    def run(items, dgrad, key):
+        for c, w in items:
+            tile = c.get(key)
+            if not tile:
+                continue
+            ent = _u_entry(c, w, dgrad, tile)
+            if tile == FUSED4:
+                conv_wino4t_filter(w, dgrad, out=ent[1])
+            else:
+                conv_wino_filter(w, _filter_tile(tile), dgrad, out=ent[1])
+            ent[2] = True
+            ent[3] = WEIGHTS_VERSION
+        ev = torch.cuda.Event()
+        ev.record(_SIDE_FILTER)
+        for c, _ in items:
+            c[("u_event", dgrad)] = ev
+    for i in range(0, len(todo), 8):
+        run(todo[i:i + 8], 0, "fwd_tile_train")
+    run(todo, 1, "dgrad_tile")
+    if tr:
+        for c, w in tr:
+            ent, K, C = _wt_entry(c, w)
+            _transpose(w, K, C, out=ent[0])
+            ent[1] = True
+        ev = torch.cuda.Event()
+        ev.record(_SIDE_FILTER)
+        for c, _ in tr:
+            c["wt_event"] = ev
+    if s2:
+        for c, w in s2:
+            ent = _ws2_entry(c, w)
+            conv_dgrad_s2_pack(w, out=ent[0])
+            ent[1] = True
+        ev = torch.cuda.Event()
+        ev.record(_SIDE_FILTER)
+        for c, _ in s2:
+            c["ws2_event"] = ev
+
+
+class _PrepTable:
+
+    def __init__(self, key, todo, tr, s2):
+        import ctypes
+        import numpy
+        global _PREP_BUILDS
+        _PREP_BUILDS += 1
+        self.key = key
+        self.keep = [c for c, _ in todo + tr + s2]
+        self.u_ents, self.flag_ents, self.fwd_events, self.events = [], [], [], []
+        rows = []
+        for c, w in todo:
+            K, _, _, C = w.shape
+            for dgrad, name in ((0, "fwd_tile_train"), (1, "dgrad_tile")):
+                tile = c.get(name)
                 if not tile:
                     continue
-                ent = c.get(("u", dgrad))
-                ft = _filter_tile(tile)
-                if ent is None or ent[0] != tile:
-                    K, _, _, C = w.shape
-                    ent = c[("u", dgrad)] = [tile, torch.empty((ft + 2) * (ft + 2) * K * C, dtype=torch.float32, device="cuda"), False,
-                                             None]
+                ent = _u_entry(c, w, dgrad, tile)
+                self.u_ents.append(ent)
+                (self.fwd_events if dgrad == 0 else self.events).append((c, ("u_event", dgrad)))
                 if tile == FUSED4:
-                    conv_wino4t_filter(w, dgrad, out=ent[1])
+                    raw = c.get(("u4t_raw", dgrad))
+                    if raw is None or raw.numel() != 36 * K * C:
+                        raw = c[("u4t_raw", dgrad)] = torch.empty(36 * K * C, dtype=torch.float32, device="cuda")
+                    red, outc = (K, C) if dgrad else (C, K)
+                    rows.append((2 * dgrad, 4, w.data_ptr(), None, raw, K, C))
+                    rows.append((2 * dgrad + 1, 0, 0, raw, ent[1], outc, red))
                 else:
-                    conv_wino_filter(w, ft, dgrad, out=ent[1])
-                ent[2] = True
-                ent[3] = WEIGHTS_VERSION
-            ev = torch.cuda.Event()
-            ev.record(_SIDE_FILTER)
-            for c, _ in items:
-                c[("u_event", dgrad)] = ev
-        for i in range(0, len(todo), 8):
-            run(todo[i:i + 8], 0, "fwd_tile_train")
-        run(todo, 1, "dgrad_tile")
-        if tr:
-            for c, w in tr:
-                K = w.shape[0]
-                C = w.numel() // K
-                ent = c.get("wt")
-                if ent is None or ent[0].numel() != K * C:
-                    ent = c["wt"] = [torch.empty(C, K, dtype=torch.float32, device="cuda"), False]
-                _transpose(w, K, C, out=ent[0])
-                ent[1] = True
-            ev = torch.cuda.Event()
-            ev.record(_SIDE_FILTER)
-            for c, _ in tr:
-                c["wt_event"] = ev
-        if s2:
-            for c, w in s2:
-                ent = c.get("ws2")
-                if ent is None or ent[0].numel() != w.numel():
-                    ent = c["ws2"] = [torch.empty(w.numel(), dtype=torch.float32, device="cuda"), False]
-                conv_dgrad_s2_pack(w, out=ent[0])
-                ent[1] = True
-            ev = torch.cuda.Event()
-            ev.record(_SIDE_FILTER)
-            for c, _ in s2:
-                c["ws2_event"] = ev
+                    rows.append((2 * dgrad, _filter_tile(tile), w.data_ptr(), None, ent[1], K, C))
+        for c, w in s2:
+            K, _, _, C = w.shape
+            ent = _ws2_entry(c, w)
+            self.flag_ents.append(ent)
+            self.events.append((c, "ws2_event"))
+            rows.append((4, 0, w.data_ptr(), None, ent[0], K, C))
+        for c, w in tr:
+            ent, K, C = _wt_entry(c, w)
+            self.flag_ents.append(ent)
+            self.events.append((c, "wt_event"))
+            rows.append((5, 0, w.data_ptr(), None, ent[0], K, C))
+        rows.sort(key=lambda r: r[0])
+        self.keep.append([r[4] for r in rows])
+        self.base = min(r[2] for r in rows if r[0] not in (1, 3))
+        table = numpy.zeros(len(rows), dtype=PREP_DESC)
+        assert PREP_DESC.itemsize == 56
+        for i, (kind, tile, wp, src, dst, K, C) in enumerate(rows):
+            assert kind in (1, 3) or (wp - self.base) % 4 == 0
+            table[i] = (kind, tile, 0 if kind in (1, 3) else (wp - self.base) // 4, ptr(src) or 0, ptr(dst), K, C, 0, 0, 0, 0)
+        self.plan = (ctypes.c_int * 18)()
+        check(_L().denet_filter_batch_plan(table.ctypes.data, len(rows), self.plan), "filter_batch_plan")
+        self.host = table
+        self.table = torch.from_numpy(table.view(numpy.uint8)).cuda()
+
+    def run(self, first_kind, last_kind):
+        check(_L().denet_wino_prepare_filters(self.base, ptr(self.table), self.plan, first_kind, last_kind, stream_ptr()),
+              "wino_prepare_filters")
+
+
+def _prep_desc_dtype():
+    import numpy
+    return numpy.dtype([("kind", "<i4"), ("tile", "<i4"), ("src_off", "<i8"), ("src", "<u8"), ("dst", "<u8"), ("K", "<i4"), ("C", "<i4"),
+                        ("grid_x", "<i4"), ("grid_y", "<i4"), ("first_wg", "<i4"), ("reserved", "<i4")], align=True)
+
+
+PREP_DESC = _prep_desc_dtype()
+
+
+def _prefetch_batched(todo, tr, s2):
+    global _PREP
+    key = tuple((id(c), w.data_ptr(), w.shape, c.get("fwd_tile_train"), c.get("dgrad_tile")) for c, w in todo) + (None,) + \
+        tuple((id(c), w.data_ptr(), w.shape) for c, w in tr) + (None,) + tuple((id(c), w.data_ptr(), w.shape) for c, w in s2)
+    if _PREP is None or _PREP.key != key:
+        _PREP = _PrepTable(key, todo, tr, s2)
+    prep = _PREP
+    prep.run(0, 1)
+    ev = torch.cuda.Event()
+    ev.record(_SIDE_FILTER)
+    for c, name in prep.fwd_events:
+        c[name] = ev
+    prep.run(2, 5)
+    ev = torch.cuda.Event()
+    ev.record(_SIDE_FILTER)
+    for ent in prep.u_ents:
+        ent[2] = True
+        ent[3] = WEIGHTS_VERSION
+    for ent in prep.flag_ents:
+        ent[1] = True
+    for c, name in prep.events:
+        c[name] = ev
 
 
 _SIDE_FILTER = None
diff --git a/denet_amd/switches.py b/denet_amd/switches.py
--- a/denet_amd/switches.py
+++ b/denet_amd/switches.py
@@ -36,6 +36,7 @@
     "DENET_WGRAD_STREAM": ("1", "kernels", "the filter-gradient chain of the backward sweep on a second stream"),
     "DENET_SHORT_HANDOFF": ("1", "host", "the short forms of the RoI hand-off (device-side editing / one native call)"),
     "DENET_HANDOFF_WARM_MS": ("0.25", "host", "milliseconds between dry runs of the hand-off's native call while the host waits for the proposal (0: none)"),
+    "DENET_FILTER_BATCH": ("1", "launches", "the filter preparation of a training step (Winograd transforms, wino4t / stride-2 packs, transposes) as one launch per kind (6 in all) over a descriptor table (csrc/filter_batch.hip; 0: one launch per layer and kind). The same device functions: the prepared filters and every product kernel's result are bit-identical"),
     "DENET_SIDE_SORT": ("1", "kernels", "the gather gradient's tap sort queued right behind the forward gather"),
     "DENET_SORT_ONE_KERNEL": ("1", "kernels", "the tap sort as one 1024-thread workgroup per image"),
     "DENET_SOFT_NMS_HOST": ("unset", "host", "inference: force the host (1) / device (0) form of Gaussian soft-NMS"),
diff --git a/include/denet_hip.h b/include/denet_hip.h
--- a/include/denet_hip.h
+++ b/include/denet_hip.h
@@ -160,6 +160,20 @@
 int denet_conv_wino4t_sums(const float* x, const float* u_packed, const float* bias, const float* add, float* y, int relu,
                            double* stats_partial, size_t stats_bytes, int* stats_rows, const denet_bn_link* sums_of, int N, int H,
                            int W, int C, int K, hipStream_t stream);
+#define DENET_PREP_KINDS 6
+typedef struct denet_prep_desc {
+    int32_t kind, tile;
+    int64_t src_off;
+    const float* src;
+    float* dst;
+    int32_t K, C;
+    int32_t grid_x, grid_y;
+    int32_t first_wg;
+    int32_t reserved;
+} denet_prep_desc;
+int denet_filter_batch_plan(denet_prep_desc* descs, int n, int* plan);
+int denet_wino_prepare_filters(const float* params, const denet_prep_desc* table, const int* plan, int first_kind, int last_kind,
+                               hipStream_t stream);
 int denet_conv_wino_wgrad_dm(const float* x, const float* dm, const float* v_cached, float* dw, float* workspace,
                              size_t workspace_bytes, float* split_ws, size_t split_ws_bytes, int tile, int N, int H, int W, int C,
                              int K, hipStream_t stream);
```

Result: no change. 1077 (median of 2 runs) (-0.8%).
